# schmidtniko/visual_marker_mapping

Measured on AMD Instinct MI355X. Metric: lm_iterations_per_sec, higher is better.
Workload: dtype f64; 1 GPU; configs[1]: 500 images x 200 tags, visibility 1.00, 100000 tag observations (400000 corner residual blocks), no loss, perturbed initial guess; eliminated_family=cameras, reduced_system_order=1200, elimination_form=dense Z + MFMA rank-k, kept_family_order=natural

## Files before the change

### __graft_entry__.py

```python
import os
import subprocess
import sys

ROOT = os.path.dirname(os.path.abspath(__file__))
if ROOT not in sys.path:
    sys.path.insert(0, ROOT)


def build():
    jobs = str(min(8, os.cpu_count() or 2))
    subprocess.check_call(["make", "-C", os.path.join(ROOT, "visual_marker_mapping_amd", "csrc"), "-j", jobs, "all", "stamps"])
    subprocess.check_call(["make", "-C", os.path.join(ROOT, "tools"), "all"])
    subprocess.check_call(["make", "-C", os.path.join(ROOT, "oracle"), "all"])
    subprocess.check_call(["make", "-C", os.path.join(ROOT, "tests", "cpp"), "all"])
    import visual_marker_mapping_amd
    from visual_marker_mapping_amd import _lib
    L = _lib.lib()
    missing = [s for s in _lib.EXPORTS if not hasattr(L, s)]
    if missing:
        raise RuntimeError("libvmm_ba.so lacks symbols: %s" % missing)


def smoke():
    import numpy as np
    from oracle import oracle as O
    from visual_marker_mapping_amd import engine as eng
    from visual_marker_mapping_amd.synthetic import make_scene

    s = make_scene(1)
    ba = eng.BundleAdjuster(s.intr, s.dist, s.cam_init, s.tag_init, s.tag_wh, s.fixed_tag, s.obs_cam,
                            s.obs_tag, s.obs_px, device=0)
    out = ba.solve(eng.default_options(robustify=1), trace_capacity=64)
    cam, tag = ba.get_state()
    ba.close()
    sc = O.Scene(s.intr, s.dist, s.cam_init, s.tag_init, s.tag_wh, s.fixed_tag, s.obs_cam, s.obs_tag, s.obs_px)
    summ, _ = O.solve(sc, O.default_options(robustify=1, linear_solver=O.DENSE_NORMAL))
    assert out["termination_type"] == summ["termination_type"] == O.CONVERGENCE, (out, summ)
    assert out["iterations"] == summ["iterations"], (out["iterations"], summ["iterations"])
    assert abs(out["final_cost"] - summ["final_cost"]) <= 1e-8 * summ["final_cost"]
    scale = max(np.abs(sc.cam_qt).max(), np.abs(sc.tag_qt).max())
    assert np.abs(cam - sc.cam_qt).max() <= 1e-6 * scale
    assert np.abs(tag - sc.tag_qt).max() <= 1e-6 * scale
    print("smoke ok: %d iterations, final cost %.9g (oracle %.9g)" % (out["iterations"], out["final_cost"],
                                                                    summ["final_cost"]))


if __name__ == "__main__":
    build()
    if len(sys.argv) > 1 and sys.argv[1] == "smoke":
        smoke()
```

### include/vmm_ba.h

```cpp
#ifndef VMM_BA_H_
#define VMM_BA_H_

#include <stddef.h>
#include <stdint.h>

#ifdef __cplusplus
extern "C" {
#endif

#define VMM_BA_ABI_VERSION 6

typedef struct vmm_ba_handle_s* vmm_ba_handle;

enum {
    VMM_BA_OK = 0,
    VMM_BA_ERR_ARGUMENT = 1,
    VMM_BA_ERR_HIP = 2,
    VMM_BA_ERR_COLLECTIVE = 3,
    VMM_BA_ERR_STATE = 4,
    VMM_BA_ERR_NUMERIC = 5
};

enum {
    VMM_BA_ELIM_AUTO = 0,
// ... 259 lines not shown
    int32_t robustify;
    double  huber_a;
    double  score_cap_px;
    double  inlier_px;
    int32_t reclassify_passes;
    int32_t min_inlier_views;
    int32_t max_pair_views;
    int32_t reserved;
} vmm_ba_triangulate_options;

typedef struct vmm_ba_triangulate_result {
    int32_t status, n_obs, n_inlier_obs, trials;
    double  rms_px, cost;
} vmm_ba_triangulate_result;

void vmm_ba_default_triangulate_options(vmm_ba_triangulate_options* o);
int vmm_ba_triangulate(const double intr[4], const double dist[5],
                       int32_t n_cams, const double* cam_qt,
                       const double* cam_cov,
                       int32_t n_pts, const int64_t* pt_start,
                       const int32_t* obs_cam, const double* obs_uv,
                       const vmm_ba_triangulate_options* o,
                       double* xyz,
                       double* xyz_cov,
                       double* xyz_cov_cams,
                       uint8_t* obs_inlier,
                       vmm_ba_triangulate_result* res,
                       int device);

int vmm_ba_locate_tags(const double intr[4], const double dist[5],
                       int32_t n_cams, const double* cam_qt,
                       const double* cam_cov,
                       int32_t n_tags, const double* tag_wh,
                       const int64_t* tag_start,
                       const int32_t* obs_cam, const double* obs_px,
                       const vmm_ba_localize_options* o,
                       double* tag_qt,
                       double* tag_cov,
                       double* tag_cov_cams,
                       uint8_t* obs_inlier,
                       vmm_ba_localize_result* res,
                       int device);

enum { VMM_BA_PRED_OK = 0, VMM_BA_PRED_NO_VISIBLE_TAG = 1, VMM_BA_PRED_TOO_FEW_TAGS = 2, VMM_BA_PRED_SINGULAR = 3 };
typedef struct vmm_ba_predict_options {
    int32_t image_width, image_height;
    double  sigma_px;
    double  margin_px;
    double  min_depth;
    double  max_view_angle_deg;
    double  min_side_px;
    int32_t min_tags;
    int32_t reserved;
} vmm_ba_predict_options;

typedef struct vmm_ba_predict_result {
    int32_t status;
    int32_t n_visible;
    double  sigma_pos_m;
    double  sigma_rot_rad;
} vmm_ba_predict_result;

void vmm_ba_default_predict_options(vmm_ba_predict_options* o);
int vmm_ba_predict_localization(const double intr[4], const double dist[5],
                                int32_t n_tags, const double* tag_qt, const double* tag_wh,
                                const double* tag_cov,
                                int32_t n_poses, const double* cam_qt,
                                const vmm_ba_predict_options* o,
                                double* cov_px,
                                double* cov_map,
                                uint8_t* visible,
                                vmm_ba_predict_result* res,
                                int device);

int vmm_ba_predict_localization_joint(const double intr[4], const double dist[5],
                                      int32_t n_tags, const double* tag_qt, const double* tag_wh,
                                      const double* tag_cov_joint,
                                      int32_t n_poses, const double* cam_qt,
                                      const uint8_t* visible_in,
                                      const vmm_ba_predict_options* o,
                                      double* cov_px,
                                      double* cov_map,
                                      uint8_t* visible,
                                      vmm_ba_predict_result* res,
                                      int device);

enum { VMM_BA_CAL_OK = 0, VMM_BA_CAL_NO_IMAGES = 1, VMM_BA_CAL_SINGULAR = 2, VMM_BA_CAL_NO_CONVERGENCE = 3 };
typedef struct vmm_ba_calibrate_options {
    vmm_ba_localize_options loc;
    int32_t max_trials;
    int32_t refine_mask;
    int32_t robustify;
    int32_t reclassify_passes;
    int32_t min_inlier_tags;
    int32_t reserved;
    double  huber_a;
    double  inlier_px;
} vmm_ba_calibrate_options;
typedef struct vmm_ba_calibrate_report {
    int32_t status, trials, accepted, passes, n_images_used, n_obs_used;
    double initial_cost, final_cost, initial_rms_px, final_rms_px, time_s;
} vmm_ba_calibrate_report;
void vmm_ba_default_calibrate_options(vmm_ba_calibrate_options* o);
int vmm_ba_calibrate(const double intr0[4], const double dist0[5],
                     int32_t n_tags, const double* tag_qt, const double* tag_wh,
                     int32_t n_imgs, const int64_t* img_start, const int32_t* obs_tag, const double* obs_px,
                     const vmm_ba_calibrate_options* o,
                     double intr[4], double dist[5],
                     double* intr_cov,
                     double* cam_qt,
                     double* cam_cov,
                     uint8_t* obs_inlier,
                     vmm_ba_localize_result* res,
                     vmm_ba_calibrate_report* rep,
                     int device);

int vmm_ba_set_intrinsics(vmm_ba_handle h, const double intr[4], const double dist[5]);
int vmm_ba_get_intrinsics(vmm_ba_handle h, double intr[4], double dist[5]);

int vmm_ba_intrinsics_system(vmm_ba_handle h, int robustify, double huber_a, double* cost, double g_k[9], double C[81],
                             double r_k[9], double S_k[81]);

typedef struct vmm_ba_selfcal_options {
    int32_t max_outer_iterations;
    int32_t refine_mask;
    double parameter_tolerance;
    double function_tolerance;
} vmm_ba_selfcal_options;
typedef struct vmm_ba_selfcal_report {
    int32_t status;
    int32_t outer_iterations;
    int32_t accepted;
    int32_t inner_lm_iterations;
    double initial_cost;
    double final_cost;
    double time_s;
} vmm_ba_selfcal_report;
void vmm_ba_default_selfcal_options(vmm_ba_selfcal_options* o);
int vmm_ba_solve_selfcal(vmm_ba_handle h, const vmm_ba_options* inner, const vmm_ba_selfcal_options* o,
                         vmm_ba_summary* last_inner, vmm_ba_selfcal_report* report, double intr[4], double dist[5],
                         double* intr_cov );

int vmm_ba_eval_blocks(vmm_ba_handle h, int robustify, double huber_a, double* cost, double* V,
                       double* U, double* W, double* g_cam, double* g_tag);

int vmm_ba_dense_spd_solve(int device, int n, const double* A, const double* b, double* x, int* info);

int vmm_ba_dense_syrk(int device, int k, int n, const double* Z, double* C);

int vmm_ba_pose_plus(int64_t n, const double* qt, const double* delta, double* out, int device);

int vmm_ba_debug_overlap(vmm_ba_handle h, int reps, double* ms);

int vmm_ba_debug_chol_schedule(int n_blk, int n_df, int n_cu, int32_t* launches, int cap, int* n_launches, int* n_df_used);
int vmm_ba_debug_chol_tile(int n_blk, const int32_t* launch, int t, int* bi, int* bj);

int vmm_ba_time_kernels(vmm_ba_handle h, const vmm_ba_options* opt, int reps, vmm_ba_kernel_times* out);

#ifdef __cplusplus
}
#endif
#endif
```

### visual_marker_mapping_amd/_lib.py

```python
import ctypes as C
import os

_HERE = os.path.dirname(os.path.abspath(__file__))
LIB_PATH = os.environ.get("VMM_BA_LIB") or os.path.join(_HERE, "libvmm_ba.so")

ABI_VERSION = 6
RCCL_ID_BYTES = 128
PRECISION_F64, PRECISION_F32_ACCUM = 0, 1
LANDMARK_TAG_POSES, LANDMARK_POINTS = 0, 1
RIG_MAX_CAMS = 8
OK, ERR_ARGUMENT, ERR_HIP, ERR_COLLECTIVE, ERR_STATE, ERR_NUMERIC = 0, 1, 2, 3, 4, 5
ELIM_AUTO, ELIM_TAGS, ELIM_CAMERAS = 0, 1, 2
CONVERGENCE, NO_CONVERGENCE, FAILURE = 0, 1, 2
LOC_OK, LOC_NO_OBSERVATIONS, LOC_NO_CANDIDATE, LOC_TOO_FEW_INLIERS, LOC_SINGULAR = 0, 1, 2, 3, 4
LOC_STATUS_NAMES = ("ok", "no_observations", "no_candidate", "too_few_inliers", "singular")
TRI_OK, TRI_TOO_FEW_VIEWS, TRI_NO_CANDIDATE, TRI_TOO_FEW_INLIERS, TRI_SINGULAR = 0, 1, 2, 3, 4
TRI_STATUS_NAMES = ("ok", "too_few_views", "no_candidate", "too_few_inliers", "singular")
CAL_OK, CAL_NO_IMAGES, CAL_SINGULAR, CAL_NO_CONVERGENCE = 0, 1, 2, 3
CAL_STATUS_NAMES = ("ok", "no_images", "singular", "no_convergence")
PRED_OK, PRED_NO_VISIBLE_TAG, PRED_TOO_FEW_TAGS, PRED_SINGULAR = 0, 1, 2, 3
PRED_STATUS_NAMES = ("ok", "no_visible_tag", "too_few_tags", "singular")


class Problem(C.Structure):
# ... 35 lines not shown
                ("num_lm_iterations", C.c_int32), ("num_jacobian_evals", C.c_int32),
                ("num_cost_evals", C.c_int32), ("elimination", C.c_int32),
                ("initial_cost", C.c_double), ("final_cost", C.c_double), ("time_solve_s", C.c_double),
                ("trace", C.POINTER(Iteration)), ("trace_capacity", C.c_int32), ("reserved", C.c_int32),
                ("time_eval_s", C.c_double), ("time_eliminate_s", C.c_double), ("time_factor_solve_s", C.c_double),
                ("time_step_s", C.c_double), ("time_control_s", C.c_double),
                ("num_sync_timeouts", C.c_int32), ("sync_timeout_kernels", C.c_int32),
                ("block_sparse", C.c_int32), ("tree_ordering", C.c_int32)]


class KernelTimes(C.Structure):
    _fields_ = [("eval_elim_ms", C.c_double), ("eval_keep_ms", C.c_double), ("cost_ms", C.c_double),
                ("form_z_ms", C.c_double), ("syrk_ms", C.c_double), ("cholesky_ms", C.c_double),
                ("backsub_ms", C.c_double), ("lm_iteration_ms", C.c_double), ("n_obs", C.c_int64),
                ("reduced_dim", C.c_int32), ("elim_dim", C.c_int32), ("schur_sparse", C.c_int32),
                ("syrk_wide", C.c_int32), ("schur_flops", C.c_double), ("chol_flops", C.c_double)]


class InitOptions(C.Structure):
    _fields_ = [("sweeps", C.c_int32), ("min_tag_observations", C.c_int32), ("score_cap_px", C.c_double),
                ("refine_iterations", C.c_int32), ("reserved", C.c_int32)]


class InitReport(C.Structure):
    _fields_ = [("rounds", C.c_int32), ("cams_reached", C.c_int32), ("tags_reached", C.c_int32),
                ("reserved", C.c_int32), ("avg_reprojection_px", C.c_double), ("time_s", C.c_double)]


class LocalizeOptions(C.Structure):
    _fields_ = [("refine_iterations", C.c_int32), ("robustify", C.c_int32), ("huber_a", C.c_double),
                ("score_cap_px", C.c_double), ("inlier_px", C.c_double), ("reclassify_passes", C.c_int32),
                ("min_inlier_tags", C.c_int32)]


class LocalizeResult(C.Structure):
    _fields_ = [("status", C.c_int32), ("n_obs", C.c_int32), ("n_inlier_obs", C.c_int32), ("trials", C.c_int32),
                ("rms_px", C.c_double), ("cost", C.c_double)]


class TriangulateOptions(C.Structure):
    _fields_ = [("refine_iterations", C.c_int32), ("robustify", C.c_int32), ("huber_a", C.c_double),
                ("score_cap_px", C.c_double), ("inlier_px", C.c_double), ("reclassify_passes", C.c_int32),
                ("min_inlier_views", C.c_int32), ("max_pair_views", C.c_int32), ("reserved", C.c_int32)]


class TriangulateResult(C.Structure):
    _fields_ = [("status", C.c_int32), ("n_obs", C.c_int32), ("n_inlier_obs", C.c_int32), ("trials", C.c_int32),
                ("rms_px", C.c_double), ("cost", C.c_double)]


class PredictOptions(C.Structure):
    _fields_ = [("image_width", C.c_int32), ("image_height", C.c_int32), ("sigma_px", C.c_double), ("margin_px", C.c_double),
                ("min_depth", C.c_double), ("max_view_angle_deg", C.c_double), ("min_side_px", C.c_double),
                ("min_tags", C.c_int32), ("reserved", C.c_int32)]


class PredictResult(C.Structure):
    _fields_ = [("status", C.c_int32), ("n_visible", C.c_int32), ("sigma_pos_m", C.c_double), ("sigma_rot_rad", C.c_double)]


class CalibrateOptions(C.Structure):
    _fields_ = [("loc", LocalizeOptions), ("max_trials", C.c_int32), ("refine_mask", C.c_int32),
                ("robustify", C.c_int32), ("reclassify_passes", C.c_int32), ("min_inlier_tags", C.c_int32),
                ("reserved", C.c_int32), ("huber_a", C.c_double), ("inlier_px", C.c_double)]


class CalibrateReport(C.Structure):
    _fields_ = [("status", C.c_int32), ("trials", C.c_int32), ("accepted", C.c_int32), ("passes", C.c_int32),
                ("n_images_used", C.c_int32), ("n_obs_used", C.c_int32), ("initial_cost", C.c_double),
                ("final_cost", C.c_double), ("initial_rms_px", C.c_double), ("final_rms_px", C.c_double),
                ("time_s", C.c_double)]


class RigCalibrateOptions(C.Structure):
    _fields_ = [("loc", LocalizeOptions), ("max_trials", C.c_int32), ("refine_mask", C.c_int32),
                ("robustify", C.c_int32), ("reclassify_passes", C.c_int32), ("min_inlier_tags", C.c_int32),
                ("reserved", C.c_int32), ("huber_a", C.c_double), ("inlier_px", C.c_double)]


class RigCalibrateReport(C.Structure):
    _fields_ = [("status", C.c_int32), ("trials", C.c_int32), ("accepted", C.c_int32), ("passes", C.c_int32),
                ("n_frames_used", C.c_int32), ("n_obs_used", C.c_int32), ("cams_refined", C.c_int32),
                ("reserved", C.c_int32), ("initial_cost", C.c_double), ("final_cost", C.c_double),
                ("initial_rms_px", C.c_double), ("final_rms_px", C.c_double), ("time_s", C.c_double)]


class SelfcalOptions(C.Structure):
    _fields_ = [("max_outer_iterations", C.c_int32), ("refine_mask", C.c_int32), ("parameter_tolerance", C.c_double),
                ("function_tolerance", C.c_double)]


class SelfcalReport(C.Structure):
    _fields_ = [("status", C.c_int32), ("outer_iterations", C.c_int32), ("accepted", C.c_int32),
                ("inner_lm_iterations", C.c_int32), ("initial_cost", C.c_double), ("final_cost", C.c_double),
                ("time_s", C.c_double)]


ALLREDUCE_FN = C.CFUNCTYPE(C.c_int, C.c_void_p, C.c_void_p, C.c_size_t, C.c_void_p)

_h = _a = C.c_void_p
_i, _i32, _i64, _d, _P = C.c_int, C.c_int32, C.c_int64, C.c_double, C.POINTER
_MAP = [_i32, _a, _a]
_BATCH = [_i32, _a, _a, _a]
SIGNATURES = {
    "vmm_ba_last_error": (C.c_char_p, []),
    "vmm_ba_abi_version": (_i, []),
    "vmm_ba_default_options": (None, [_P(Options)]),
    "vmm_ba_default_create_options": (None, [_P(CreateOptions)]),
    "vmm_ba_create": (_i, [_P(Problem), _P(CreateOptions), _P(C.c_void_p)]),
    "vmm_ba_destroy": (None, [_h]),
    "vmm_ba_set_state": (_i, [_h, _a, _a]),
    "vmm_ba_get_state": (_i, [_h, _a, _a]),
    "vmm_ba_get_points": (_i, [_h, _a]),
    "vmm_ba_set_allreduce": (_i, [_h, ALLREDUCE_FN, C.c_void_p]),
    "vmm_ba_rccl_available": (_i, []),
    "vmm_ba_rccl_unique_id": (_i, [_a]),
    "vmm_ba_enable_rccl": (_i, [_h, _a]),
    "vmm_ba_set_observation_mask": (_i, [_h, _a]),
    "vmm_ba_set_constant_poses": (_i, [_h, _a, _a]),
    "vmm_ba_solve": (_i, [_h, _P(Options), _P(Summary)]),
    "vmm_ba_cost": (_i, [_h, _i, _d, _P(_d)]),
    "vmm_ba_reprojection_stats": (_i, [_h, _a, _a, _P(_d), _a]),
    "vmm_ba_tag_translation_covariance": (_i, [_h, _i, _d, _a]),
    "vmm_ba_covariance_blocks": (_i, [_h, _i, _d, _i64, _a, _a, _a]),
    "vmm_ba_project_points": (_i, [_a, _a, _i64, _a, _a, _i]),
    "vmm_ba_quad_poses": (_i, [_a, _a, _i64, _a, _a, _a, _a, _i]),
    "vmm_ba_default_init_options": (None, [_P(InitOptions)]),
    "vmm_ba_initialize": (_i, [_h, _P(InitOptions), _P(InitReport), _a, _a]),
    "vmm_ba_default_localize_options": (None, [_P(LocalizeOptions)]),
    "vmm_ba_localize": (_i, [_a, _a] + _MAP + _BATCH + [_P(LocalizeOptions), _a, _a, _a, _a, _i]),
    "vmm_ba_rig_localize": (_i, [_i32, _a, _a, _a] + _MAP + _BATCH + [_P(LocalizeOptions), _a, _a, _a, _a, _i]),
    "vmm_ba_default_rig_calibrate_options": (None, [_P(RigCalibrateOptions)]),
    "vmm_ba_rig_calibrate": (_i, [_i32, _a, _a, _a] + _MAP + _BATCH + [_P(RigCalibrateOptions), _a, _a, _a, _a, _a, _a,
                                  _P(RigCalibrateReport), _i]),
    "vmm_ba_default_triangulate_options": (None, [_P(TriangulateOptions)]),
    "vmm_ba_triangulate": (_i, [_a, _a, _i32, _a, _a] + _BATCH + [_P(TriangulateOptions), _a, _a, _a, _a, _a, _i]),
    "vmm_ba_locate_tags": (_i, [_a, _a, _i32, _a, _a, _i32, _a, _a, _a, _a, _P(LocalizeOptions), _a, _a, _a, _a, _a, _i]),
    "vmm_ba_default_predict_options": (None, [_P(PredictOptions)]),
    "vmm_ba_predict_localization": (_i, [_a, _a] + _MAP + [_a, _i32, _a, _P(PredictOptions), _a, _a, _a, _a, _i]),
    "vmm_ba_predict_localization_joint": (_i, [_a, _a] + _MAP + [_a, _i32, _a, _a, _P(PredictOptions), _a, _a, _a, _a, _i]),
    "vmm_ba_default_calibrate_options": (None, [_P(CalibrateOptions)]),
    "vmm_ba_calibrate": (_i, [_a, _a] + _MAP + _BATCH + [_P(CalibrateOptions), _a, _a, _a, _a, _a, _a, _a,
                              _P(CalibrateReport), _i]),
    "vmm_ba_set_intrinsics": (_i, [_h, _a, _a]),
    "vmm_ba_get_intrinsics": (_i, [_h, _a, _a]),
    "vmm_ba_intrinsics_system": (_i, [_h, _i, _d, _P(_d), _a, _a, _a, _a]),
    "vmm_ba_default_selfcal_options": (None, [_P(SelfcalOptions)]),
    "vmm_ba_solve_selfcal": (_i, [_h, _P(Options), _P(SelfcalOptions), _P(Summary), _P(SelfcalReport), _a, _a, _a]),
    "vmm_ba_eval_blocks": (_i, [_h, _i, _d, _P(_d), _a, _a, _a, _a, _a]),
    "vmm_ba_dense_spd_solve": (_i, [_i, _i, _a, _a, _a, _P(_i)]),
    "vmm_ba_dense_syrk": (_i, [_i, _i, _i, _a, _a]),
    "vmm_ba_pose_plus": (_i, [_i64, _a, _a, _a, _i]),
    "vmm_ba_debug_overlap": (_i, [_h, _i, _a]),
    "vmm_ba_debug_chol_schedule": (_i, [_i, _i, _i, _a, _i, _a, _a]),
    "vmm_ba_debug_chol_tile": (_i, [_i, _a, _i, _a, _a]),
    "vmm_ba_time_kernels": (_i, [_h, _P(Options), _i, _P(KernelTimes)]),
}
EXPORTS = list(SIGNATURES)
OPTIONAL = {"vmm_ba_covariance_blocks", "vmm_ba_rig_localize", "vmm_ba_default_rig_calibrate_options", "vmm_ba_rig_calibrate",
            "vmm_ba_default_calibrate_options", "vmm_ba_calibrate", "vmm_ba_default_triangulate_options",
            "vmm_ba_triangulate", "vmm_ba_locate_tags", "vmm_ba_default_predict_options", "vmm_ba_predict_localization",
            "vmm_ba_predict_localization_joint",
            "vmm_ba_set_intrinsics", "vmm_ba_get_intrinsics", "vmm_ba_intrinsics_system",
            "vmm_ba_default_selfcal_options", "vmm_ba_solve_selfcal"}

_LIB = None


class VmmBaError(RuntimeError):
    def __init__(self, status, message):
        super().__init__("libvmm_ba status %d: %s" % (status, message))
        self.status = status


def lib():
    global _LIB
    if _LIB is None:
        if not os.path.exists(LIB_PATH):
            raise ImportError("%s is missing: build it with __graft_entry__.build() or "
                              "make -C visual_marker_mapping_amd/csrc" % LIB_PATH)
        L = C.CDLL(LIB_PATH)
        L.vmm_ba_abi_version.restype = C.c_int
        if L.vmm_ba_abi_version() != ABI_VERSION:
            raise ImportError("%s has ABI version %d, this binding needs %d: rebuild it"
                              % (LIB_PATH, L.vmm_ba_abi_version(), ABI_VERSION))
        for name, (restype, argtypes) in SIGNATURES.items():
            if name in OPTIONAL and not hasattr(L, name):
                continue
            fn = getattr(L, name)
            fn.restype, fn.argtypes = restype, argtypes
        _LIB = L
    return _LIB


def check(status):
    if status != OK:
        raise VmmBaError(status, lib().vmm_ba_last_error().decode("utf-8", "replace"))
```

### visual_marker_mapping_amd/csrc/diagnostics.hip

```cpp
#include <stdio.h>
#include <string.h>

#include <string>
#include <vector>

#include "host.hpp"

namespace vmm {

template <typename T, hipError_t (*Destroy)(T), int N = 1>
struct Owned {
    T h[N] = {};
    Owned() = default;
    Owned(const Owned&) = delete;
    Owned& operator=(const Owned&) = delete;
    ~Owned() { release(); }
    void release()
    {
        for (T& x : h) {
            if (x)
                (void)Destroy(x);
            x = nullptr;
        }
    }
// ... 120 lines not shown
    for (int r = 0; r < reps; ++r) {
        if ((rc = run_iteration(e, ot))) return rc;
        passes += e.last_passes;
    }
    HIP_TRY(hipEventRecord(ev1, e.stream));
    HIP_TRY(hipEventSynchronize(ev1));
    float ms = 0.f;
    HIP_TRY(hipEventElapsedTime(&ms, ev0, ev1));
    out->lm_iteration_ms = ms / passes;
    events.release();
    return restore_raw();
}

int vmm_ba_debug_chol_schedule(int n_blk, int n_df, int n_cu, int32_t* launches, int cap, int* n_launches, int* n_df_used)
{
    if (n_blk < 1 || n_cu < 1 || cap < 0 || (cap > 0 && !launches) || !n_launches || (n_df > 0 && n_df > n_blk - 2)) {
        set_error("bad argument");
        return VMM_BA_ERR_ARGUMENT;
    }
    if (n_df < 0) {
        n_df = dataflow_blocks(n_blk, n_cu, read_switches());
        if (n_df == n_blk)
            n_df = 0;
    }
    const std::vector<CholLaunch> sched = chol_step_schedule(n_blk, n_df);
    for (size_t i = 0; i < sched.size() && (int)i < cap; ++i) {
        const CholLaunch& L = sched[i];
        const int32_t row[8] = { L.k, L.lazy[0], L.lazy[1], L.upd[0], L.upd[1], L.c0, L.t0, L.t1 };
        memcpy(launches + 8 * i, row, sizeof(row));
    }
    *n_launches = (int)sched.size();
    if (n_df_used)
        *n_df_used = n_df;
    return VMM_BA_OK;
}

int vmm_ba_debug_chol_tile(int n_blk, const int32_t* launch, int t, int* bi, int* bj)
{
    if (!launch || !bi || !bj || t < 0 || t >= launch[7]) {
        set_error("bad argument");
        return VMM_BA_ERR_ARGUMENT;
    }
    const CholLaunch L = { launch[0], { launch[1], launch[2] }, { launch[3], launch[4] }, launch[5], launch[6], launch[7] };
    chol_schedule_tile(n_blk, L, t, bi, bj);
    return VMM_BA_OK;
}

int vmm_ba_debug_overlap(vmm_ba_handle h, int reps, double* ms)
{
    if (!h || !ms || reps <= 0) {
        set_error("bad argument");
        return VMM_BA_ERR_ARGUMENT;
    }
    Engine& e = *reinterpret_cast<Engine*>(h);
    if (e.multi || e.sparse_schur || !e.Z) {
        set_error("debug_overlap needs a single-GPU handle on the dense elimination path");
        return VMM_BA_ERR_STATE;
    }
    HIP_TRY(hipSetDevice(e.device));
    int rc;
    if ((rc = flush_state(e))) return rc;
    vmm_ba_options o;
    vmm_ba_default_options(&o);
    o.max_num_iterations = 1 << 30;
    o.function_tolerance = o.parameter_tolerance = o.gradient_tolerance = 0.0;
    if (e.trace_capacity < 1) {
        if ((rc = dev_alloc(e, &e.trace, 1, false))) return rc;
        e.trace_capacity = 1;
        drop_graphs(e);
    }
    if ((rc = begin_lm_loop(e, o, 0))) return rc;
    if ((rc = enqueue_iteration(e, o))) return rc;
    HIP_TRY(hipStreamSynchronize(e.stream));
    Arena scratch;
    Owned<hipStream_t, hipStreamDestroy> second;
    OwnedEvents<5> events;
    hipStream_t& sb = second.h[0];
    hipEvent_t(&ev)[5] = events.h;
    hipError_t err = scratch.alloc(sizeof(double) * (size_t)e.ldz * e.ldz);
    double* const S2 = reinterpret_cast<double*>(scratch.base);
    if (err == hipSuccess) err = hipStreamCreateWithFlags(&sb, hipStreamNonBlocking);
    for (int i = 0; i < 5 && err == hipSuccess; ++i)
        err = hipEventCreate(&ev[i]);
    auto reset_flags = [&]() -> hipError_t {
        hipError_t r = hipMemcpy(e.ctl_host, e.ctl, sizeof(LmCtl), hipMemcpyDeviceToHost);
        if (r != hipSuccess) return r;
        e.ctl_host->done = 0;
        e.ctl_host->lin_fail = 0;
        e.ctl_host->sync_timeout = 0;
        return hipMemcpy(e.ctl, e.ctl_host, sizeof(LmCtl), hipMemcpyHostToDevice);
    };
    double acc[8] = { 0.0, 0.0, 0.0, 0.0, 0.0, 0.0, 0.0, 0.0 };
    for (int r = 0; r < reps + 1 && err == hipSuccess; ++r) {
        float t[8] = { 0.f, 0.f, 0.f, 0.f, 0.f, 0.f, 0.f, 0.f };
        if ((err = reset_flags()) != hipSuccess) break;
        (void)hipEventRecord(ev[0], e.stream);
        launch_syrk_reduced(e);
        (void)hipEventRecord(ev[1], e.stream);
        launch_cholesky_solve(e, e.S, e.n_pad, e.ldz, e.yf, e.ctl);
        (void)hipEventRecord(ev[2], e.stream);
        if ((err = hipEventSynchronize(ev[2])) != hipSuccess) break;
        (void)hipEventElapsedTime(&t[0], ev[0], ev[1]);
        (void)hipEventElapsedTime(&t[1], ev[1], ev[2]);
        (void)hipEventElapsedTime(&t[2], ev[0], ev[2]);
        if ((err = reset_flags()) != hipSuccess) break;
        launch_syrk_reduced(e);
        if ((err = hipStreamSynchronize(e.stream)) != hipSuccess) break;
        (void)hipEventRecord(ev[0], e.stream);
        (void)hipStreamWaitEvent(sb, ev[0], 0);
        launch_cholesky_solve(e, e.S, e.n_pad, e.ldz, e.yf, e.ctl);
        (void)hipEventRecord(ev[3], e.stream);
        launch_syrk_plan(sb, e.ctl, e.Z, e.ldz, e.syrk);
        launch_reduce_plan(sb, e.ctl, e.syrk, e.ldz, e.n_pad + 1, S2);
        (void)hipEventRecord(ev[1], sb);
        (void)hipStreamWaitEvent(e.stream, ev[1], 0);
        (void)hipEventRecord(ev[2], e.stream);
        if ((err = hipEventSynchronize(ev[2])) != hipSuccess) break;
        (void)hipEventElapsedTime(&t[3], ev[0], ev[2]);
        (void)hipEventElapsedTime(&t[4], ev[0], ev[3]);
        (void)hipEventElapsedTime(&t[5], ev[0], ev[1]);
        if ((err = reset_flags()) != hipSuccess) break;
        launch_syrk_reduced(e);
        if ((err = hipStreamSynchronize(e.stream)) != hipSuccess) break;
        (void)hipEventRecord(ev[0], e.stream);
        (void)hipStreamWaitEvent(sb, ev[0], 0);
        launch_syrk_plan(sb, e.ctl, e.Z, e.ldz, e.syrk);
        launch_reduce_plan(sb, e.ctl, e.syrk, e.ldz, e.n_pad + 1, S2);
        (void)hipEventRecord(ev[1], sb);
        (void)hipEventRecord(ev[4], e.stream);
        launch_cholesky_solve(e, e.S, e.n_pad, e.ldz, e.yf, e.ctl);
        (void)hipEventRecord(ev[3], e.stream);
        (void)hipStreamWaitEvent(e.stream, ev[1], 0);
        (void)hipEventRecord(ev[2], e.stream);
        if ((err = hipEventSynchronize(ev[2])) != hipSuccess) break;
        (void)hipEventElapsedTime(&t[6], ev[0], ev[2]);
        (void)hipEventElapsedTime(&t[7], ev[4], ev[3]);
        if (r > 0)
            for (int i = 0; i < 8; ++i)
                acc[i] += t[i];
    }
    if (err == hipSuccess)
        err = hipGetLastError();
    events.release();
    second.release();
    if (err != hipSuccess) {
        set_error(std::string("debug_overlap: ") + hipGetErrorString(err));
        return VMM_BA_ERR_HIP;
    }
    for (int i = 0; i < 8; ++i)
        ms[i] = acc[i] / reps;
    return VMM_BA_OK;
}

}
```

### visual_marker_mapping_amd/csrc/engine.hpp

```cpp
#pragma once
#include <hip/hip_runtime.h>
#include <stdint.h>

#include <string>
#include <vector>

#include "../../include/vmm_ba.h"
#include "geom.hpp"
#include "plan.hpp"

namespace vmm {

constexpr int kLdsRow = 80;

struct ObsOrder {
    int64_t n = 0;
    int64_t n_pad = 0;
    int32_t* own = nullptr;
    int32_t* other = nullptr;
    int32_t* caller = nullptr;
    double* px = nullptr;
    Task* tasks = nullptr;
    int32_t n_tasks = 0;
    int32_t* pose_task = nullptr;
    double* part = nullptr;
    int32_t* start = nullptr;
};

struct LmCtl {
    int32_t max_num_iterations, robustify, jacobi_scaling, max_invalid;
    double huber_a, function_tolerance, gradient_tolerance, parameter_tolerance;
    double max_radius, min_radius, min_relative_decrease, min_lm_diagonal, max_lm_diagonal;
    double radius, decrease_factor;
    int32_t reuse_diagonal, num_invalid;
    double x_cost, cand_cost, model_cost_change, x_norm, initial_cost;
    int32_t iteration;
    int32_t first_eval;
    int32_t done, termination;
    int32_t lin_fail;
    int32_t sync_timeout;
    int32_t num_sync_timeouts;
    int32_t sync_kernels;
    uint32_t spin_limit_df, spin_limit_chain;
    int32_t spin_wg;
    int32_t records;
    int32_t num_successful, num_unsuccessful, num_lm_iterations, num_jac_evals, num_cost_evals;
    int32_t trace_capacity;
    int32_t w_which;
    vmm_ba_iteration cur;
    unsigned long long stamp[6];
    unsigned long long phase_ticks[5];
};

__device__ __forceinline__ int64_t small_sel(const LmCtl* ctl, const int64_t alt_off) { return ctl->w_which ? alt_off : 0; }

__device__ __forceinline__ void phase_stamp(const LmCtl* ctl, int slot)
{
    if (blockIdx.x == 0 && blockIdx.y == 0 && threadIdx.x == 0)
        const_cast<LmCtl*>(ctl)->stamp[slot] = __builtin_amdgcn_s_memrealtime();
}

struct SyrkPlan {
    int n_tiles = 0, n_kt = 0, n_wg = 0, n_segments = 0;
    int32_t *tile_bi = nullptr, *tile_bj = nullptr, *wg_seg0 = nullptr, *tile_seg0 = nullptr;
    int64_t *wg_u0 = nullptr, *wg_u1 = nullptr;
    double* partials = nullptr;
    bool wide = false;
};

struct Engine {
    int device = 0;
    int n_cu = 256;
    hipStream_t stream = nullptr;
    int rank = 0, world = 1;
    Switches sw;
    bool multi = false;
    vmm_ba_allreduce_fn allreduce = nullptr;
    void* allreduce_user = nullptr;
    void* rccl_comm = nullptr;
    bool rccl_graph = true;

    Intrinsics K;
    int n_cams = 0, n_tags = 0, fixed_tag = -1;
    bool points = false;
    int n_tags_user = 0;
    int64_t n_obs_user = 0;
    std::vector<double> user_tag_wh;
    int64_t n_obs = 0;
    bool elim_cams = true;
    int n_e = 0, n_f = 0;

    double* cam_qt = nullptr;
    double* tag_qt = nullptr;
    double* cam_cand = nullptr;
    double* tag_cand = nullptr;
    double* tag_wh = nullptr;

    ObsOrder ordE, ordF;

    double* small = nullptr;
    size_t small_count = 0;
    double *H_cam = nullptr, *H_tag = nullptr, *g_cam = nullptr, *g_tag = nullptr, *cost_slot = nullptr;
    double* small_stage = nullptr;
    int64_t small_alt_off = 0;
    double *ev_H_cam = nullptr, *ev_H_tag = nullptr, *ev_g_cam = nullptr, *ev_g_tag = nullptr, *ev_cost = nullptr;
    double* ev_pose_cost = nullptr;
    double* W = nullptr;
    double* W2 = nullptr;
    float* Wf2 = nullptr;
    uint8_t* obs_mask = nullptr;
    uint8_t* pose_const = nullptr;
    bool any_const = false;
    float* Wf = nullptr;
    bool f32_accum = false;

    bool fused_eval = false;
    int32_t* pair_obs = nullptr;
    int32_t* fused_e_list = nullptr;
    int32_t* fused_e_part0 = nullptr;
    int32_t* fused_pose_task = nullptr;
    double* fused_partE = nullptr;
    double* fused_partF = nullptr;
    int fused_n_e_act = 0, fused_f_pad = 0, fused_chunks = 0, fused_group = 1, fused_groups = 0;

    double *scale = nullptr, *diag = nullptr, *D2 = nullptr, *delta = nullptr;
    int32_t* active = nullptr;

    double* Le = nullptr;
    double* ze = nullptr;
    double* Z = nullptr;
    int k_dim = 0, k_pad = 0;
    int n_red = 0, n_pad = 0, ldz = 0, n_blk = 0;
    bool sparse_schur = false;
    double* Zc = nullptr;
    int32_t* f2e = nullptr;
    int32_t* pair_start = nullptr;
    int32_t* pair_tstart = nullptr;
    int32_t* pair_terms = nullptr;
    int32_t* row_items = nullptr;
    double co_terms = 0.0;
    bool explicit_pairs = false;
    int32_t* pair_col = nullptr;
    int32_t* row_of = nullptr;
    int32_t* pose_of_row = nullptr;
    std::vector<int32_t> h_row_of;
    unsigned long long* chol_nz = nullptr;
    unsigned char* chol_order = nullptr;
    int32_t* df_wg = nullptr;
    int32_t* df_slot = nullptr;
    int n_df_wg = 0;
    size_t df_tree_slots = 0;
    bool chol_nz_on = false;
    std::vector<int32_t> nd_node_first_blk;
    int n_row_items = 0;
    double schur_flops = 0.0;
    double chol_flops = 0.0;
    SyrkPlan syrk;
    double* S = nullptr;
    double* S_packed = nullptr;
    double* P = nullptr;
    double* P4[4] = { nullptr, nullptr, nullptr, nullptr };
    double* dinv = nullptr;
    double* Ldiag = nullptr;
    double* Linv = nullptr;
    unsigned* flags = nullptr;
    unsigned long long* gran = nullptr;
    unsigned long long* df_gran = nullptr;
    double* df_compact = nullptr;
    unsigned* df_done = nullptr;
    double* yf = nullptr;
    double* step_comm = nullptr;
    double* cost_comm = nullptr;
    double* part_cost = nullptr;
    double* part_cross = nullptr;
    double* part_k1 = nullptr;
    double* pose_part = nullptr;
    double* pose_gm = nullptr;

    double* stats_part = nullptr;
    int32_t* stats_cnt = nullptr;
    double* stats_pose = nullptr;
    double* stats_corner = nullptr;

    double* init_quad_qt = nullptr;
    double* init_quad_rms = nullptr;
    int32_t* init_placed = nullptr;
    int32_t* init_todo = nullptr;
    int32_t* init_counter = nullptr;
    double* init_stats = nullptr;
    double* init_host = nullptr;

    LmCtl* ctl = nullptr;
    LmCtl* ctl_host = nullptr;
    double* pose_stage = nullptr;
    hipEvent_t pose_ev = nullptr;
    bool pose_ev_pending = false;
    double* pose_stage_dev = nullptr;
    bool dirty_cam = false, dirty_tag = false;
    vmm_ba_iteration* trace = nullptr;
    int trace_capacity = 0;

    hipGraphExec_t iter_graph = nullptr;
    hipGraphExec_t iter_graph_seg[5] = { nullptr, nullptr, nullptr, nullptr, nullptr };
    int graph_robustify = -1;
    double graph_huber_a = 0.0;
    int last_passes = 1;
    bool launched_eagerly = false;

    std::vector<void*> allocs;
};

void set_error(const std::string& s);

__host__ __device__ inline Intrinsics make_intrinsics(const double intr[4], const double dist[5])
{
    Intrinsics K;
    K.fx = intr[0]; K.fy = intr[1]; K.cx = intr[2]; K.cy = intr[3];
    K.k1 = dist[0]; K.k2 = dist[1]; K.p1 = dist[2]; K.p2 = dist[3]; K.k3 = dist[4];
    return K;
}
__host__ __device__ inline Intrinsics make_intrinsics(const double k[9]) { return make_intrinsics(k, k + 4); }

struct Arena {
    char* base = nullptr;
    size_t used = 0;
    hipError_t err = hipSuccess;
    Arena() = default;
    Arena(const Arena&) = delete;
    Arena& operator=(const Arena&) = delete;
    ~Arena()
    {
        if (base)
            (void)hipFree(base);
    }
    hipError_t alloc(size_t bytes)
    {
        err = hipMalloc((void**)&base, bytes);
        if (err != hipSuccess)
            base = nullptr;
        return err;
    }
    static size_t round(size_t bytes) { return (bytes + 255) & ~(size_t)255; }
    template <typename T>
    T* take(size_t count)
    {
        T* p = base ? reinterpret_cast<T*>(base + used) : nullptr;
        used += round(count * sizeof(T));
        return p;
    }
    template <typename Carve>
    hipError_t layout(Carve&& carve)
    {
        carve(*this);
        const size_t total = used;
        used = 0;
        if (alloc(total) == hipSuccess)
            carve(*this);
        return err;
    }
    void copy(void* dst, const void* src, size_t bytes, hipMemcpyKind kind)
    {
        if (err == hipSuccess)
            err = hipMemcpy(dst, src, bytes, kind);
    }
};

int preload_eval_kernels();
int preload_schur_kernels();
int preload_chol_kernels();
int preload_lm_kernels();
int preload_cov_kernels();
int preload_init_kernels();

void launch_eval_passes(Engine& e, int robustify, double huber_a, bool use_ctl);
void launch_cost_kernel(Engine& e, const double* cam, const double* tag, bool guard, int robustify, double huber_a);
void launch_cost(Engine& e, const double* cam, const double* tag, bool guard, int robustify, double huber_a,
// ... 254 lines not shown
```

### visual_marker_mapping_amd/csrc/kernels_eval.hip

```cpp
#include "engine.hpp"

namespace vmm {

struct EvalArgs {
    Intrinsics K;
    const Task* tasks;
    int n_tasks;
    const int32_t* other;
    const double* px;
    int64_t n_pad;
    const double* own_pose;
    const double* other_pose;
    const double* tag_wh;
    const uint8_t* cam_const;
    const uint8_t* tag_const;
    int robustify;
    double huber_a;
    double* part;
    void* W;
    void* W_alt;
    const int32_t* caller;
    const uint8_t* mask;
    const LmCtl* ctl;
};

__device__ __forceinline__ int tri(int a, int b) { return a * (a + 1) / 2 + b; }

template <bool OWN_IS_CAM, bool WRITE_W, typename AT, bool POINTS = false>
__device__ __forceinline__ void eval_body(const EvalArgs& a, const int wave)
{
    const int lane = threadIdx.x & 63;
    if (wave >= a.n_tasks)
        return;
    const Task t = a.tasks[wave];
    const int64_t i = (int64_t)t.begin + lane;
    const bool valid = i < t.end;
    const int64_t is = valid ? i : t.begin;
    const int o = a.other[is];
    AT* __restrict__ const Wout = static_cast<AT*>((WRITE_W && a.W_alt && a.ctl && a.ctl->w_which == 0) ? a.W_alt : a.W);

    const int tag_idx = OWN_IS_CAM ? o : t.pose;
    const int cam_idx = OWN_IS_CAM ? t.pose : o;
    const double* camq = (OWN_IS_CAM ? a.own_pose : a.other_pose) + 7 * (int64_t)cam_idx;
    const double* tagq = (OWN_IS_CAM ? a.other_pose : a.own_pose) + 7 * (int64_t)tag_idx;
    Rigid cam, tag;
    double pt[6];
    if (POINTS) {
        load_rigid<false>(camq, cam);
#pragma unroll
        for (int k = 0; k < 6; ++k)
            pt[k] = tagq[k];
    } else {
        load_rigid<true>(camq, cam);
        load_rigid<true>(tagq, tag);
    }
    const double hw = POINTS ? 0.0 : 0.5 * a.tag_wh[2 * tag_idx], hh = POINTS ? 0.0 : 0.5 * a.tag_wh[2 * tag_idx + 1];
    const bool cam_c = a.cam_const[cam_idx] != 0, tag_c = a.tag_const[tag_idx] != 0;
    const bool on = valid && a.mask[a.caller[is]];

    AT H[21];
    double g[6], cost = 0.0;
    AT Wacc[WRITE_W ? 36 : 1];
#pragma unroll
    for (int k = 0; k < 21; ++k)
        H[k] = (AT)0;
#pragma unroll
    for (int k = 0; k < 6; ++k)
        g[k] = 0.0;
    if (WRITE_W) {
#pragma unroll
        for (int k = 0; k < 36; ++k)
            Wacc[k] = (AT)0;
    }

    constexpr bool NEED_JC = OWN_IS_CAM || WRITE_W;
    constexpr bool NEED_JT = !OWN_IS_CAM || WRITE_W;
#pragma unroll 1
    for (int c = 0; c < (POINTS ? 2 : 4); ++c) {
        const double sx = (c == 1 || c == 2) ? hw : -hw;
        const double sy = (c >= 2) ? hh : -hh;
        const double u = a.px[(2 * c) * a.n_pad + is];
        const double v = a.px[(2 * c + 1) * a.n_pad + is];
        CornerEval e;
        if (POINTS) {
            eval_point<NEED_JC, NEED_JT>(a.K, cam, camq, pt[3 * c], pt[3 * c + 1], pt[3 * c + 2], u, v, e, on);
            if (NEED_JT) {
#pragma unroll
                for (int r = 0; r < 2; ++r) {
                    const double j0 = e.jt[r][0], j1 = e.jt[r][1], j2 = e.jt[r][2];
                    e.jt[r][0] = c == 0 ? j0 : 0.0;
                    e.jt[r][1] = c == 0 ? j1 : 0.0;
                    e.jt[r][2] = c == 0 ? j2 : 0.0;
                    e.jt[r][3] = c == 0 ? 0.0 : j0;
                    e.jt[r][4] = c == 0 ? 0.0 : j1;
                    e.jt[r][5] = c == 0 ? 0.0 : j2;
                }
            }
        } else {
            eval_corner<NEED_JC, NEED_JT>(a.K, cam, tag, sx, sy, u, v, e, on);
        }
        const double s = e.ru * e.ru + e.rv * e.rv;
        double rho0, wgt;
        huber(a.robustify != 0, a.huber_a, s, rho0, wgt);
        wgt = on ? wgt : 0.0;
        cost += on ? 0.5 * rho0 : 0.0;
        const double w_cam = cam_c ? 0.0 : wgt, w_tag = tag_c ? 0.0 : wgt;
        const double w_own = OWN_IS_CAM ? w_cam : w_tag;
        const double w_oth = OWN_IS_CAM ? w_tag : w_cam;
#pragma unroll
        for (int r = 0; r < 2; ++r) {
            const double res = (r == 0 ? e.ru : e.rv) * wgt;
            double jo[6];
#pragma unroll
            for (int k = 0; k < 6; ++k)
                jo[k] = (OWN_IS_CAM ? e.jc[r][k] : e.jt[r][k]) * w_own;
            AT ja[6];
#pragma unroll
            for (int k = 0; k < 6; ++k)
                ja[k] = (AT)jo[k];
#pragma unroll
            for (int p = 0; p < 6; ++p) {
                g[p] += jo[p] * res;
#pragma unroll
                for (int q = 0; q <= p; ++q)
                    H[tri(p, q)] += ja[p] * ja[q];
            }
            if (WRITE_W) {
                AT jx[6];
#pragma unroll
                for (int k = 0; k < 6; ++k)
                    jx[k] = (AT)((OWN_IS_CAM ? e.jt[r][k] : e.jc[r][k]) * w_oth);
#pragma unroll
                for (int p = 0; p < 6; ++p)
#pragma unroll
                    for (int q = 0; q < 6; ++q)
                        Wacc[6 * p + q] += ja[p] * jx[q];
            }
        }
    }
    if (WRITE_W && valid) {
#pragma unroll
        for (int k = 0; k < 36; ++k)
            Wout[(int64_t)k * a.n_pad + i] = Wacc[k];
    }
    double red[32];
#pragma unroll
    for (int k = 0; k < 21; ++k)
        red[k] = (double)H[k];
#pragma unroll
    for (int k = 0; k < 6; ++k)
        red[21 + k] = g[k];
    red[27] = cost;
#pragma unroll
    for (int k = 28; k < 32; ++k)
        red[k] = 0.0;
    const double mine = wave_sum32(red, lane);
    const int slot = wave_sum32_index(lane);
    if (!(lane & 1) && slot < 28)
        a.part[(int64_t)wave * kPart + slot] = mine;
}

template <bool E_IS_CAM, typename AT = double, bool POINTS = false>
__global__ __launch_bounds__(256) __attribute__((amdgpu_waves_per_eu(2, 2))) void k_eval_both(const EvalArgs aE, const EvalArgs aF, const int nb_e)
{
    if (aE.ctl) {
        if (aE.ctl->done)
            return;
        phase_stamp(aE.ctl, 0);
    }
    if ((int)blockIdx.x < nb_e)
        eval_body<E_IS_CAM, true, AT, POINTS>(aE, (int)((blockIdx.x * blockDim.x + threadIdx.x) >> 6));
    else
        eval_body<!E_IS_CAM, false, AT, POINTS>(aF, (int)(((blockIdx.x - nb_e) * blockDim.x + threadIdx.x) >> 6));
}


struct FusedArgs {
    const int32_t* pair_obs;
    const int32_t* e_list;
    const int32_t* e_part0;
    int n_e_act, n_f, n_f_pad, n_chunks, group, n_groups;
    double* partF;
};

template <bool E_IS_CAM, typename AT, bool POINTS>
__global__ __launch_bounds__(256) __attribute__((amdgpu_waves_per_eu(1, 1)))
void k_eval_fused(const EvalArgs a, const FusedArgs fa)
{
    if (a.ctl) {
        if (a.ctl->done)
            return;
        phase_stamp(a.ctl, 0);
    }
    const int lane = threadIdx.x & 63;
    const int wave = (int)((blockIdx.x * blockDim.x + threadIdx.x) >> 6);
    if (wave >= fa.n_groups * fa.n_chunks)
        return;
    const int grp = wave / fa.n_chunks, c = wave - grp * fa.n_chunks;
    const int f = 64 * c + lane;
    const bool fvalid = f < fa.n_f;
    const int fs = fvalid ? f : fa.n_f - 1;
    AT* __restrict__ const Wout = static_cast<AT*>((a.W_alt && a.ctl && a.ctl->w_which == 0) ? a.W_alt : a.W);
    const double* keptq = a.other_pose + 7 * (int64_t)fs;
    Rigid kept;
    double pt[6];
    if (POINTS && E_IS_CAM) {
#pragma unroll
        for (int k = 0; k < 6; ++k)
            pt[k] = keptq[k];
    } else if (POINTS) {
        load_rigid<false>(keptq, kept);
    } else {
        load_rigid<true>(keptq, kept);
    }
    AT HF[21];
    double gF[6];
#pragma unroll
    for (int k = 0; k < 21; ++k)
        HF[k] = (AT)0;
#pragma unroll
    for (int k = 0; k < 6; ++k)
        gF[k] = 0.0;
    const int e0 = grp * fa.group, e1 = min(e0 + fa.group, fa.n_e_act);
    constexpr int NPX = POINTS ? 4 : 8;
    int e_n = __builtin_amdgcn_readfirstlane(fa.e_list[e0]);
    int idx_n = fvalid ? fa.pair_obs[(int64_t)e_n * fa.n_f_pad + f] : -1;
    int e_nn = e_n, idx_nn = -1;
    if (e0 + 1 < e1) {
        e_nn = __builtin_amdgcn_readfirstlane(fa.e_list[e0 + 1]);
        idx_nn = fvalid ? fa.pair_obs[(int64_t)e_nn * fa.n_f_pad + f] : -1;
    }
    double px_n[NPX];
    int on_n;
    {
        const int64_t isn = idx_n >= 0 ? idx_n : 0;
#pragma unroll
        for (int k = 0; k < NPX; ++k)
            px_n[k] = a.px[(int64_t)k * a.n_pad + isn];
        on_n = idx_n >= 0 && a.mask[a.caller[isn]];
    }
    for (int ei = e0; ei < e1; ++ei) {
        const int e = e_n;
        const int idx = idx_n;
        const bool valid = idx >= 0;
        const bool on = on_n != 0;
        double pxc[NPX];
#pragma unroll
        for (int k = 0; k < NPX; ++k)
            pxc[k] = px_n[k];
        e_n = e_nn;
        idx_n = idx_nn;
        if (ei + 1 < e1) {
            const int64_t isn = idx_n >= 0 ? idx_n : 0;
#pragma unroll
            for (int k = 0; k < NPX; ++k)
                px_n[k] = a.px[(int64_t)k * a.n_pad + isn];
            on_n = idx_n >= 0 && a.mask[a.caller[isn]];
        }
        if (ei + 2 < e1) {
            e_nn = __builtin_amdgcn_readfirstlane(fa.e_list[ei + 2]);
            idx_nn = fvalid ? fa.pair_obs[(int64_t)e_nn * fa.n_f_pad + f] : -1;
        }
        const int tag_idx = E_IS_CAM ? fs : e;
        const double* elimq = a.own_pose + 7 * (int64_t)e;
        Rigid elim;
        if (POINTS && !E_IS_CAM) {
#pragma unroll
            for (int k = 0; k < 6; ++k)
                pt[k] = elimq[k];
        } else if (POINTS) {
            load_rigid<false>(elimq, elim);
        } else {
            load_rigid<true>(elimq, elim);
        }
        const Rigid& cam = E_IS_CAM ? elim : kept;
        const Rigid& tag = E_IS_CAM ? kept : elim;
        const double* camq = E_IS_CAM ? elimq : keptq;
        const double hw = POINTS ? 0.0 : 0.5 * a.tag_wh[2 * tag_idx], hh = POINTS ? 0.0 : 0.5 * a.tag_wh[2 * tag_idx + 1];
        const int cam_idx = E_IS_CAM ? e : fs;
        const bool cam_c = a.cam_const[cam_idx] != 0, tag_c = a.tag_const[tag_idx] != 0;
        AT H[21];
        double g[6], cost = 0.0;
        AT Wacc[36];
#pragma unroll
        for (int k = 0; k < 21; ++k)
            H[k] = (AT)0;
#pragma unroll
        for (int k = 0; k < 6; ++k)
            g[k] = 0.0;
#pragma unroll
        for (int k = 0; k < 36; ++k)
            Wacc[k] = (AT)0;
#pragma unroll 1
        for (int cn = 0; cn < (POINTS ? 2 : 4); ++cn) {
            const double sx = (cn == 1 || cn == 2) ? hw : -hw;
            const double sy = (cn >= 2) ? hh : -hh;
            double u = pxc[0], v = pxc[1];
#pragma unroll
            for (int k = 1; k < NPX / 2; ++k) {
                u = (cn == k) ? pxc[2 * k] : u;
                v = (cn == k) ? pxc[2 * k + 1] : v;
            }
            CornerEval ce;
            if (POINTS) {
                eval_point<true, true>(a.K, cam, camq, pt[3 * cn], pt[3 * cn + 1], pt[3 * cn + 2], u, v, ce, on);
#pragma unroll
                for (int r = 0; r < 2; ++r) {
                    const double j0 = ce.jt[r][0], j1 = ce.jt[r][1], j2 = ce.jt[r][2];
                    ce.jt[r][0] = cn == 0 ? j0 : 0.0;
                    ce.jt[r][1] = cn == 0 ? j1 : 0.0;
                    ce.jt[r][2] = cn == 0 ? j2 : 0.0;
                    ce.jt[r][3] = cn == 0 ? 0.0 : j0;
                    ce.jt[r][4] = cn == 0 ? 0.0 : j1;
                    ce.jt[r][5] = cn == 0 ? 0.0 : j2;
                }
            } else {
                eval_corner<true, true>(a.K, cam, tag, sx, sy, u, v, ce, on);
            }
            const double s = ce.ru * ce.ru + ce.rv * ce.rv;
            double rho0, wgt;
            huber(a.robustify != 0, a.huber_a, s, rho0, wgt);
            wgt = on ? wgt : 0.0;
            cost += on ? 0.5 * rho0 : 0.0;
            const double w_cam = cam_c ? 0.0 : wgt, w_tag = tag_c ? 0.0 : wgt;
            const double w_e = E_IS_CAM ? w_cam : w_tag;
            const double w_f = E_IS_CAM ? w_tag : w_cam;
#pragma unroll
            for (int r = 0; r < 2; ++r) {
                const double res = (r == 0 ? ce.ru : ce.rv) * wgt;
                double je[6], jf[6];
                AT ae[6], af[6];
#pragma unroll
                for (int k = 0; k < 6; ++k) {
                    je[k] = (E_IS_CAM ? ce.jc[r][k] : ce.jt[r][k]) * w_e;
                    jf[k] = (E_IS_CAM ? ce.jt[r][k] : ce.jc[r][k]) * w_f;
                    ae[k] = (AT)je[k];
                    af[k] = (AT)jf[k];
                }
#pragma unroll
                for (int p = 0; p < 6; ++p) {
                    g[p] += je[p] * res;
                    gF[p] += jf[p] * res;
#pragma unroll
                    for (int q = 0; q <= p; ++q) {
                        H[tri(p, q)] += ae[p] * ae[q];
                        HF[tri(p, q)] += af[p] * af[q];
                    }
#pragma unroll
                    for (int q = 0; q < 6; ++q)
                        Wacc[6 * p + q] += ae[p] * af[q];
                }
            }
        }
        if (valid) {
#pragma unroll
            for (int k = 0; k < 36; ++k)
                Wout[(int64_t)k * a.n_pad + idx] = Wacc[k];
        }
        double red[32];
#pragma unroll
        for (int k = 0; k < 21; ++k)
            red[k] = (double)H[k];
#pragma unroll
        for (int k = 0; k < 6; ++k)
            red[21 + k] = g[k];
        red[27] = cost;
#pragma unroll
        for (int k = 28; k < 32; ++k)
            red[k] = 0.0;
        const double mine = wave_sum32(red, lane);
        const int slot = wave_sum32_index(lane);
        if (!(lane & 1) && slot < 28)
            a.part[(int64_t)(fa.e_part0[e] + c) * kPart + slot] = mine;
    }
    if (fvalid) {
        double* pf = fa.partF + (int64_t)grp * 28 * fa.n_f_pad + f;
#pragma unroll
        for (int k = 0; k < 21; ++k)
            pf[(int64_t)k * fa.n_f_pad] = (double)HF[k];
#pragma unroll
        for (int k = 0; k < 6; ++k)
            pf[(int64_t)(21 + k) * fa.n_f_pad] = gF[k];
    }
}

struct ReduceArgs {
    int n_pose;
    const int32_t* pose_task;
    int n_fixed;
    int64_t st, sk, sp;
    const double* part;
    double* Hout;
    double* gout;
    double* pose_cost;
    const double* pose7;
    int euclid;
    double* gm_out;
};

__global__ void k_reduce_pose(const LmCtl* ctl, const ReduceArgs rE, const ReduceArgs rF, const int64_t alt_off)
{
    int64_t off = 0;
    if (ctl) {
        if (ctl->done)
            return;
        off = ctl->w_which ? 0 : alt_off;
    }
    int tid = blockIdx.x * blockDim.x + threadIdx.x;
    const bool first = tid < 32 * rE.n_pose;
    if (!first)
        tid -= 32 * rE.n_pose;
    const ReduceArgs& r = first ? rE : rF;
    const int n_pose = r.n_pose;
    const int32_t* __restrict__ pose_task = r.pose_task;
    const double* __restrict__ part = r.part;
    double* __restrict__ Hout = r.Hout + off;
    double* __restrict__ gout = r.gout + off;
    double* __restrict__ pose_cost = r.pose_cost;
    const int p = tid >> 5, k = tid & 31;
    if (p >= n_pose || k >= 28)
        return;
    const int t0 = pose_task ? pose_task[p] : 0, t1 = pose_task ? pose_task[p + 1] : r.n_fixed;
    const double* __restrict__ pp = part + (int64_t)k * r.sk + (int64_t)p * r.sp;
    double s0 = 0.0, s1 = 0.0, s2 = 0.0, s3 = 0.0;
    int t = t0;
    for (; t + 3 < t1; t += 4) {
        s0 += pp[(int64_t)t * r.st];
        s1 += pp[(int64_t)(t + 1) * r.st];
        s2 += pp[(int64_t)(t + 2) * r.st];
        s3 += pp[(int64_t)(t + 3) * r.st];
    }
    if (t < t1) s0 += pp[(int64_t)t * r.st];
    if (t + 1 < t1) s1 += pp[(int64_t)(t + 1) * r.st];
    if (t + 2 < t1) s2 += pp[(int64_t)(t + 2) * r.st];
    const double s = (s0 + s1) + (s2 + s3);
    if (k < 21) {
        int a = 0;
        while ((a + 1) * (a + 2) / 2 <= k)
            ++a;
        const int b = k - a * (a + 1) / 2;
        Hout[36 * (int64_t)p + 6 * a + b] = s;
        Hout[36 * (int64_t)p + 6 * b + a] = s;
    } else if (k < 27) {
        gout[6 * (int64_t)p + (k - 21)] = s;
    } else if (pose_cost) {
        pose_cost[p] = s;
    }
    if (r.gm_out) {
        double ng[6];
#pragma unroll
        for (int j = 0; j < 6; ++j)
            ng[j] = -__shfl(s, 21 + j, 32);
        if (k == 21) {
            const double* x = r.pose7 + 7 * (int64_t)p;
            double xp[7], gm = 0.0;
            if (r.euclid) {
#pragma unroll
                for (int j = 0; j < 6; ++j)
                    xp[j] = x[j] + ng[j];
                xp[6] = x[6];
            } else {
                pose_plus(x, ng, xp);
            }
#pragma unroll
            for (int j = 0; j < 7; ++j)
                gm = fmax(gm, fabs(x[j] - xp[j]));
            r.gm_out[p] = gm;
        }
    }
}

__global__ __launch_bounds__(256) void k_sum(const LmCtl* ctl, const double* __restrict__ in, int n, int stride,
                                             double* __restrict__ out)
{
    if (ctl && ctl->done)
        return;
    __shared__ double sh[256];
    double s = 0.0;
    for (int i = threadIdx.x; i < n; i += 256)
        s += in[(int64_t)i * stride];
    sh[threadIdx.x] = s;
    __syncthreads();
    for (int m = 128; m >= 1; m >>= 1) {
        if ((int)threadIdx.x < m)
            sh[threadIdx.x] += sh[threadIdx.x + m];
        __syncthreads();
    }
    if (threadIdx.x == 0)
        out[0] = sh[0];
}

struct CostArgs {
    Intrinsics K;
    const Task* tasks;
    int n_tasks;
    const int32_t* other;
    const double* px;
    int64_t n_pad;
    const double* own_pose;
    const double* other_pose;
    const double* tag_wh;
    int robustify;
    double huber_a;
    double* part;
    const int32_t* caller;
    const uint8_t* mask;
    const LmCtl* ctl;
};

template <bool OWN_IS_CAM, bool POINTS = false>
__global__ __launch_bounds__(256) void k_cost(const CostArgs a)
{
    if (a.ctl && a.ctl->done)
        return;
    const int wave = (int)((blockIdx.x * blockDim.x + threadIdx.x) >> 6);
    const int lane = threadIdx.x & 63;
    if (wave >= a.n_tasks)
        return;
    const Task t = a.tasks[wave];
    const int64_t i = (int64_t)t.begin + lane;
    const bool valid = i < t.end;
    const int64_t is = valid ? i : t.begin;
    const int o = a.other[is];
    const int tag_idx = OWN_IS_CAM ? o : t.pose;
    const int cam_idx = OWN_IS_CAM ? t.pose : o;
    const double* camq = (OWN_IS_CAM ? a.own_pose : a.other_pose) + 7 * (int64_t)cam_idx;
    const double* tagq = (OWN_IS_CAM ? a.other_pose : a.own_pose) + 7 * (int64_t)tag_idx;
    Rigid cam, tag;
    double pt[6];
    if (POINTS) {
        load_rigid<false>(camq, cam);
#pragma unroll
        for (int k = 0; k < 6; ++k)
            pt[k] = tagq[k];
    } else {
        load_rigid<true>(camq, cam);
        load_rigid<true>(tagq, tag);
    }
    const double hw = POINTS ? 0.0 : 0.5 * a.tag_wh[2 * tag_idx], hh = POINTS ? 0.0 : 0.5 * a.tag_wh[2 * tag_idx + 1];
    double cost = 0.0;
#pragma unroll
    for (int c = 0; c < (POINTS ? 2 : 4); ++c) {
        const double sx = (c == 1 || c == 2) ? hw : -hw;
        const double sy = (c >= 2) ? hh : -hh;
        CornerEval e;
        if (POINTS)
            eval_point<false, false>(a.K, cam, camq, pt[3 * c], pt[3 * c + 1], pt[3 * c + 2],
                                     a.px[(2 * c) * a.n_pad + is], a.px[(2 * c + 1) * a.n_pad + is], e);
        else
            eval_corner<false, false>(a.K, cam, tag, sx, sy, a.px[(2 * c) * a.n_pad + is],
                                      a.px[(2 * c + 1) * a.n_pad + is], e);
        double rho0, wgt;
        huber(a.robustify != 0, a.huber_a, e.ru * e.ru + e.rv * e.rv, rho0, wgt);
        cost += 0.5 * rho0;
    }
    cost = wave_sum((valid && a.mask[a.caller[is]]) ? cost : 0.0);
    if (lane == 0)
        a.part[wave] = cost;
}

struct StatsArgs {
    Intrinsics K;
    const Task* tasks;
    int n_tasks;
    const int32_t* other;
    const int32_t* caller;
    const double* px;
    int64_t n_pad;
    const double* own_pose;
    const double* other_pose;
    const double* tag_wh;
    double* part;
    int32_t* part_n;
    double* per_corner;
    const uint8_t* mask;
};

template <bool OWN_IS_CAM>
__global__ __launch_bounds__(256) void k_stats(const StatsArgs a)
{
    const int wave = (int)((blockIdx.x * blockDim.x + threadIdx.x) >> 6);
    const int lane = threadIdx.x & 63;
    if (wave >= a.n_tasks)
        return;
    const Task t = a.tasks[wave];
    const int64_t i = (int64_t)t.begin + lane;
    const bool valid = i < t.end;
    const int64_t is = valid ? i : t.begin;
    const int o = a.other[is];
    Rigid own, oth;
    load_rigid<false>(a.own_pose + 7 * (int64_t)t.pose, own);
    load_rigid<false>(a.other_pose + 7 * (int64_t)o, oth);
    const Rigid& cam = OWN_IS_CAM ? own : oth;
    const Rigid& tag = OWN_IS_CAM ? oth : own;
    const int tag_idx = OWN_IS_CAM ? o : t.pose;
    const double hw = 0.5 * a.tag_wh[2 * tag_idx], hh = 0.5 * a.tag_wh[2 * tag_idx + 1];
    const int64_t ci = a.caller[is];
    const bool on = valid && a.mask[ci];
    double sum = 0.0;
#pragma unroll
    for (int c = 0; c < 4; ++c) {
        const double sx = (c == 1 || c == 2) ? hw : -hw;
        const double sy = (c >= 2) ? hh : -hh;
        CornerEval e;
        eval_corner<false, false, true>(a.K, cam, tag, sx, sy, a.px[(2 * c) * a.n_pad + is],
                                        a.px[(2 * c + 1) * a.n_pad + is], e);
        sum += sqrt(e.ru * e.ru + e.rv * e.rv);
        if (a.per_corner && valid) {
            a.per_corner[8 * ci + 2 * c] = on ? e.ru : 0.0;
            a.per_corner[8 * ci + 2 * c + 1] = on ? e.rv : 0.0;
        }
    }
    sum = wave_sum(on ? sum : 0.0);
    const int n_on = __popcll(__ballot(on));
    if (lane == 0) {
        a.part[wave] = sum;
        a.part_n[wave] = n_on;
    }
}

__global__ void k_stats_pose(int n_cam, const int32_t* __restrict__ task_c, const double* __restrict__ part_c,
                             const int32_t* __restrict__ cnt_c, int n_tag, const int32_t* __restrict__ task_t,
                             const double* __restrict__ part_t, const int32_t* __restrict__ cnt_t,
                             double* __restrict__ out)
{
    const int p = blockIdx.x * blockDim.x + threadIdx.x;
    if (p >= n_cam + n_tag)
        return;
    const bool is_cam = p < n_cam;
    const int q = is_cam ? p : p - n_cam;
    const int32_t* pt = is_cam ? task_c : task_t;
    const double* part = is_cam ? part_c : part_t;
    const int32_t* cnt = is_cam ? cnt_c : cnt_t;
    double s = 0.0;
    int64_t n = 0;
    for (int t = pt[q]; t < pt[q + 1]; ++t) {
        s += part[t];
        n += 4 * (int64_t)cnt[t];
    }
    out[p] = s;
    out[n_cam + n_tag + p] = (double)n;
}

__global__ void k_project(Intrinsics K, int64_t n, const double* __restrict__ pc, double* __restrict__ uv)
{
    const int64_t i = (int64_t)blockIdx.x * blockDim.x + threadIdx.x;
    if (i >= n)
        return;
    const double X = pc[3 * i], Y = pc[3 * i + 1], Z = pc[3 * i + 2];
    const double x = X / Z, y = Y / Z;
    const double r2 = x * x + y * y;
    const double rad = 1.0 + r2 * (K.k1 + r2 * (K.k2 + r2 * K.k3));
    double xd, yd;
    distort(K, true, x, y, r2, rad, xd, yd);
    uv[2 * i] = K.fx * xd + K.cx;
    uv[2 * i + 1] = K.fy * yd + K.cy;
}


static inline int blocks_for_tasks(int n_tasks) { return (n_tasks + 3) / 4; }

static EvalArgs make_eval_args(Engine& e, const ObsOrder& ord, bool own_is_cam, void* W, bool lm = false)
{
    EvalArgs a;
    a.K = e.K;
    a.tasks = ord.tasks;
    a.n_tasks = ord.n_tasks;
    a.other = ord.other;
    a.px = ord.px;
    a.n_pad = ord.n_pad;
    const double* cam = lm ? e.cam_cand : e.cam_qt;
    const double* tag = lm ? e.tag_cand : e.tag_qt;
    a.own_pose = own_is_cam ? cam : tag;
    a.other_pose = own_is_cam ? tag : cam;
    a.tag_wh = e.tag_wh;
    a.cam_const = e.pose_const;
    a.tag_const = e.pose_const + e.n_cams;
    a.robustify = 0;
    a.huber_a = 1.0;
    a.part = ord.part;
    a.W = W;
    a.W_alt = (lm && W) ? (e.f32_accum ? (void*)e.Wf2 : (void*)e.W2) : nullptr;
    a.caller = ord.caller;
    a.mask = e.obs_mask;
    a.ctl = e.ctl;
    return a;
}

void launch_eval_passes(Engine& e, int robustify, double huber_a, bool use_ctl)
{
    const bool e_is_cam = e.elim_cams;
    const bool lm = use_ctl;
    EvalArgs aE = make_eval_args(e, e.ordE, e_is_cam, e.f32_accum ? (void*)e.Wf : (void*)e.W, lm);
    EvalArgs aF = make_eval_args(e, e.ordF, !e_is_cam, nullptr, lm);
    aE.robustify = aF.robustify = robustify;
    aE.huber_a = aF.huber_a = huber_a;
    if (!use_ctl)
        aE.ctl = aF.ctl = nullptr;
    const int nb_e = blocks_for_tasks(aE.n_tasks), nb_f = blocks_for_tasks(aF.n_tasks);
    if (e.fused_eval) {
        FusedArgs fa;
        fa.pair_obs = e.pair_obs;
        fa.e_list = e.fused_e_list;
        fa.e_part0 = e.fused_e_part0;
        fa.n_e_act = e.fused_n_e_act;
        fa.n_f = e.n_f;
        fa.n_f_pad = e.fused_f_pad;
        fa.n_chunks = e.fused_chunks;
        fa.group = e.fused_group;
        fa.n_groups = e.fused_groups;
        fa.partF = e.fused_partF;
        aE.part = e.fused_partE;
        const int n_waves = fa.n_groups * fa.n_chunks;
        const dim3 grid((n_waves + 3) / 4);
        if (n_waves > 0) {
            if (e.points) {
                if (e_is_cam)
                    hipLaunchKernelGGL((k_eval_fused<true, double, true>), grid, dim3(256), 0, e.stream, aE, fa);
                else
                    hipLaunchKernelGGL((k_eval_fused<false, double, true>), grid, dim3(256), 0, e.stream, aE, fa);
            } else if (e.f32_accum) {
                if (e_is_cam)
                    hipLaunchKernelGGL((k_eval_fused<true, float, false>), grid, dim3(256), 0, e.stream, aE, fa);
                else
                    hipLaunchKernelGGL((k_eval_fused<false, float, false>), grid, dim3(256), 0, e.stream, aE, fa);
            } else if (e_is_cam)
                hipLaunchKernelGGL((k_eval_fused<true, double, false>), grid, dim3(256), 0, e.stream, aE, fa);
            else
                hipLaunchKernelGGL((k_eval_fused<false, double, false>), grid, dim3(256), 0, e.stream, aE, fa);
        }
    } else if (nb_e + nb_f > 0) {
        if (e.points) {
            if (e_is_cam)
                hipLaunchKernelGGL((k_eval_both<true, double, true>), dim3(nb_e + nb_f), dim3(256), 0, e.stream, aE, aF, nb_e);
            else
                hipLaunchKernelGGL((k_eval_both<false, double, true>), dim3(nb_e + nb_f), dim3(256), 0, e.stream, aE, aF, nb_e);
        } else if (e.f32_accum) {
            if (e_is_cam)
                hipLaunchKernelGGL((k_eval_both<true, float>), dim3(nb_e + nb_f), dim3(256), 0, e.stream, aE, aF, nb_e);
            else
                hipLaunchKernelGGL((k_eval_both<false, float>), dim3(nb_e + nb_f), dim3(256), 0, e.stream, aE, aF, nb_e);
        } else if (e_is_cam)
            hipLaunchKernelGGL((k_eval_both<true>), dim3(nb_e + nb_f), dim3(256), 0, e.stream, aE, aF, nb_e);
        else
            hipLaunchKernelGGL((k_eval_both<false>), dim3(nb_e + nb_f), dim3(256), 0, e.stream, aE, aF, nb_e);
    }
    const LmCtl* ctl = use_ctl ? e.ctl : nullptr;
    const bool stage = lm && e.multi;
    double* const oH_cam = stage ? e.ev_H_cam : e.H_cam;
    double* const oH_tag = stage ? e.ev_H_tag : e.H_tag;
    double* const og_cam = stage ? e.ev_g_cam : e.g_cam;
    double* const og_tag = stage ? e.ev_g_tag : e.g_tag;
    ReduceArgs rE, rF;
    rE.n_pose = e.n_e;
    rE.pose_task = e.ordE.pose_task;
    rE.part = e.ordE.part;
    rE.Hout = e_is_cam ? oH_cam : oH_tag;
    rE.gout = e_is_cam ? og_cam : og_tag;
    rE.pose_cost = (lm && e.multi) ? e.ev_pose_cost : e.part_cost;
    const bool want_gm = lm && !e.multi;
    rE.pose7 = want_gm ? (e_is_cam ? e.cam_cand : e.tag_cand) : nullptr;
    rE.euclid = (e.points && !e_is_cam) ? 1 : 0;
    rE.gm_out = want_gm ? e.pose_gm + (e_is_cam ? 0 : e.n_cams) : nullptr;
    rF.pose7 = want_gm ? (e_is_cam ? e.tag_cand : e.cam_cand) : nullptr;
    rF.euclid = (e.points && e_is_cam) ? 1 : 0;
    rF.gm_out = want_gm ? e.pose_gm + (e_is_cam ? e.n_cams : 0) : nullptr;
    rF.n_pose = e.n_f;
    rF.pose_task = e.ordF.pose_task;
    rF.part = e.ordF.part;
    rE.n_fixed = rF.n_fixed = 0;
    rE.st = rF.st = kPart;
    rE.sk = rF.sk = 1;
    rE.sp = rF.sp = 0;
    if (e.fused_eval) {
        rE.pose_task = e.fused_pose_task;
        rE.part = e.fused_partE;
        rF.pose_task = nullptr;
        rF.n_fixed = e.fused_groups;
        rF.part = e.fused_partF;
        rF.st = 28 * (int64_t)e.fused_f_pad;
        rF.sk = e.fused_f_pad;
        rF.sp = 1;
    }
    rF.Hout = e_is_cam ? oH_tag : oH_cam;
    rF.gout = e_is_cam ? og_tag : og_cam;
    rF.pose_cost = nullptr;
    hipLaunchKernelGGL(k_reduce_pose, dim3(((e.n_e + e.n_f) * 32 + 255) / 256), dim3(256), 0, e.stream, ctl, rE, rF,
                       (lm && !e.multi) ? e.small_alt_off : (int64_t)0);
    if (!lm)
        hipLaunchKernelGGL(k_sum, dim3(1), dim3(256), 0, e.stream, ctl, e.part_cost, e.n_e, 1,
                           e.cost_slot);
}

void launch_sum(Engine& e, bool guard, const double* in, int n, double* out)
{
    hipLaunchKernelGGL(k_sum, dim3(1), dim3(256), 0, e.stream, guard ? e.ctl : (const LmCtl*)nullptr, in, n, 1, out);
}

void launch_cost_kernel(Engine& e, const double* cam, const double* tag, bool guard, int robustify, double huber_a)
{
    CostArgs a;
    a.K = e.K;
    a.tasks = e.ordE.tasks;
    a.n_tasks = e.ordE.n_tasks;
    a.other = e.ordE.other;
    a.px = e.ordE.px;
    a.n_pad = e.ordE.n_pad;
    a.own_pose = e.elim_cams ? cam : tag;
    a.other_pose = e.elim_cams ? tag : cam;
    a.tag_wh = e.tag_wh;
    a.robustify = robustify;
    a.huber_a = huber_a;
    a.part = e.part_k1;
    a.caller = e.ordE.caller;
    a.mask = e.obs_mask;
    a.ctl = guard ? e.ctl : nullptr;
    if (a.n_tasks <= 0)
        return;
    const dim3 grid(blocks_for_tasks(a.n_tasks));
    if (e.points) {
        if (e.elim_cams)
            hipLaunchKernelGGL((k_cost<true, true>), grid, dim3(256), 0, e.stream, a);
        else
            hipLaunchKernelGGL((k_cost<false, true>), grid, dim3(256), 0, e.stream, a);
    } else if (e.elim_cams)
        hipLaunchKernelGGL((k_cost<true>), grid, dim3(256), 0, e.stream, a);
    else
        hipLaunchKernelGGL((k_cost<false>), grid, dim3(256), 0, e.stream, a);
}

void launch_cost(Engine& e, const double* cam, const double* tag, bool guard, int robustify, double huber_a,
                 double* out_scalar)
{
    launch_cost_kernel(e, cam, tag, guard, robustify, huber_a);
    launch_sum(e, guard, e.part_k1, e.ordE.n_tasks, out_scalar);
}

void launch_stats(Engine& e, double* per_corner_dev)
{
    const ObsOrder& oc = e.elim_cams ? e.ordE : e.ordF;
    const ObsOrder& ot = e.elim_cams ? e.ordF : e.ordE;
    double* part_cam = e.stats_part;
    double* part_tag = e.stats_part + oc.n_tasks;
    int32_t* n_cam = e.stats_cnt;
    int32_t* n_tag = e.stats_cnt + oc.n_tasks;
    StatsArgs a;
    a.K = e.K;
    a.tag_wh = e.tag_wh;
    a.mask = e.obs_mask;
    a.tasks = oc.tasks; a.n_tasks = oc.n_tasks; a.other = oc.other; a.caller = oc.caller; a.px = oc.px;
    a.n_pad = oc.n_pad; a.own_pose = e.cam_qt; a.other_pose = e.tag_qt; a.part = part_cam; a.part_n = n_cam;
    a.per_corner = per_corner_dev;
    if (a.n_tasks > 0)
        hipLaunchKernelGGL((k_stats<true>), dim3(blocks_for_tasks(a.n_tasks)), dim3(256), 0, e.stream, a);
    a.tasks = ot.tasks; a.n_tasks = ot.n_tasks; a.other = ot.other; a.caller = ot.caller; a.px = ot.px;
    a.n_pad = ot.n_pad; a.own_pose = e.tag_qt; a.other_pose = e.cam_qt; a.part = part_tag; a.part_n = n_tag;
    a.per_corner = nullptr;
    if (a.n_tasks > 0)
        hipLaunchKernelGGL((k_stats<false>), dim3(blocks_for_tasks(a.n_tasks)), dim3(256), 0, e.stream, a);
    hipLaunchKernelGGL(k_stats_pose, dim3((e.n_cams + e.n_tags + 255) / 256), dim3(256), 0, e.stream, e.n_cams,
                       (const int32_t*)oc.pose_task, (const double*)part_cam, (const int32_t*)n_cam, e.n_tags,
                       (const int32_t*)ot.pose_task, (const double*)part_tag, (const int32_t*)n_tag, e.stats_pose);
}

void launch_project(hipStream_t st, const Intrinsics& K, int64_t n, const double* pc, double* uv)
{
    if (n > 0)
        hipLaunchKernelGGL(k_project, dim3((unsigned)((n + 255) / 256)), dim3(256), 0, st, K, n, pc, uv);
}

int preload_eval_kernels()
{
    hipFuncAttributes at;
    int bad = 0;
    bad += hipFuncGetAttributes(&at, reinterpret_cast<const void*>(&k_eval_both<true, double>)) != hipSuccess;
    bad += hipFuncGetAttributes(&at, reinterpret_cast<const void*>(&k_eval_both<false, double>)) != hipSuccess;
    bad += hipFuncGetAttributes(&at, reinterpret_cast<const void*>(&k_eval_both<true, float>)) != hipSuccess;
    bad += hipFuncGetAttributes(&at, reinterpret_cast<const void*>(&k_eval_both<false, float>)) != hipSuccess;
    bad += hipFuncGetAttributes(&at, reinterpret_cast<const void*>(&k_eval_both<true, double, true>)) != hipSuccess;
    bad += hipFuncGetAttributes(&at, reinterpret_cast<const void*>(&k_eval_both<false, double, true>)) != hipSuccess;
    bad += hipFuncGetAttributes(&at, reinterpret_cast<const void*>(&k_eval_fused<true, double, false>)) != hipSuccess;
    bad += hipFuncGetAttributes(&at, reinterpret_cast<const void*>(&k_eval_fused<false, double, false>)) != hipSuccess;
    bad += hipFuncGetAttributes(&at, reinterpret_cast<const void*>(&k_eval_fused<true, float, false>)) != hipSuccess;
    bad += hipFuncGetAttributes(&at, reinterpret_cast<const void*>(&k_eval_fused<false, float, false>)) != hipSuccess;
    bad += hipFuncGetAttributes(&at, reinterpret_cast<const void*>(&k_eval_fused<true, double, true>)) != hipSuccess;
    bad += hipFuncGetAttributes(&at, reinterpret_cast<const void*>(&k_eval_fused<false, double, true>)) != hipSuccess;
    bad += hipFuncGetAttributes(&at, reinterpret_cast<const void*>(&k_cost<true, true>)) != hipSuccess;
    bad += hipFuncGetAttributes(&at, reinterpret_cast<const void*>(&k_cost<false, true>)) != hipSuccess;
    bad += hipFuncGetAttributes(&at, reinterpret_cast<const void*>(&k_reduce_pose)) != hipSuccess;
    bad += hipFuncGetAttributes(&at, reinterpret_cast<const void*>(&k_sum)) != hipSuccess;
    bad += hipFuncGetAttributes(&at, reinterpret_cast<const void*>(&k_cost<true>)) != hipSuccess;
    bad += hipFuncGetAttributes(&at, reinterpret_cast<const void*>(&k_cost<false>)) != hipSuccess;
    bad += hipFuncGetAttributes(&at, reinterpret_cast<const void*>(&k_stats<true>)) != hipSuccess;
    bad += hipFuncGetAttributes(&at, reinterpret_cast<const void*>(&k_stats<false>)) != hipSuccess;
    bad += hipFuncGetAttributes(&at, reinterpret_cast<const void*>(&k_stats_pose)) != hipSuccess;
    bad += hipFuncGetAttributes(&at, reinterpret_cast<const void*>(&k_project)) != hipSuccess;
    return bad;
}

}
```

### visual_marker_mapping_amd/csrc/kernels_schur.hip

```cpp
#include "engine.hpp"
#include "small_solve.hpp"

namespace vmm {


__device__ __forceinline__ bool chol6(double (&A)[36])
{
    return cholesky<6>(A, A, RowMajor<6>{}, PivotOrOne{});
}

template <typename WT, bool SPARSE>
__global__ __launch_bounds__(256) void k_form_z(LmCtl* ctl, int64_t n_obs, int64_t n_pad,
                                                 const int32_t* __restrict__ own,
                                                 const int32_t* __restrict__ other,
                                                 const WT* __restrict__ W0, const WT* __restrict__ W1,
                                                 const double* __restrict__ H_E0, const double* __restrict__ g_E0,
                                                 const int64_t alt_off,
                                                 const double* __restrict__ D2,
                                                 double* __restrict__ Le, double* __restrict__ ze,
                                                 const double* __restrict__ scale, int e_off_pose,
                                                 int f_off_pose, double* __restrict__ Z, int ldz, int zcol,
                                                 const int32_t* __restrict__ e_start)
{
    if (ctl->done)
        return;
    phase_stamp(ctl, 2);
    const int64_t i = (int64_t)blockIdx.x * blockDim.x + threadIdx.x;
    if (i >= n_obs)
        return;
    const WT* __restrict__ W = ctl->w_which ? W1 : W0;
    const double* __restrict__ H_E = H_E0 + small_sel(ctl, alt_off);
    const double* __restrict__ g_E = g_E0 + small_sel(ctl, alt_off);
    const int e = own[i], f = other[i];
    const double* se = scale + 6 * (int64_t)(e_off_pose + e);
    const double* sf = scale + 6 * (int64_t)(f_off_pose + f);
    double L[36];
    {
        const double* d2 = D2 + 6 * (int64_t)(e_off_pose + e);
#pragma unroll
        for (int a = 0; a < 6; ++a) {
#pragma unroll
            for (int b = 0; b < 6; ++b)
                L[6 * a + b] = se[a] * H_E[36 * (int64_t)e + 6 * a + b] * se[b];
            L[6 * a + a] += d2[a];
        }
    }
    const bool ok = chol6(L);
    const bool first = i == 0 || own[i - 1] != e;
    if (first) {
        if (!ok)
            ctl->lin_fail = 1;
        double v[6];
#pragma unroll
        for (int a = 0; a < 6; ++a)
            v[a] = se[a] * g_E[6 * (int64_t)e + a];
        forward_substitute<6>(L, RowMajor<6>{}, [&](const int r) { return v[r]; }, [&](const int r, const double t) { v[r] = t; });
#pragma unroll
        for (int k = 0; k < 36; ++k)
            Le[36 * (int64_t)e + k] = L[k];
#pragma unroll
        for (int k = 0; k < 6; ++k) {
            ze[6 * (int64_t)e + k] = v[k];
            if (!SPARSE)
                Z[(int64_t)(6 * e + k) * ldz + zcol] = v[k];
        }
    }
    double X[36];
#pragma unroll
    for (int a = 0; a < 6; ++a)
#pragma unroll
        for (int b = 0; b < 6; ++b)
            X[6 * a + b] = se[a] * (double)W[(int64_t)(6 * a + b) * n_pad + i] * sf[b];
    forward_block<6, 6>(L, RowMajor<6>{}, X);
    int64_t rs = ldz;
    double* zrow = Z + (int64_t)(6 * e) * ldz + 6 * f;
    if (SPARSE) {
        double* zb = Z + 36 * i;
#pragma unroll
        for (int c = 0; c < 6; ++c)
#pragma unroll
            for (int r = 0; r < 6; ++r)
                zb[6 * c + r] = X[6 * r + c];
        return;
    }
#pragma unroll
    for (int r = 0; r < 6; ++r)
#pragma unroll
        for (int c = 0; c < 6; ++c)
            zrow[(int64_t)r * rs + c] = X[6 * r + c];
}


typedef double double4_t __attribute__((ext_vector_type(4)));

constexpr int kSyrkKT = kKT;
constexpr int kSyrkT = kST;
constexpr int kSyrkRow = 144;
constexpr int kSyrkTile = kSyrkT * kSyrkT;

struct SyrkPlanDev {
    int n_tiles, n_kt, n_wg;
    const int32_t* tile_bi;
    const int32_t* tile_bj;
    const int64_t* wg_u0;
    const int64_t* wg_u1;
    const int32_t* wg_seg0;
    const int32_t* tile_seg0;
    double* partials;
};

__global__ __launch_bounds__(256, 2) void k_syrk_streamk(const LmCtl* ctl, const double* __restrict__ Z, int ldz,
                                                         SyrkPlanDev pl)
{
    if (ctl && ctl->done)
        return;
    __shared__ __attribute__((aligned(16))) double As[2][kSyrkKT * kSyrkRow];
    __shared__ __attribute__((aligned(16))) double Bs[2][kSyrkKT * kSyrkRow];
    const int g = blockIdx.x;
    int64_t u = pl.wg_u0[g];
    const int64_t u_end = pl.wg_u1[g];
    int seg = pl.wg_seg0[g];
    const int tid = threadIdx.x;
    const int lane = tid & 63, wave = tid >> 6;
    const int wi = wave >> 1, wj = wave & 1;
    const int lr = tid >> 5;
    const int lc = (tid & 31) * 4;
    const int fk = lane >> 4, fi = lane & 15;
    while (u < u_end) {
        const int t = (int)(u / pl.n_kt);
        const int kt0 = (int)(u % pl.n_kt);
        const int64_t left = u_end - u;
        const int kt1 = (kt0 + left < pl.n_kt) ? (int)(kt0 + left) : pl.n_kt;
        const int I0 = pl.tile_bi[t] * kSyrkT, J0 = pl.tile_bj[t] * kSyrkT;
        const bool diag = I0 == J0;
        double4_t acc[4][4];
#pragma unroll
        for (int a = 0; a < 4; ++a)
#pragma unroll
            for (int b = 0; b < 4; ++b)
                acc[a][b] = (double4_t){ 0.0, 0.0, 0.0, 0.0 };
        double4_t va[2], vb[2];
        auto gload = [&](int kt) {
#pragma unroll
            for (int h = 0; h < 2; ++h) {
                const double* zr = Z + (int64_t)(kt * kSyrkKT + lr + 8 * h) * ldz;
                va[h] = *reinterpret_cast<const double4_t*>(zr + I0 + lc);
                vb[h] = *reinterpret_cast<const double4_t*>(zr + J0 + lc);
            }
        };
        auto lstore = [&](int buf) {
#pragma unroll
            for (int h = 0; h < 2; ++h) {
                *reinterpret_cast<double4_t*>(&As[buf][(lr + 8 * h) * kSyrkRow + lc]) = va[h];
                *reinterpret_cast<double4_t*>(&Bs[buf][(lr + 8 * h) * kSyrkRow + lc]) = vb[h];
            }
        };
        gload(kt0);
        __syncthreads();
        lstore(0);
        __syncthreads();
        const bool live = !(diag && wi == 0 && wj == 1);
        for (int kt = kt0; kt < kt1; ++kt) {
            const int buf = (kt - kt0) & 1;
            if (kt + 1 < kt1)
                gload(kt + 1);
            const double* Ap = As[buf];
            const double* Bp = Bs[buf];
            if (live) {
#pragma unroll
                for (int ks = 0; ks < kSyrkKT / 4; ++ks) {
                    const int row = (ks * 4 + fk) * kSyrkRow;
                    double a[4], b[4];
#pragma unroll
                    for (int i = 0; i < 4; ++i) {
                        a[i] = Ap[row + wi * 64 + 16 * i + fi];
                        b[i] = Bp[row + wj * 64 + 16 * i + fi];
                    }
#pragma unroll
                    for (int i = 0; i < 4; ++i)
#pragma unroll
                        for (int j = 0; j < 4; ++j)
                            acc[i][j] = __builtin_amdgcn_mfma_f64_16x16x4f64(a[i], b[j], acc[i][j], 0, 0, 0);
                }
            }
            if (kt + 1 < kt1)
                lstore(buf ^ 1);
            __syncthreads();
        }
        double* Cb = pl.partials + (size_t)seg * kSyrkTile;
        if (live) {
#pragma unroll
            for (int a = 0; a < 4; ++a)
#pragma unroll
                for (int b = 0; b < 4; ++b)
#pragma unroll
                    for (int r = 0; r < 4; ++r)
                        Cb[(wi * 64 + a * 16 + fk + 4 * r) * kSyrkT + wj * 64 + b * 16 + fi] = acc[a][b][r];
        }
        u += kt1 - kt0;
        ++seg;
    }
}

constexpr int kWideRows = 2 * kSyrkKT;
constexpr int kWideStage = kWideRows * kSyrkRow;

template <bool DIAG, int W>
struct WideTiles {
    static constexpr int NT = DIAG ? 9 : 16, NA = DIAG ? 2 : 4, NB = DIAG ? 8 - W : 4;
    static __device__ __host__ constexpr int arow(int i) { return DIAG ? (i == 0 ? W : 7 - W) : 4 * (W >> 1) + i; }
    static __device__ __host__ constexpr int bcol(int j) { return DIAG ? j : 4 * (W & 1) + j; }
    static __device__ __host__ constexpr int ai(int n) { return DIAG ? (n <= W ? 0 : 1) : (n >> 2); }
    static __device__ __host__ constexpr int bi(int n) { return DIAG ? (n <= W ? n : n - (W + 1)) : (n & 3); }
};

template <bool DIAG, int W>
__device__ __forceinline__ void syrk_wide_item(const double* __restrict__ Z, const int ldz, const int I0, const int J0,
                                               const int kt0, const int kt1, double* smem, double* __restrict__ Cb)
{
    using T = WideTiles<DIAG, W>;
    const int tid = threadIdx.x;
    const int lane = tid & 63;
    const int g = tid >> 8;
    const int t = tid & 255;
    const int lr = t >> 5;
    const int lc = (t & 31) * 4;
// ... 286 lines not shown
            double2 v[NI];
#pragma unroll
            for (int u = 0; u < NI; ++u) {
                const int i = tid + kPairThreads * u;
                const int k = min(i / 18, hi - lo - 1);
                ie[u] = a.f2e[fs + lo + k];
            }
#pragma unroll
            for (int u = 0; u < NI; ++u) {
                const int i = tid + kPairThreads * u;
                v[u] = *reinterpret_cast<const double2*>(Zc + 36 * (int64_t)ie[u] + 2 * (i % 18));
            }
#pragma unroll
            for (int u = 0; u < NI; ++u) {
                const int i = tid + kPairThreads * u;
                if (i < (hi - lo) * 18)
                    *reinterpret_cast<double2*>(&As[kPairBlk * (i / 18) + 2 * (i % 18)]) = v[u];
            }
        }
        __syncthreads();
#ifndef VMM_PAIR_TB
#define VMM_PAIR_TB 4
#endif
        constexpr int TB = VMM_PAIR_TB;
        int2 tt[TB];
        if (active && t < t1) {
#pragma unroll
            for (int u = 0; u < TB; ++u)
                tt[u] = terms[min(t + u * kPairSplit, t1 - 1)];
        }
        while (active && t < t1) {
            double b[TB][6];
            bool ok[TB];
#pragma unroll
            for (int u = 0; u < TB; ++u) {
                ok[u] = t + u * kPairSplit < t1 && tt[u].x < hi;
                if (rhs) {
#pragma unroll
                    for (int r = 0; r < 6; ++r)
                        b[u][r] = a.ze[6 * (int64_t)tt[u].y + r];
                } else {
                    const double2* __restrict__ bp = reinterpret_cast<const double2*>(Zc + 36 * (int64_t)tt[u].y + 6 * c);
#pragma unroll
                    for (int r = 0; r < 3; ++r) {
                        const double2 v2 = bp[r];
                        b[u][2 * r] = v2.x;
                        b[u][2 * r + 1] = v2.y;
                    }
                }
            }
            int2 tn[TB];
#pragma unroll
            for (int u = 0; u < TB; ++u)
                tn[u] = terms[min(t + (TB + u) * kPairSplit, t1 - 1)];
            int n_ok = 0;
#pragma unroll
            for (int u = 0; u < TB; ++u) {
                if (ok[u]) {
                    const double* __restrict__ Ap = As + kPairBlk * (tt[u].x - lo);
#pragma unroll
                    for (int r = 0; r < 6; ++r)
#pragma unroll
                        for (int q = 0; q < 6; ++q)
                            acc[q] = fma(Ap[6 * q + r], b[u][r], acc[q]);
                    ++n_ok;
                }
            }
            t += n_ok * kPairSplit;
            if (n_ok < TB)
                break;
#pragma unroll
            for (int u = 0; u < TB; ++u)
                tt[u] = tn[u];
        }
    }
#pragma unroll
    for (int m = 1; m < kPairSplit; m <<= 1)
#pragma unroll
        for (int q = 0; q < 6; ++q)
            acc[q] += __shfl_xor(acc[q], m, 64);
    if (!active || sl != 0)
        return;
    if (a.add_diag && a.ctl) {
        a.da.H_F += small_sel(a.ctl, a.da.alt_off);
        a.da.g_F += small_sel(a.ctl, a.da.alt_off);
    }
    if (rhs) {
#pragma unroll
        for (int q = 0; q < 6; ++q) {
            const int par = 6 * f + q;
            a.S[(int64_t)n_pad * ld + rbase + q] = (a.add_diag ? a.da.scale_F[par] * a.da.g_F[par] : 0.0) - acc[q];
        }
        return;
    }
    const bool diag_pair = cbase == rbase;
#pragma unroll
    for (int q = 0; q < 6; ++q) {
        const int par = 6 * f + q;
        double v = -acc[q];
        if (a.add_diag && diag_pair) {
            v += a.da.scale_F[par] * a.da.H_F[36 * (int64_t)f + 6 * q + c] * a.da.scale_F[6 * f + c];
            if (q == c)
                v += a.da.D2_F[par];
        }
        a.S[(int64_t)(rbase + q) * ld + cbase + c] = v;
    }
}

__global__ __launch_bounds__(256) void k_fill_lower(const LmCtl* ctl, double* __restrict__ S, int ld, int n_pad, int unit_diag)
{
    if (ctl && ctl->done)
        return;
    const int row = blockIdx.x;
    const int c1 = row == n_pad ? n_pad : (row / 64) * 64 + 64;
    double2* __restrict__ dst = reinterpret_cast<double2*>(S + (int64_t)row * ld);
    for (int j = threadIdx.x; 2 * j < c1; j += 256) {
        double2 v = make_double2(0.0, 0.0);
        if (unit_diag && row < n_pad) {
            if (2 * j == row)
                v.x = 1.0;
            if (2 * j + 1 == row)
                v.y = 1.0;
        }
        dst[j] = v;
    }
}


static SyrkPlanDev plan_dev(const SyrkPlan& p)
{
    SyrkPlanDev d;
    d.n_tiles = p.n_tiles;
    d.n_kt = p.n_kt;
    d.n_wg = p.n_wg;
    d.tile_bi = p.tile_bi;
    d.tile_bj = p.tile_bj;
    d.wg_u0 = p.wg_u0;
    d.wg_u1 = p.wg_u1;
    d.wg_seg0 = p.wg_seg0;
    d.tile_seg0 = p.tile_seg0;
    d.partials = p.partials;
    return d;
}

void launch_elim(Engine& e)
{
    const int e_off = e.elim_cams ? 0 : e.n_cams;
    const int f_off = e.elim_cams ? e.n_cams : 0;
    const double* H_E = e.elim_cams ? e.H_cam : e.H_tag;
    const double* g_E = e.elim_cams ? e.g_cam : e.g_tag;
    if (e.ordE.n > 0) {
        const dim3 grid((unsigned)((e.ordE.n + 255) / 256));
        double* const Zout = e.sparse_schur ? e.Zc : e.Z;
#define VMM_FORM_Z(WT, SP, W0, W1)                                                                                      \
    hipLaunchKernelGGL((k_form_z<WT, SP>), grid, dim3(256), 0, e.stream, e.ctl, e.ordE.n, e.ordE.n_pad, e.ordE.own,      \
                       e.ordE.other, (const WT*)(W0), (const WT*)(W1), H_E, g_E, e.small_alt_off, (const double*)e.D2,   \
                       e.Le, e.ze, e.scale, e_off, f_off, Zout, e.ldz, e.n_pad, (const int32_t*)e.ordE.start)
        if (e.f32_accum) {
            if (e.sparse_schur)
                VMM_FORM_Z(float, true, e.Wf, e.Wf2);
            else
                VMM_FORM_Z(float, false, e.Wf, e.Wf2);
        } else {
            if (e.sparse_schur)
                VMM_FORM_Z(double, true, e.W, e.W2);
            else
                VMM_FORM_Z(double, false, e.W, e.W2);
        }
#undef VMM_FORM_Z
    }
}

void launch_syrk_plan(hipStream_t st, const LmCtl* ctl, const double* Z, int ldz, const SyrkPlan& p)
{
    if (p.n_wg > 0 && p.wide)
        hipLaunchKernelGGL(k_syrk_wide, dim3(p.n_wg), dim3(512), 0, st, ctl, Z, ldz, plan_dev(p));
    else if (p.n_wg > 0)
        hipLaunchKernelGGL(k_syrk_streamk, dim3(p.n_wg), dim3(256), 0, st, ctl, Z, ldz, plan_dev(p));
}

void launch_reduce_plan(hipStream_t st, const LmCtl* ctl, const SyrkPlan& p, int ld, int n_rows, double* S)
{
    DiagArgs da = {};
    if (p.n_tiles > 0)
        hipLaunchKernelGGL((k_reduce_partials<false>), dim3(16 * p.n_tiles), dim3(256), 0, st, ctl, plan_dev(p), ld, n_rows,
                           S, da);
}

void launch_schur_rows(Engine& e, bool add_diag)
{
    if (e.n_row_items <= 0)
        return;
    const int f_off = e.elim_cams ? e.n_cams : 0;
    PairArgs a;
    a.ctl = e.ctl;
    a.item_row = e.row_items;
    a.item_p0 = e.row_items + e.n_row_items;
    a.pair_start = e.pair_start;
    a.tstart = e.pair_tstart;
    a.terms = reinterpret_cast<const int2*>(e.pair_terms);
    a.f_start = e.ordF.start;
    a.f2e = e.f2e;
    a.Zc = e.Zc;
    a.ze = e.ze;
    a.S = e.S;
    a.ld = e.ldz;
    a.n_items = e.n_row_items;
    a.n_f = e.n_f;
    a.da.H_F = e.elim_cams ? e.H_tag : e.H_cam;
    a.da.g_F = e.elim_cams ? e.g_tag : e.g_cam;
    a.da.scale_F = e.scale + 6 * (size_t)f_off;
    a.da.D2_F = e.D2 + 6 * (size_t)f_off;
    a.da.n_red = e.n_red;
    a.da.n_pad = e.n_pad;
    a.da.alt_off = e.small_alt_off;
    a.add_diag = add_diag ? 1 : 0;
    a.pair_col = e.explicit_pairs ? e.pair_col : nullptr;
    a.row_of = e.explicit_pairs ? e.row_of : nullptr;
    if (e.explicit_pairs)
        hipLaunchKernelGGL(k_fill_lower, dim3(e.n_pad + 1), dim3(256), 0, e.stream, (const LmCtl*)e.ctl, e.S, e.ldz, e.n_pad,
                           add_diag ? 1 : 0);
    const int n_fill = e.explicit_pairs ? 0 : std::min(64, e.n_pad + 1);
    hipLaunchKernelGGL(k_schur_pairs, dim3(e.n_row_items + n_fill), dim3(kPairThreads), 0, e.stream, a);
}

void launch_syrk_only(Engine& e)
{
    if (e.sparse_schur)
        launch_schur_rows(e, !e.multi);
    else
        launch_syrk_plan(e.stream, e.ctl, e.Z, e.ldz, e.syrk);
}

void launch_syrk_reduced(Engine& e)
{
    launch_syrk_only(e);
    if (e.sparse_schur)
        return;
    if (e.multi) {
        DiagArgs none = {};
        if (e.syrk.n_tiles > 0)
            hipLaunchKernelGGL((k_reduce_partials<false>), dim3(16 * e.syrk.n_tiles), dim3(256), 0, e.stream, e.ctl,
                               plan_dev(e.syrk), e.ldz, e.n_pad + 1, e.S, none, e.S_packed);
        return;
    }
    const int f_off = e.elim_cams ? e.n_cams : 0;
    DiagArgs da;
    da.H_F = e.elim_cams ? e.H_tag : e.H_cam;
    da.g_F = e.elim_cams ? e.g_tag : e.g_cam;
    da.scale_F = e.scale + 6 * (size_t)f_off;
    da.D2_F = e.D2 + 6 * (size_t)f_off;
    da.n_red = e.n_red;
    da.n_pad = e.n_pad;
    da.alt_off = e.small_alt_off;
    hipLaunchKernelGGL((k_reduce_partials<true>), dim3(16 * e.syrk.n_tiles), dim3(256), 0, e.stream, e.ctl,
                       plan_dev(e.syrk), e.ldz, e.n_pad + 1, e.S, da);
}

__global__ __launch_bounds__(256) void k_pack_lower(const LmCtl* ctl, const double* __restrict__ S, int ld, int n_rows,
                                                    double* __restrict__ packed, bool unpack, double* __restrict__ Sout)
{
    if (ctl && ctl->done)
        return;
    const int r = blockIdx.x;
    if (r >= n_rows)
        return;
    const int64_t base = (int64_t)r * (r + 1) / 2;
    for (int c = threadIdx.x; c <= r; c += 256) {
        if (unpack)
            Sout[(int64_t)r * ld + c] = packed[base + c];
        else
            packed[base + c] = S[(int64_t)r * ld + c];
    }
}

__global__ __launch_bounds__(256) void k_unpack_diag(const LmCtl* ctl, const double* __restrict__ packed, int ld,
                                                     int f_off_pose, const double* __restrict__ H_F,
                                                     const double* __restrict__ g_F, const double* __restrict__ scale,
                                                     const double* __restrict__ D2, double* __restrict__ S, int n_red,
                                                     int n_pad, const int32_t* __restrict__ pose_of_row,
                                                     const int32_t* __restrict__ row_of)
{
    if (ctl && ctl->done)
        return;
    const int r = blockIdx.x;
    const int64_t base = (int64_t)r * (r + 1) / 2;
    const double* sF = scale + 6 * (int64_t)f_off_pose;
    const double* dF = D2 + 6 * (int64_t)f_off_pose;
    if (pose_of_row) {
        const int fr = r < n_pad ? pose_of_row[r] : -1;
        for (int c = threadIdx.x; c <= r; c += 256) {
            double v = packed[base + c];
            const int fc = c < n_pad ? pose_of_row[c] : -1;
            if (r == n_pad) {
                if (fc >= 0) {
                    const int k = 6 * fc + (c - row_of[fc]);
                    v += sF[k] * g_F[k];
                }
            } else if (fr >= 0) {
                if (fc == fr) {
                    const int a = r - row_of[fr], b = c - row_of[fr];
                    double add = sF[6 * fr + a] * H_F[36 * (int64_t)fr + 6 * a + b] * sF[6 * fr + b];
                    if (c == r)
                        add += dF[6 * fr + a];
                    v += add;
                }
            } else if (c == r) {
                v = 1.0;
            }
            S[(int64_t)r * ld + c] = v;
        }
        return;
    }
    for (int c = threadIdx.x; c <= r; c += 256) {
        double v = packed[base + c];
        if (r == n_pad) {
            if (c < n_red)
                v += sF[c] * g_F[c];
        } else if (r < n_red) {
            if (c / 6 == r / 6) {
                double add = sF[r] * H_F[36 * (int64_t)(r / 6) + 6 * (r % 6) + c % 6] * sF[c];
                if (c == r)
                    add += dF[r];
                v += add;
            }
        } else if (c == r) {
            v = 1.0;
        }
        S[(int64_t)r * ld + c] = v;
    }
}

void launch_pack_lower(Engine& e, bool unpack)
{
    if (!e.multi)
        return;
    if (!unpack) {
        if (e.sparse_schur)
            hipLaunchKernelGGL(k_pack_lower, dim3(e.n_pad + 1), dim3(256), 0, e.stream, (const LmCtl*)e.ctl,
                               (const double*)e.S, e.ldz, e.n_pad + 1, e.S_packed, false, e.S);
        return;
    }
    const int f_off = e.elim_cams ? e.n_cams : 0;
    const double* H_F = e.elim_cams ? e.H_tag : e.H_cam;
    const double* g_F = e.elim_cams ? e.g_tag : e.g_cam;
    hipLaunchKernelGGL(k_unpack_diag, dim3(e.n_pad + 1), dim3(256), 0, e.stream, (const LmCtl*)e.ctl,
                       (const double*)e.S_packed, e.ldz, f_off, H_F, g_F, (const double*)e.scale, (const double*)e.D2,
                       e.S, e.n_red, e.n_pad, (const int32_t*)e.pose_of_row, (const int32_t*)e.row_of);
}


int preload_schur_kernels()
{
    hipFuncAttributes at;
    int bad = 0;
    bad += hipFuncGetAttributes(&at, reinterpret_cast<const void*>(&k_form_z<double, false>)) != hipSuccess;
    bad += hipFuncGetAttributes(&at, reinterpret_cast<const void*>(&k_form_z<float, false>)) != hipSuccess;
    bad += hipFuncGetAttributes(&at, reinterpret_cast<const void*>(&k_form_z<double, true>)) != hipSuccess;
    bad += hipFuncGetAttributes(&at, reinterpret_cast<const void*>(&k_form_z<float, true>)) != hipSuccess;
    bad += hipFuncGetAttributes(&at, reinterpret_cast<const void*>(&k_schur_pairs)) != hipSuccess;
    bad += hipFuncGetAttributes(&at, reinterpret_cast<const void*>(&k_fill_lower)) != hipSuccess;
    bad += hipFuncGetAttributes(&at, reinterpret_cast<const void*>(&k_syrk_streamk)) != hipSuccess;
    bad += hipFuncGetAttributes(&at, reinterpret_cast<const void*>(&k_syrk_wide)) != hipSuccess;
    bad += hipFuncGetAttributes(&at, reinterpret_cast<const void*>(&k_reduce_partials<true>)) != hipSuccess;
    bad += hipFuncGetAttributes(&at, reinterpret_cast<const void*>(&k_reduce_partials<false>)) != hipSuccess;
    bad += hipFuncGetAttributes(&at, reinterpret_cast<const void*>(&k_unpack_diag)) != hipSuccess;
    bad += hipFuncGetAttributes(&at, reinterpret_cast<const void*>(&k_pack_lower)) != hipSuccess;
    return bad;
}

}
```

### visual_marker_mapping_amd/csrc/plan.cpp

```cpp
#include "plan.hpp"

#include <math.h>
#include <stdio.h>
#include <stdlib.h>
#include <string.h>

#include <algorithm>
#include <utility>

namespace vmm {


Switches read_switches()
{
    auto env_is = [](const char* name, char c) {
        const char* v = getenv(name);
        return v && v[0] == c;
    };
    Switches s;
    s.debug = getenv("VMM_BA_DEBUG") != nullptr;
    s.force_collectives = env_is("VMM_BA_FORCE_COLLECTIVES", '1');
    s.no_preload = env_is("VMM_BA_NO_PRELOAD", '1');
    s.eager_first = env_is("VMM_BA_EAGER_FIRST", '1');
    s.rccl_graph = !env_is("VMM_BA_RCCL_GRAPH", '0');
    s.use_graph = !env_is("VMM_BA_NO_GRAPH", '1');
    if (const char* v = getenv("VMM_BA_GRAPH_PASSES"))
        s.graph_passes = std::min(std::max(atoi(v), 1), 8);
    s.no_chain = env_is("VMM_BA_NO_CHAIN", '1');
    s.no_dataflow = env_is("VMM_BA_NO_DATAFLOW", '1');
    if (const char* v = getenv("VMM_BA_DEBUG_CAPTURE_FAIL"))
        if (v[0])
            s.capture_fail_rank = atoi(v);
    if (const char* sl = getenv("VMM_BA_DEBUG_SPIN_LIMIT")) {
        const unsigned lim = (unsigned)std::max(1L, atol(sl));
        const char* sk = getenv("VMM_BA_DEBUG_SPIN_KERNEL");
        const std::string which = sk ? sk : "both";
        if (which == "df" || which == "both")
            s.spin_df = lim;
        if (which == "chain" || which == "both")
            s.spin_chain = lim;
        s.spin_once = env_is("VMM_BA_DEBUG_SPIN_ONCE", '1');
        const char* sw = getenv("VMM_BA_DEBUG_SPIN_WG");
        s.spin_wg = sw ? atoi(sw) : -1;
    }
    if (const char* v = getenv("VMM_BA_EVAL"))
        s.eval_fused = !strcmp(v, "fused");
    if (const char* v = getenv("VMM_BA_FUSED_GROUP"))
        s.fused_group = std::min(64, std::max(1, atoi(v)));
    if (const char* v = getenv("VMM_BA_SCHUR"))
        s.schur = !strcmp(v, "dense") ? 1 : !strcmp(v, "sparse") ? 2 : 0;
    if (const char* v = getenv("VMM_BA_ORDER")) {
        s.order_nd = !strcmp(v, "nd");
        s.order_natural = !strcmp(v, "natural");
    }
    if (const char* v = getenv("VMM_BA_ND_LEAF"))
        s.nd_leaf = std::max(1, atoi(v));
    if (const char* v = getenv("VMM_BA_TREE_MAX_WG"))
        s.tree_max_wg = atoi(v);
    if (const char* v = getenv("VMM_BA_TREE_MODEL"))
        s.tree_model_r3 = !strcmp(v, "r3");
    if (const char* v = getenv("VMM_BA_PAIRS"))
        s.pairs = !strcmp(v, "explicit") ? 1 : 0;
    if (const char* v = getenv("VMM_BA_SYRK_WG_PER_CU"))
        s.syrk_wg_per_cu = std::max(1, atoi(v));
    if (const char* v = getenv("VMM_BA_SYRK_SLICES"))
        s.syrk_slices = std::max(1, atoi(v));
    s.syrk_no_xcd = env_is("VMM_BA_SYRK_NO_XCD", '1');
    s.syrk_wide = !env_is("VMM_BA_SYRK_WIDE", '0');
    if (const char* v = getenv("VMM_BA_DF_MAX_WG"))
        s.df_max_wg = atoi(v);
    if (const char* v = getenv("VMM_BA_CHOL_TAIL"))
        s.chol_tail = atoi(v);
    if (const char* v = getenv("VMM_BA_DF_BULK"))
        s.df_bulk = atoi(v) > 0;
    if (const char* v = getenv("VMM_BA_DF_HELP"))
        s.df_help = v[0] == '1';
    return s;
}

static void tag_to_points(const double* qt, const double* wh, double* pts)
{
    const double w = qt[0], x = qt[1], y = qt[2], z = qt[3];
    const double R[9] = { 1.0 - 2.0 * (y * y + z * z), 2.0 * (x * y - w * z), 2.0 * (x * z + w * y),
                          2.0 * (x * y + w * z), 1.0 - 2.0 * (x * x + z * z), 2.0 * (y * z - w * x),
                          2.0 * (x * z - w * y), 2.0 * (y * z + w * x), 1.0 - 2.0 * (x * x + y * y) };
    static const double sx[4] = { -1.0, 1.0, 1.0, -1.0 }, sy[4] = { -1.0, -1.0, 1.0, 1.0 };
    for (int k = 0; k < 4; ++k) {
        const double lx = sx[k] * wh[0] / 2.0, ly = sy[k] * wh[1] / 2.0;
        for (int a = 0; a < 3; ++a)
            pts[3 * k + a] = (R[3 * a] * lx + R[3 * a + 1] * ly) + qt[4 + a];
    }
}

std::vector<double> pairs_from_tags(const double* tag_qt, const double* tag_wh, int n_tags)
{
    std::vector<double> pairs((size_t)14 * n_tags, 0.0);
    for (int t = 0; t < n_tags; ++t) {
        double pts[12];
        tag_to_points(tag_qt + 7 * (size_t)t, tag_wh + 2 * (size_t)t, pts);
        for (int k = 0; k < 6; ++k) {
            pairs[(size_t)14 * t + k] = pts[k];
            pairs[(size_t)14 * t + 7 + k] = pts[6 + k];
        }
    }
    return pairs;
}

void expand_points(const vmm_ba_problem& user, PointProblem& x)
{
    const vmm_ba_problem* p = &user;
    x.tag_qt = pairs_from_tags(p->tag_qt, p->tag_wh, p->n_tags);
    x.tag_wh.assign((size_t)4 * p->n_tags, 0.0);
    x.cam.resize((size_t)2 * p->n_obs);
    x.tag.resize((size_t)2 * p->n_obs);
    x.px.assign((size_t)16 * p->n_obs, 0.0);
    for (int64_t i = 0; i < p->n_obs; ++i)
        for (int h2 = 0; h2 < 2; ++h2) {
            x.cam[(size_t)2 * i + h2] = p->obs_cam[i];
            x.tag[(size_t)2 * i + h2] = 2 * p->obs_tag[i] + h2;
            for (int k = 0; k < 4; ++k)
                x.px[(size_t)8 * (2 * i + h2) + k] = p->obs_px[8 * i + 4 * h2 + k];
        }
    x.problem = user;
    x.problem.n_tags = 2 * p->n_tags;
    x.problem.tag_qt = x.tag_qt.data();
    x.problem.tag_wh = x.tag_wh.data();
    x.problem.n_obs = 2 * p->n_obs;
    x.problem.obs_cam = x.cam.data();
    x.problem.obs_tag = x.tag.data();
    x.problem.obs_px = x.px.data();
}


OrderPlan plan_order(int n_own, const int32_t* own_idx, const int32_t* other_idx, const double* px, int64_t n)
{
    OrderPlan o;
    std::vector<int64_t> start((size_t)n_own + 1, 0);
    for (int64_t i = 0; i < n; ++i)
        start[own_idx[i] + 1]++;
    for (int p = 0; p < n_own; ++p)
        start[p + 1] += start[p];
    std::vector<int64_t> pos(start.begin(), start.end() - 1);
    o.n = n;
    o.n_pad = std::max<int64_t>(64, round_up(n, 64));
    o.own.resize((size_t)n);
    o.other.resize((size_t)n);
    o.caller.resize((size_t)n);
    o.px.assign((size_t)8 * o.n_pad, 0.0);
    for (int64_t i = 0; i < n; ++i) {
        const int64_t d = pos[own_idx[i]]++;
        o.own[d] = own_idx[i];
        o.other[d] = other_idx[i];
        o.caller[d] = (int32_t)i;
        for (int k = 0; k < 8; ++k)
            o.px[(size_t)k * o.n_pad + d] = px[8 * i + k];
    }
    o.pose_task.assign((size_t)n_own + 1, 0);
    for (int p = 0; p < n_own; ++p) {
        o.pose_task[p] = (int32_t)o.tasks.size();
        for (int64_t b = start[p]; b < start[p + 1]; b += kWave) {
            Task t;
            t.pose = p;
            t.begin = (int32_t)b;
            t.end = (int32_t)std::min<int64_t>(b + kWave, start[p + 1]);
            o.tasks.push_back(t);
        }
    }
    o.pose_task[n_own] = (int32_t)o.tasks.size();
    o.start.assign(start.begin(), start.end());
    return o;
}

SyrkSchedule plan_syrk(int n_row_blk, int n_col_blk, int k_pad, int n_cu, const Switches& sw)
{
    SyrkSchedule p;
    std::vector<int32_t>& bi = p.tile_bi;
    std::vector<int32_t>& bj = p.tile_bj;
    for (int r = 0; r < n_row_blk; ++r)
        for (int c = 0; c <= std::min(r, n_col_blk - 1); ++c) {
            bi.push_back(r);
            bj.push_back(c);
        }
    p.n_tiles = (int)bi.size();
    p.n_kt = k_pad / kKT;
    const int hw = n_cu > 0 ? n_cu : 256;
    const int per_cu = sw.syrk_wg_per_cu > 0 ? sw.syrk_wg_per_cu : 2;
    const int64_t slots = per_cu * (int64_t)hw;
    const bool xcd_rounds = !sw.syrk_no_xcd;
    const int n_xcd = 8;
    std::vector<int64_t>& wg_u0 = p.wg_u0;
    std::vector<int64_t>& wg_u1 = p.wg_u1;
    std::vector<int32_t>& wg_seg0 = p.wg_seg0;
    std::vector<int32_t>& tile_seg0 = p.tile_seg0;
    tile_seg0.assign((size_t)p.n_tiles + 1, 0);
    int seg = 0;
    if (xcd_rounds && (int64_t)p.n_tiles * n_xcd <= slots && p.n_kt >= n_xcd) {
        std::vector<int> order;
        for (int t = 0; t < p.n_tiles; ++t)
            if (bi[t] != bj[t])
                order.push_back(t);
        for (int t = 0; t < p.n_tiles; ++t)
            if (bi[t] == bj[t])
                order.push_back(t);
        std::vector<int32_t> bi2(bi.size()), bj2(bj.size());
        for (int t = 0; t < p.n_tiles; ++t) {
            bi2[t] = bi[order[t]];
            bj2[t] = bj[order[t]];
        }
        bi.swap(bi2);
        bj.swap(bj2);
        if (sw.syrk_wide && !sw.syrk_slices && !sw.syrk_wg_per_cu) {
            int n_diag = 0;
            for (int t = 0; t < p.n_tiles; ++t)
                n_diag += bi[t] == bj[t];
            const int n_off = p.n_tiles - n_diag;
            const double kDiagCost = 9.0 / 16.0;
            const int max_w = std::max(1, p.n_kt / 2);
            int w_off = (int)std::floor(hw / (n_off + kDiagCost * n_diag));
            w_off = std::max(1, std::min(w_off, max_w));
            int w_diag = std::max(1, std::min((int)std::lround(kDiagCost * w_off), max_w));
            while (w_off > 1 && (int64_t)w_off * n_off + (int64_t)w_diag * n_diag > hw) {
                --w_off;
                w_diag = std::max(1, std::min((int)std::lround(kDiagCost * w_off), max_w));
            }
            std::vector<int> w_of((size_t)p.n_tiles);
            int n_items = 0;
            for (int t = 0; t < p.n_tiles; ++t) {
                w_of[t] = bi[t] == bj[t] ? w_diag : w_off;
                tile_seg0[t] = n_items;
                n_items += w_of[t];
            }
            tile_seg0[p.n_tiles] = n_items;
            std::vector<std::pair<int, int>> items;
            for (int sl = 0; sl < std::max(w_off, w_diag); ++sl)
                for (int t = 0; t < p.n_tiles; ++t)
                    if (sl < w_of[t])
                        items.emplace_back(t, sl);
            const int per_x = (n_items + n_xcd - 1) / n_xcd;
            p.n_wg = per_x * n_xcd;
            p.wide = true;
            wg_u0.assign((size_t)p.n_wg, 0);
            wg_u1.assign((size_t)p.n_wg, 0);
            wg_seg0.assign((size_t)p.n_wg, 0);
            for (int b = 0; b < p.n_wg; ++b) {
                const int x = b % n_xcd, j = b / n_xcd;
                const int it = x * per_x + j;
                if (j >= per_x || it >= n_items)
                    continue;
                const int t = items[(size_t)it].first, sl = items[(size_t)it].second;
                wg_u0[b] = (int64_t)t * p.n_kt + (int64_t)p.n_kt * sl / w_of[t];
                wg_u1[b] = (int64_t)t * p.n_kt + (int64_t)p.n_kt * (sl + 1) / w_of[t];
                wg_seg0[b] = tile_seg0[t] + sl;
            }
            seg = n_items;
        } else {
        int n_sl = (int)std::min<int64_t>(slots / p.n_tiles, p.n_kt);
        if (sw.syrk_slices)
            n_sl = std::max(1, std::min(sw.syrk_slices, p.n_kt));
        const int n_items = p.n_tiles * n_sl;
        const int per_x = (n_items + n_xcd - 1) / n_xcd;
        p.n_wg = per_x * n_xcd;
        wg_u0.assign((size_t)p.n_wg, 0);
        wg_u1.assign((size_t)p.n_wg, 0);
        wg_seg0.assign((size_t)p.n_wg, 0);
        for (int b = 0; b < p.n_wg; ++b) {
            const int x = b % n_xcd, j = b / n_xcd;
            const int it = x * per_x + j;
            if (j >= per_x || it >= n_items)
                continue;
            const int sl = it / p.n_tiles, t = it % p.n_tiles;
            wg_u0[b] = (int64_t)t * p.n_kt + (int64_t)p.n_kt * sl / n_sl;
            wg_u1[b] = (int64_t)t * p.n_kt + (int64_t)p.n_kt * (sl + 1) / n_sl;
            wg_seg0[b] = n_sl * t + sl;
        }
        for (int t = 0; t <= p.n_tiles; ++t)
            tile_seg0[t] = n_sl * t;
        seg = n_sl * p.n_tiles;
        }
    } else {
    const int64_t full_rounds = (xcd_rounds && slots % n_xcd == 0) ? p.n_tiles / slots : 0;
    const int64_t tiles_a = full_rounds * slots;
    const int64_t units_b = (int64_t)(p.n_tiles - tiles_a) * p.n_kt;
    int64_t n_wg_b = std::min<int64_t>(units_b, slots);
    if (full_rounds == 0 && units_b > 64 * slots)
        n_wg_b = 4 * slots;
    const int64_t upw_b = n_wg_b > 0 ? (units_b + n_wg_b - 1) / n_wg_b : 0;
    n_wg_b = upw_b > 0 ? (units_b + upw_b - 1) / upw_b : 0;
    p.n_wg = (int)(tiles_a + n_wg_b);
    std::vector<int64_t> lu0((size_t)p.n_wg + 1, 0);
    for (int64_t l = 0; l < tiles_a; ++l)
        lu0[(size_t)l] = l * p.n_kt;
    for (int64_t l = 0; l <= n_wg_b; ++l)
        lu0[(size_t)(tiles_a + l)] = std::min<int64_t>(tiles_a * p.n_kt + l * upw_b, (int64_t)p.n_tiles * p.n_kt);
    std::vector<int32_t> lseg0((size_t)p.n_wg + 1, 0);
    for (int l = 0; l < p.n_wg; ++l) {
        lseg0[l] = seg;
        int64_t u = lu0[l];
        const int64_t u_end = lu0[l + 1];
        while (u < u_end) {
            const int t = (int)(u / p.n_kt);
            const int kt0 = (int)(u % p.n_kt);
            const int64_t take = std::min<int64_t>(p.n_kt - kt0, u_end - u);
            if (kt0 == 0)
                tile_seg0[t] = seg;
            u += take;
            ++seg;
        }
    }
    tile_seg0[p.n_tiles] = seg;
    wg_u0.resize((size_t)p.n_wg);
    wg_u1.resize((size_t)p.n_wg);
    wg_seg0.resize((size_t)p.n_wg);
    for (int b = 0; b < p.n_wg; ++b) {
        int64_t l = b;
        if (b < tiles_a) {
            const int64_t r = b / slots, o = b % slots;
            l = r * slots + (o % n_xcd) * (slots / n_xcd) + o / n_xcd;
        }
        wg_u0[b] = lu0[(size_t)l];
        wg_u1[b] = lu0[(size_t)l + 1];
        wg_seg0[b] = lseg0[(size_t)l];
    }
    }
// ... 194 lines not shown
    P.pair_obs.swap(pair);
    P.fused_e_list.swap(e_list);
    P.fused_e_part0.swap(part0);
    P.fused_pose_task.swap(ptask);
}

Plan make_plan(const vmm_ba_problem& p, const vmm_ba_create_options& co, bool elim_cams, bool multi, int world,
               bool points, const Switches& sw)
{
    Plan P;
    P.n_e = elim_cams ? p.n_cams : p.n_tags;
    P.n_f = elim_cams ? p.n_tags : p.n_cams;
    const int n_e = P.n_e, n_f = P.n_f;
    const int64_t n_obs = p.n_obs;

    const int32_t* own_e = elim_cams ? p.obs_cam : p.obs_tag;
    const int32_t* own_f = elim_cams ? p.obs_tag : p.obs_cam;
    P.ordE = plan_order(n_e, own_e, own_f, p.obs_px, n_obs);
    P.ordF = plan_order(n_f, own_f, own_e, p.obs_px, n_obs);
    const std::vector<int32_t>& startE = P.ordE.start;
    const std::vector<int32_t>& otherE = P.ordE.other;
    const std::vector<int32_t>& callerE = P.ordE.caller;
    const std::vector<int32_t>& startF = P.ordF.start;
    const std::vector<int32_t>& callerF = P.ordF.caller;

    plan_fused_eval(P, n_obs, sw);

    P.n_red = 6 * n_f;
    P.n_pad = round_up(P.n_red, kNB);
    P.n_blk = P.n_pad / kNB;
    P.ldz = round_up(P.n_pad + 1, kST) + 32;
    P.k_dim = 6 * n_e;
    P.k_pad = round_up(P.k_dim, kKT);
    std::vector<int32_t> gStartV, gOtherV;
    const bool have_structure = co.n_structure_obs > 0 && co.structure_obs_cam && co.structure_obs_tag;
    if (multi && have_structure) {
        gStartV.assign((size_t)n_e + 1, 0);
        for (int64_t d = 0; d < co.n_structure_obs; ++d) {
            const int32_t c = co.structure_obs_cam[d], t = co.structure_obs_tag[d];
            if (c < 0 || c >= p.n_cams || t < 0 || t >= p.n_tags) {
                P.error = "structure_obs index out of range";
                return P;
            }
            if (points) {
                P.error = "structure_obs is not supported with point landmarks";
                return P;
            }
            gStartV[(size_t)(elim_cams ? c : t) + 1]++;
        }
        for (int q = 0; q < n_e; ++q)
            gStartV[(size_t)q + 1] += gStartV[(size_t)q];
        gOtherV.resize((size_t)co.n_structure_obs);
        std::vector<int32_t> fillg(gStartV.begin(), gStartV.end() - 1);
        for (int64_t d = 0; d < co.n_structure_obs; ++d) {
            const int32_t c = co.structure_obs_cam[d], t = co.structure_obs_tag[d];
            gOtherV[(size_t)fillg[(size_t)(elim_cams ? c : t)]++] = elim_cams ? t : c;
        }
    }
    const bool global_lists = !gStartV.empty();
    const std::vector<int32_t>& gStart = global_lists ? gStartV : startE;
    const std::vector<int32_t>& gOther = global_lists ? gOtherV : otherE;
    const bool layout_free = !multi || world == 1 || global_lists;
    {
        double pairs = 0.0;
        P.co_terms = 0.0;
        for (int q = 0; q < n_e; ++q) {
            const double deg = (double)(gStart[q + 1] - gStart[q]);
            pairs += 0.5 * deg * (deg + 1.0);
            P.co_terms += deg * deg;
        }
        const double dense_flops = (double)(P.n_pad + 1) * (P.n_pad + 2) * P.k_dim;
        const double n_obs_model = global_lists ? (double)co.n_structure_obs : (double)n_obs;
        const double sparse_flops = 432.0 * pairs + 72.0 * n_obs_model;
        const double dense_us = dense_flops / 44e6 + 12.0, sparse_us = sparse_flops / 9e6 + 18.0;
        const double plan_terms = pairs + n_obs_model;
        P.sparse_schur = n_obs_model > 0 && sparse_us < dense_us && plan_terms <= 4e7;
        if (sw.schur == 1)
            P.sparse_schur = false;
        else if (sw.schur == 2)
            P.sparse_schur = n_obs_model > 0;
        if (P.sparse_schur && plan_terms >= 2147483647.0) {
            P.error = "block-sparse elimination: more than 2^31 block products (set VMM_BA_SCHUR=dense)";
            return P;
        }
        P.schur_flops = P.sparse_schur ? sparse_flops : dense_flops;
    }
    std::vector<std::vector<int32_t>> tree_nbr;
    if (P.sparse_schur && layout_free && !sw.order_natural && n_f > 1 && P.n_blk >= 4 && P.co_terms <= 5e7) {
        std::vector<std::vector<int32_t>>& nbr = tree_nbr;
        nbr.assign((size_t)n_f, {});
        for (int q = 0; q < n_e; ++q)
            for (int32_t d1 = gStart[q]; d1 < gStart[q + 1]; ++d1)
                for (int32_t d2 = gStart[q]; d2 < gStart[q + 1]; ++d2)
                    if (d1 != d2)
                        nbr[(size_t)gOther[(size_t)d1]].push_back(gOther[(size_t)d2]);
        for (auto& v : nbr) {
            std::sort(v.begin(), v.end());
            v.erase(std::unique(v.begin(), v.end()), v.end());
        }
        std::vector<int32_t> all((size_t)n_f), stamp((size_t)n_f, 0);
        for (int fq = 0; fq < n_f; ++fq)
            all[(size_t)fq] = fq;
        int32_t stamp_next = 1;
        std::vector<std::vector<int32_t>> nodes;
        nd_dissect(nbr, all, sw.nd_leaf, 12, stamp, stamp_next, nodes);
        std::vector<int32_t> rows((size_t)n_f, -1);
        int row = 0;
        for (const auto& nd : nodes) {
            row = round_up(row, kNB);
            for (const int32_t v : nd) {
                rows[(size_t)v] = row;
                row += 6;
            }
        }
        const int n_pad_nd = round_up(row, kNB);
        const int nb = n_pad_nd / kNB;
        bool take = nodes.size() > 2 && nb <= kDfMaxBlk - 1;
        if (take) {
            const std::vector<BlkMask> nzr = symbolic_factor(nb, rows, nbr);
            int n_wg = nb;
            for (int i = 0; i < nb; ++i)
                for (int k = 0; k < i; ++k)
                    n_wg += nzr[(size_t)i].test(k) ? 1 : 0;
            n_wg += nb;
            int path_max = 1;
            const double t_tree = model_tree_factorisation(nb, nzr, nullptr, &path_max, sw.tree_model_r3);
            const double t_nat = P.n_blk <= 48 ? 9.8 * P.n_blk : 32.0 * P.n_blk;
            take = n_wg <= sw.tree_max_wg && (sw.order_nd || (path_max * 10 <= P.n_blk * 7 && t_tree <= 0.9 * t_nat));
            if (sw.debug)
                fprintf(stderr, "[vmm_ba debug] tree ordering candidate: longest chain %d of %d block columns against %d in "
                                "natural order, %d workgroups, modelled %.0f against %.0f us -> %s\n", path_max, nb, P.n_blk,
                        n_wg, t_tree, t_nat, take ? "taken" : "not taken");
        }
        if (take) {
            P.h_row_of = rows;
            int r2 = 0;
            for (const auto& nd : nodes) {
                r2 = round_up(r2, kNB);
                P.nd_node_first_blk.push_back(r2 / kNB);
                r2 += 6 * (int)nd.size();
            }
            P.n_pad = n_pad_nd;
            P.n_blk = P.n_pad / kNB;
            P.ldz = round_up(P.n_pad + 1, kST) + 32;
            if (sw.debug) {
                fprintf(stderr, "[vmm_ba debug] tree ordering: %zu nodes, %d rows (%d blocks) for %d kept poses; node sizes:",
                        nodes.size(), P.n_pad, P.n_blk, n_f);
                for (const auto& nd : nodes)
                    fprintf(stderr, " %zu", nd.size());
                fprintf(stderr, "\n");
            }
        }
    }
    if (!P.sparse_schur)
        return P;

    std::vector<int32_t> posE((size_t)n_obs), row_pos((size_t)n_obs);
    P.f2e.assign((size_t)n_obs, 0);
    for (int64_t d = 0; d < n_obs; ++d)
        posE[(size_t)callerE[(size_t)d]] = (int32_t)d;
    for (int fq = 0; fq < n_f; ++fq)
        for (int32_t d = startF[fq]; d < startF[fq + 1]; ++d) {
            P.f2e[(size_t)d] = posE[(size_t)callerF[(size_t)d]];
            row_pos[(size_t)P.f2e[(size_t)d]] = d - startF[fq];
        }
    const bool tree = !P.h_row_of.empty();
    std::vector<int32_t> rank_of((size_t)n_f);
    for (int fq = 0; fq < n_f; ++fq)
        rank_of[(size_t)fq] = tree ? P.h_row_of[(size_t)fq] : fq;
    std::vector<std::vector<int32_t>> partners;
    {
        double co_pairs = 0.0;
        std::vector<std::vector<int32_t>> adj((size_t)n_f);
        const bool list_pairs = tree || P.co_terms <= 5e7;
        for (int q = 0; q < n_e && list_pairs; ++q)
            for (int32_t d1 = startE[q]; d1 < startE[q + 1]; ++d1)
                for (int32_t d2 = startE[q]; d2 < startE[q + 1]; ++d2) {
                    const int f1 = otherE[(size_t)d1], f2 = otherE[(size_t)d2];
                    if (rank_of[(size_t)f2] < rank_of[(size_t)f1])
                        adj[(size_t)f1].push_back(f2);
                }
        for (int fq = 0; fq < n_f; ++fq) {
            std::vector<int32_t>& a = adj[(size_t)fq];
            std::sort(a.begin(), a.end(), [&](int32_t x, int32_t y) { return rank_of[(size_t)x] < rank_of[(size_t)y]; });
            a.erase(std::unique(a.begin(), a.end()), a.end());
            a.push_back(fq);
            co_pairs += (double)a.size();
        }
        const double all = 0.5 * (double)n_f * (n_f + 1.0);
        P.explicit_pairs = tree || (list_pairs && co_pairs < 0.5 * all);
        if (sw.pairs >= 0)
            P.explicit_pairs = tree || (list_pairs && sw.pairs == 1);
        if (P.explicit_pairs)
            partners.swap(adj);
    }
    std::vector<int32_t>& pstart = P.pair_start;
    pstart.assign((size_t)n_f + 1, 0);
    for (int fq = 0; fq < n_f; ++fq)
        pstart[(size_t)fq + 1] = pstart[(size_t)fq] + (P.explicit_pairs ? (int32_t)partners[(size_t)fq].size() + 1 : fq + 2);
    const size_t n_pairs = (size_t)pstart[(size_t)n_f];
    if (P.explicit_pairs) {
        P.pair_col.assign(n_pairs, -1);
        for (int fq = 0; fq < n_f; ++fq)
            for (size_t k = 0; k < partners[(size_t)fq].size(); ++k)
                P.pair_col[(size_t)pstart[(size_t)fq] + k] = tree ? P.h_row_of[(size_t)partners[(size_t)fq][k]]
                                                                   : 6 * partners[(size_t)fq][k];
    }
    auto pair_id = [&](int f1, int f2) -> int64_t {
        if (!P.explicit_pairs)
            return f2 <= f1 ? (int64_t)pstart[(size_t)f1] + f2 : -1;
        if (rank_of[(size_t)f2] > rank_of[(size_t)f1])
            return -1;
        const std::vector<int32_t>& a = partners[(size_t)f1];
        const auto it = std::lower_bound(a.begin(), a.end(), f2,
                                         [&](int32_t x, int32_t y) { return rank_of[(size_t)x] < rank_of[(size_t)y]; });
        return (int64_t)pstart[(size_t)f1] + (it - a.begin());
    };
    auto rhs_id = [&](int f1) -> int64_t { return (int64_t)pstart[(size_t)f1 + 1] - 1; };
    std::vector<int32_t>& tstart = P.pair_tstart;
    tstart.assign(n_pairs + 1, 0);
    for (int q = 0; q < n_e; ++q)
        for (int32_t d1 = startE[q]; d1 < startE[q + 1]; ++d1) {
            const int f1 = otherE[(size_t)d1];
            tstart[(size_t)rhs_id(f1) + 1]++;
            for (int32_t d2 = startE[q]; d2 < startE[q + 1]; ++d2) {
                const int64_t id = pair_id(f1, otherE[(size_t)d2]);
                if (id >= 0)
                    tstart[(size_t)id + 1]++;
            }
        }
    for (size_t k = 0; k < n_pairs; ++k)
        tstart[k + 1] += tstart[k];
    const size_t n_terms = (size_t)tstart[n_pairs];
    if (n_terms >= ((size_t)1 << 31)) {
        P.error = "block-sparse elimination: more than 2^31 block products (set VMM_BA_SCHUR=dense)";
        return P;
    }
    std::vector<int32_t> ta(n_terms), tb(n_terms), fill(tstart.begin(), tstart.end() - 1);
    for (int q = 0; q < n_e; ++q)
        for (int32_t d1 = startE[q]; d1 < startE[q + 1]; ++d1) {
            const int f1 = otherE[(size_t)d1];
            {
                const int32_t k = fill[(size_t)rhs_id(f1)]++;
                ta[(size_t)k] = row_pos[(size_t)d1];
                tb[(size_t)k] = q;
            }
            for (int32_t d2 = startE[q]; d2 < startE[q + 1]; ++d2) {
                const int64_t id = pair_id(f1, otherE[(size_t)d2]);
                if (id < 0)
                    continue;
                const int32_t k = fill[(size_t)id]++;
                ta[(size_t)k] = row_pos[(size_t)d1];
                tb[(size_t)k] = d2;
            }
        }
    for (size_t k = 0; k < n_pairs; ++k) {
        const int32_t t0 = tstart[k], t1 = tstart[k + 1];
        bool sorted = true;
        for (int32_t t = t0 + 1; t < t1 && sorted; ++t)
            sorted = ta[(size_t)t - 1] <= ta[(size_t)t];
        if (!sorted) {
            std::vector<std::pair<int32_t, int32_t>> tmp;
            for (int32_t t = t0; t < t1; ++t)
                tmp.emplace_back(ta[(size_t)t], tb[(size_t)t]);
            std::stable_sort(tmp.begin(), tmp.end(),
                             [](const std::pair<int32_t, int32_t>& x, const std::pair<int32_t, int32_t>& y) { return x.first < y.first; });
            for (int32_t t = t0; t < t1; ++t) {
                ta[(size_t)t] = tmp[(size_t)(t - t0)].first;
                tb[(size_t)t] = tmp[(size_t)(t - t0)].second;
            }
        }
    }
    P.pair_terms.assign(2 * std::max<size_t>(n_terms, 1), 0);
    for (size_t k = 0; k < n_terms; ++k) {
        P.pair_terms[2 * k] = ta[k];
        P.pair_terms[2 * k + 1] = tb[k];
    }
    std::vector<int32_t> item_row, item_p0;
    std::vector<int32_t> rows_by_len((size_t)n_f);
    for (int fq = 0; fq < n_f; ++fq)
        rows_by_len[(size_t)fq] = n_f - 1 - fq;
    if (P.explicit_pairs)
        std::stable_sort(rows_by_len.begin(), rows_by_len.end(), [&](int32_t x, int32_t y) {
            return pstart[(size_t)x + 1] - pstart[(size_t)x] > pstart[(size_t)y + 1] - pstart[(size_t)y];
        });
    for (const int32_t fq : rows_by_len)
        for (int j0 = 0; j0 < pstart[(size_t)fq + 1] - pstart[(size_t)fq]; j0 += kPairsPerItem) {
            item_row.push_back(fq);
            item_p0.push_back(pstart[(size_t)fq] + j0);
        }
    P.n_row_items = (int)item_row.size();
    P.row_items = item_row;
    P.row_items.insert(P.row_items.end(), item_p0.begin(), item_p0.end());
    if (tree) {
        const int nb = P.n_blk;
        const std::vector<BlkMask> nzr = symbolic_factor(nb, P.h_row_of, tree_nbr);
        P.chol_nz.assign((size_t)(nb + 1) * kDfMaskWords, 0);
        for (int i = 0; i <= nb; ++i)
            for (int w = 0; w < kDfMaskWords; ++w)
                P.chol_nz[(size_t)i * kDfMaskWords + w] = nzr[(size_t)i].w[w];
        {
            const double d = (double)kNB;
            double fl = 0.0;
            for (int j2 = 0; j2 < nb; ++j2) {
                int nbl = 0;
                for (int r = j2 + 1; r < nb; ++r)
// ... 51 lines not shown
```

### visual_marker_mapping_amd/csrc/plan.hpp

```cpp
#pragma once
#include <stdint.h>

#include <string>
#include <vector>

#include "../../include/vmm_ba.h"

namespace vmm {

constexpr int kWave = 64;
constexpr int kPart = 32;
constexpr int kNB = 64;
constexpr int kDfMaskWords = 4;
constexpr int kDfMaxBlk = 256;
constexpr int kKT = 16;
constexpr int kST = 128;

#ifndef VMM_PAIR_NS
#define VMM_PAIR_NS 2
#endif
#ifndef VMM_PAIR_THREADS
#define VMM_PAIR_THREADS 256
#endif
constexpr int kPairSplit = VMM_PAIR_NS;
constexpr int kPairThreads = VMM_PAIR_THREADS;
constexpr int kPairsPerItem = kPairThreads / (6 * kPairSplit);

inline int round_up(int64_t v, int m) { return (int)(((v + m - 1) / m) * m); }

struct Task {
    int32_t pose;
    int32_t begin;
    int32_t end;
};

struct Switches {
    bool debug = false;
    bool force_collectives = false;
    bool no_preload = false;
    bool eager_first = false;
    bool rccl_graph = true;
    bool use_graph = true;
    int graph_passes = 2;
    bool no_chain = false;
    bool no_dataflow = false;
    int capture_fail_rank = -1;
    uint32_t spin_df = 0, spin_chain = 0;
    bool spin_once = false;
    int spin_wg = -1;
    bool eval_fused = false;
    int fused_group = 0;
    int schur = 0;
    bool order_nd = false;
    bool order_natural = false;
    int nd_leaf = 42;
    int tree_max_wg = 16384;
    bool tree_model_r3 = false;
    int pairs = -1;
    int syrk_wg_per_cu = 0;
    int syrk_slices = 0;
    bool syrk_no_xcd = false;
    bool syrk_wide = true;
    int df_max_wg = 0;
    int chol_tail = -1;
    bool df_bulk = false;
    int df_help = -1;
};
Switches read_switches();

struct PointProblem {
    std::vector<double> tag_qt, tag_wh, px;
    std::vector<int32_t> cam, tag;
    vmm_ba_problem problem;
};
void expand_points(const vmm_ba_problem& user, PointProblem& x);
std::vector<double> pairs_from_tags(const double* tag_qt, const double* tag_wh, int n_tags);

struct OrderPlan {
    int64_t n = 0;
    int64_t n_pad = 0;
    std::vector<int32_t> own, other, caller;
    std::vector<double> px;
    std::vector<Task> tasks;
    std::vector<int32_t> pose_task;
    std::vector<int32_t> start;
};
OrderPlan plan_order(int n_own, const int32_t* own_idx, const int32_t* other_idx, const double* px, int64_t n);

struct SyrkSchedule {
    int n_tiles = 0, n_kt = 0, n_wg = 0, n_segments = 0;
    bool wide = false;
    std::vector<int32_t> tile_bi, tile_bj, wg_seg0, tile_seg0;
    std::vector<int64_t> wg_u0, wg_u1;
};
SyrkSchedule plan_syrk(int n_row_blk, int n_col_blk, int k_pad, int n_cu, const Switches& sw);

struct Plan {
    std::string error;
    int n_e = 0, n_f = 0;
    OrderPlan ordE, ordF;
    bool fused_eval = false;
    int fused_n_e_act = 0, fused_f_pad = 0, fused_chunks = 0, fused_group = 1, fused_groups = 0, fused_slots = 0;
    std::vector<int32_t> pair_obs, fused_e_list, fused_e_part0, fused_pose_task;
    int n_red = 0, n_pad = 0, n_blk = 0, ldz = 0, k_dim = 0, k_pad = 0;
    bool sparse_schur = false;
    double co_terms = 0.0, schur_flops = 0.0;
    std::vector<int32_t> h_row_of;
    std::vector<int32_t> nd_node_first_blk;
    std::vector<int32_t> f2e, pair_start, pair_tstart;
    std::vector<int32_t> pair_terms;
    std::vector<int32_t> row_items;
    int n_row_items = 0;
    bool explicit_pairs = false;
    std::vector<int32_t> pair_col, row_of, pose_of_row;
    std::vector<unsigned long long> chol_nz;
    std::vector<unsigned char> chol_order;
    std::vector<int32_t> df_wg, df_slot;
    int n_df_wg = 0;
    size_t df_tree_slots = 0;
    double chol_flops = 0.0;
};
Plan make_plan(const vmm_ba_problem& p, const vmm_ba_create_options& co, bool elim_cams, bool multi, int world,
               bool points, const Switches& sw);

}
```

### visual_marker_mapping_amd/csrc/vmm_ba.hip

```cpp
#include <dlfcn.h>
#include <math.h>
#include <rccl/rccl.h>
#include <stdio.h>
#include <stdlib.h>
#include <string.h>

#include <algorithm>
#include <chrono>
#include <cmath>
#include <string>
#include <functional>
#include <vector>

#include "host.hpp"

namespace vmm {

static thread_local std::string g_err;
void set_error(const std::string& s) { g_err = s; }

template <typename T>
static int upload(Engine& e, T* dst, const std::vector<T>& src)
{
    if (!src.empty())
// ... 441 lines not shown
}

static int recover_sync_timeout(Engine& e, const vmm_ba_options& o)
{
    LmCtl& c = *e.ctl_host;
    c.num_sync_timeouts++;
    c.sync_kernels |= c.sync_timeout;
    c.sync_timeout = 0;
    c.lin_fail = 0;
    c.done = 0;
    if (e.sw.spin_once)
        c.spin_limit_df = c.spin_limit_chain = 0;
    HIP_TRY(hipMemcpyAsync(e.ctl, e.ctl_host, sizeof(LmCtl), hipMemcpyHostToDevice, e.stream));
    Range r("vmm_ba sync time-out recovery");
    int rc;
    for (int seg = 1; seg < kNumSeg; ++seg) {
        if (seg == kNumSeg - 1 && !e.multi)
            break;
        enqueue_segment(e, o, seg, true);
        if (e.multi && (rc = allreduce_after(e, seg)))
            return rc;
    }
    HIP_TRY(hipGetLastError());
    return VMM_BA_OK;
}

int begin_lm_loop(Engine& e, const vmm_ba_options& o, int trace_capacity)
{
    init_ctl(e, *e.ctl_host, o, trace_capacity);
    launch_begin_loop(e, *e.ctl_host);
    HIP_TRY(hipGetLastError());
    if (e.dirty_cam || e.dirty_tag) {
        HIP_TRY(hipEventRecord(e.pose_ev, e.stream));
        e.pose_ev_pending = true;
        e.dirty_cam = e.dirty_tag = false;
    }
    return VMM_BA_OK;
}

int flush_state(Engine& e)
{
    if (!e.dirty_cam && !e.dirty_tag)
        return VMM_BA_OK;
    if (e.dirty_cam)
        HIP_TRY(hipMemcpyAsync(e.cam_qt, e.pose_stage, sizeof(double) * 7 * e.n_cams, hipMemcpyHostToDevice, e.stream));
    if (e.dirty_tag)
        HIP_TRY(hipMemcpyAsync(e.tag_qt, e.pose_stage + (size_t)7 * e.n_cams, sizeof(double) * 7 * e.n_tags,
                               hipMemcpyHostToDevice, e.stream));
    HIP_TRY(hipEventRecord(e.pose_ev, e.stream));
    e.pose_ev_pending = true;
    e.dirty_cam = e.dirty_tag = false;
    return VMM_BA_OK;
}

void init_ctl(Engine& e, LmCtl& c, const vmm_ba_options& o, int trace_capacity)
{
    memset(&c, 0, sizeof(c));
    c.spin_limit_df = e.sw.spin_df;
    c.spin_limit_chain = e.sw.spin_chain;
    c.spin_wg = e.sw.spin_wg;
    c.max_num_iterations = o.max_num_iterations;
    c.robustify = o.robustify;
    c.jacobi_scaling = o.jacobi_scaling;
    c.max_invalid = o.max_num_consecutive_invalid_steps;
    c.huber_a = o.huber_a;
    c.function_tolerance = o.function_tolerance;
    c.gradient_tolerance = o.gradient_tolerance;
    c.parameter_tolerance = o.parameter_tolerance;
    c.max_radius = o.max_trust_region_radius;
    c.min_radius = o.min_trust_region_radius;
    c.min_relative_decrease = o.min_relative_decrease;
    c.min_lm_diagonal = o.min_lm_diagonal;
    c.max_lm_diagonal = o.max_lm_diagonal;
    c.radius = o.initial_trust_region_radius;
    c.decrease_factor = 2.0;
    c.first_eval = 1;
    c.termination = VMM_BA_NO_CONVERGENCE;
    c.trace_capacity = trace_capacity;
}


static int validate_problem(const vmm_ba_problem* p, const vmm_ba_create_options& co)
{
    if (p->n_cams <= 0 || p->n_tags <= 0 || p->n_obs < 0 || !p->cam_qt || !p->tag_qt || !p->tag_wh
        || (p->n_obs > 0 && (!p->obs_cam || !p->obs_tag || !p->obs_px))) {
        set_error("problem needs >= 1 camera, >= 1 tag and non-null arrays");
        return VMM_BA_ERR_ARGUMENT;
    }
    if (p->n_obs >= (int64_t)1 << 31) {
        set_error("n_obs must fit in 31 bits");
        return VMM_BA_ERR_ARGUMENT;
    }
    for (int64_t i = 0; i < p->n_obs; ++i)
        if (p->obs_cam[i] < 0 || p->obs_cam[i] >= p->n_cams || p->obs_tag[i] < 0 || p->obs_tag[i] >= p->n_tags) {
            set_error("observation " + std::to_string(i) + " references a camera or tag index out of range");
            return VMM_BA_ERR_ARGUMENT;
        }
    if (p->fixed_tag >= p->n_tags) {
        set_error("fixed_tag out of range");
        return VMM_BA_ERR_ARGUMENT;
    }
    if (co.landmarks != VMM_BA_LANDMARK_TAG_POSES && co.landmarks != VMM_BA_LANDMARK_POINTS) {
        set_error("create_options.landmarks must be VMM_BA_LANDMARK_TAG_POSES or VMM_BA_LANDMARK_POINTS");
        return VMM_BA_ERR_ARGUMENT;
    }
    if (co.landmarks == VMM_BA_LANDMARK_POINTS && co.precision != VMM_BA_PRECISION_F64) {
        set_error("point landmarks run in f64 only");
        return VMM_BA_ERR_ARGUMENT;
    }
    if (co.landmarks == VMM_BA_LANDMARK_POINTS && (p->n_obs >= (int64_t)1 << 30 || p->n_tags >= 1 << 30)) {
        set_error("problem too large for point landmarks");
        return VMM_BA_ERR_ARGUMENT;
    }
    if (co.precision != VMM_BA_PRECISION_F64 && co.precision != VMM_BA_PRECISION_F32_ACCUM) {
        set_error("create_options.precision must be VMM_BA_PRECISION_F64 or VMM_BA_PRECISION_F32_ACCUM");
        return VMM_BA_ERR_ARGUMENT;
    }
    if (co.world_size < 1 || co.rank < 0 || co.rank >= co.world_size) {
        set_error("bad rank / world_size");
        return VMM_BA_ERR_ARGUMENT;
    }
    return VMM_BA_OK;
}

static int open_device(Engine& e, int device)
{
    e.device = device;
    if (hipSetDevice(e.device) != hipSuccess || hipStreamCreateWithFlags(&e.stream, hipStreamNonBlocking) != hipSuccess) {
        set_error("hipSetDevice / hipStreamCreate failed");
        e.stream = nullptr;
        return VMM_BA_ERR_HIP;
    }
    hipDeviceProp_t prop;
    if (hipGetDeviceProperties(&prop, e.device) == hipSuccess && prop.multiProcessorCount > 0)
        e.n_cu = prop.multiProcessorCount;
    static bool preloaded[64] = {};
    if (e.device < 64 && !preloaded[e.device] && !e.sw.no_preload) {
        const int bad = preload_eval_kernels() + preload_schur_kernels() + preload_chol_kernels() + preload_lm_kernels()
            + preload_cov_kernels() + preload_init_kernels() + preload_border_kernels();
        if (bad) {
            set_error("hipFuncGetAttributes failed for " + std::to_string(bad) + " kernels (code object not loadable on this device)");
            return VMM_BA_ERR_HIP;
        }
        preloaded[e.device] = true;
    }
    return VMM_BA_OK;
}

static void take_plan(Engine& e, const Plan& P)
{
    e.n_e = P.n_e;
    e.n_f = P.n_f;
    e.fused_eval = P.fused_eval;
    e.fused_n_e_act = P.fused_n_e_act;
    e.fused_f_pad = P.fused_f_pad;
    e.fused_chunks = P.fused_chunks;
    e.fused_group = P.fused_group;
    e.fused_groups = P.fused_groups;
    e.n_red = P.n_red;
    e.n_pad = P.n_pad;
    e.n_blk = P.n_blk;
    e.ldz = P.ldz;
    e.k_dim = P.k_dim;
    e.k_pad = P.k_pad;
    e.sparse_schur = P.sparse_schur;
    e.co_terms = P.co_terms;
    e.schur_flops = P.schur_flops;
    e.h_row_of = P.h_row_of;
    e.nd_node_first_blk = P.nd_node_first_blk;
    e.explicit_pairs = P.explicit_pairs;
    e.n_row_items = P.n_row_items;
    e.chol_flops = P.chol_flops;
    e.n_df_wg = P.n_df_wg;
    e.df_tree_slots = P.df_tree_slots;
    e.chol_nz_on = !P.chol_nz.empty();
}

static int upload_pose_const(Engine& e, const uint8_t* cam_const, const uint8_t* tag_const)
{
    std::vector<uint8_t> c((size_t)e.n_cams + (size_t)e.n_tags, 0);
    const int rep = e.points ? 2 : 1;
    if (cam_const)
        for (int i = 0; i < e.n_cams; ++i)
            c[(size_t)i] = cam_const[i] ? 1 : 0;
    for (int t = 0; t < e.n_tags; ++t)
        c[(size_t)e.n_cams + t] = ((tag_const && tag_const[t / rep]) || t / rep == e.fixed_tag) ? 1 : 0;
    if (c.empty())
        return VMM_BA_OK;
    HIP_TRY(hipMemcpyAsync(e.pose_const, c.data(), c.size(), hipMemcpyHostToDevice, e.stream));
    HIP_TRY(hipStreamSynchronize(e.stream));
    e.any_const = std::find(c.begin(), c.end(), (uint8_t)1) != c.end();
    return VMM_BA_OK;
}

static int allocate_and_upload(Engine& e, const Plan& P, const vmm_ba_problem& p)
{
    const int n_pose = e.n_cams + e.n_tags;
    int rc;
    if ((rc = dev_alloc(e, &e.cam_qt, (size_t)7 * e.n_cams))) return rc;
    if ((rc = dev_alloc(e, &e.tag_qt, (size_t)7 * e.n_tags))) return rc;
    if ((rc = dev_alloc(e, &e.cam_cand, (size_t)7 * e.n_cams))) return rc;
    if ((rc = dev_alloc(e, &e.tag_cand, (size_t)7 * e.n_tags))) return rc;
    if ((rc = dev_alloc(e, &e.tag_wh, (size_t)2 * e.n_tags))) return rc;
    if (hipMemcpyAsync(e.cam_qt, p.cam_qt, sizeof(double) * 7 * e.n_cams, hipMemcpyHostToDevice, e.stream) != hipSuccess
        || hipMemcpyAsync(e.tag_qt, p.tag_qt, sizeof(double) * 7 * e.n_tags, hipMemcpyHostToDevice, e.stream) != hipSuccess
        || hipMemcpyAsync(e.tag_wh, p.tag_wh, sizeof(double) * 2 * e.n_tags, hipMemcpyHostToDevice, e.stream) != hipSuccess
        || hipStreamSynchronize(e.stream) != hipSuccess) {
        set_error("pose upload failed");
        return VMM_BA_ERR_HIP;
    }
    if ((rc = upload_order(e, e.ordE, P.ordE))) return rc;
    if ((rc = upload_order(e, e.ordF, P.ordF))) return rc;
    if (e.fused_eval) {
        if ((rc = dev_alloc(e, &e.pair_obs, P.pair_obs.size()))) return rc;
        if ((rc = dev_alloc(e, &e.fused_e_list, P.fused_e_list.size()))) return rc;
        if ((rc = dev_alloc(e, &e.fused_e_part0, P.fused_e_part0.size()))) return rc;
        if ((rc = dev_alloc(e, &e.fused_pose_task, P.fused_pose_task.size()))) return rc;
        if ((rc = dev_alloc(e, &e.fused_partE, (size_t)std::max(P.fused_slots, 1) * kPart))) return rc;
        if ((rc = dev_alloc(e, &e.fused_partF, (size_t)e.fused_groups * 28 * e.fused_f_pad))) return rc;
        if ((rc = upload(e, e.pair_obs, P.pair_obs))) return rc;
        if ((rc = upload(e, e.fused_e_list, P.fused_e_list))) return rc;
        if ((rc = upload(e, e.fused_e_part0, P.fused_e_part0))) return rc;
        if ((rc = upload(e, e.fused_pose_task, P.fused_pose_task))) return rc;
    }

    e.small_count = (size_t)42 * n_pose + 2;
    if ((rc = dev_alloc(e, &e.small, e.small_count))) return rc;
    e.H_cam = e.small;
    e.H_tag = e.H_cam + (size_t)36 * e.n_cams;
    e.g_cam = e.H_tag + (size_t)36 * e.n_tags;
    e.g_tag = e.g_cam + (size_t)6 * e.n_cams;
    e.cost_slot = e.g_tag + (size_t)6 * e.n_tags;
    if ((rc = dev_alloc(e, &e.small_stage, e.small_count + (size_t)e.n_e))) return rc;
    e.ev_pose_cost = e.small_stage + e.small_count;
    e.small_alt_off = e.multi ? 0 : (int64_t)(e.small_stage - e.small);
    e.ev_H_cam = e.small_stage;
    e.ev_H_tag = e.ev_H_cam + (size_t)36 * e.n_cams;
    e.ev_g_cam = e.ev_H_tag + (size_t)36 * e.n_tags;
    e.ev_g_tag = e.ev_g_cam + (size_t)6 * e.n_cams;
    e.ev_cost = e.ev_g_tag + (size_t)6 * e.n_tags;
    if ((rc = dev_alloc(e, &e.obs_mask, (size_t)std::max<int64_t>(e.n_obs, 1), false))) return rc;
    if (hipMemsetAsync(e.obs_mask, 1, (size_t)std::max<int64_t>(e.n_obs, 1), e.stream) != hipSuccess) {
        set_error("hipMemsetAsync(obs_mask) failed");
        return VMM_BA_ERR_HIP;
    }
    if ((rc = dev_alloc(e, &e.pose_const, (size_t)n_pose))) return rc;
    if ((rc = upload_pose_const(e, nullptr, nullptr))) return rc;
    const size_t n_stat = (size_t)e.ordE.n_tasks + (size_t)e.ordF.n_tasks + 1;
    if ((rc = dev_alloc(e, &e.stats_part, n_stat))) return rc;
    if ((rc = dev_alloc(e, &e.stats_cnt, n_stat))) return rc;
    if ((rc = dev_alloc(e, &e.stats_pose, (size_t)2 * n_pose))) return rc;
    if (e.f32_accum) {
        if ((rc = dev_alloc(e, &e.Wf, (size_t)36 * e.ordE.n_pad))) return rc;
        if ((rc = dev_alloc(e, &e.Wf2, (size_t)36 * e.ordE.n_pad))) return rc;
    } else {
        if ((rc = dev_alloc(e, &e.W, (size_t)36 * e.ordE.n_pad))) return rc;
        if ((rc = dev_alloc(e, &e.W2, (size_t)36 * e.ordE.n_pad))) return rc;
    }
    if ((rc = dev_alloc(e, &e.scale, (size_t)6 * n_pose))) return rc;
    if ((rc = dev_alloc(e, &e.diag, (size_t)6 * n_pose))) return rc;
    if ((rc = dev_alloc(e, &e.D2, (size_t)6 * n_pose))) return rc;
    if ((rc = dev_alloc(e, &e.delta, (size_t)6 * n_pose))) return rc;
    if ((rc = dev_alloc(e, &e.active, (size_t)n_pose))) return rc;

    if ((rc = dev_alloc(e, &e.Le, (size_t)36 * e.n_e))) return rc;
    if ((rc = dev_alloc(e, &e.ze, (size_t)6 * e.n_e))) return rc;
    if (e.sparse_schur) {
        if ((rc = dev_alloc(e, &e.Zc, (size_t)36 * std::max<int64_t>(e.n_obs, 1)))) return rc;
        if ((rc = dev_alloc(e, &e.f2e, P.f2e.size()))) return rc;
        if ((rc = dev_alloc(e, &e.pair_start, P.pair_start.size()))) return rc;
        if ((rc = dev_alloc(e, &e.pair_tstart, P.pair_tstart.size()))) return rc;
        if ((rc = dev_alloc(e, &e.pair_terms, P.pair_terms.size()))) return rc;
        if ((rc = dev_alloc(e, &e.row_items, P.row_items.size()))) return rc;
        if ((rc = upload(e, e.f2e, P.f2e))) return rc;
        if ((rc = upload(e, e.pair_start, P.pair_start))) return rc;
        if ((rc = upload(e, e.pair_tstart, P.pair_tstart))) return rc;
        if ((rc = upload(e, e.pair_terms, P.pair_terms))) return rc;
        if ((rc = upload(e, e.row_items, P.row_items))) return rc;
        if (e.chol_nz_on) {
            if ((rc = dev_alloc(e, &e.chol_nz, P.chol_nz.size()))) return rc;
            if ((rc = upload(e, e.chol_nz, P.chol_nz))) return rc;
            if ((rc = dev_alloc(e, &e.chol_order, P.chol_order.size()))) return rc;
            if ((rc = upload(e, e.chol_order, P.chol_order))) return rc;
            if ((rc = dev_alloc(e, &e.df_wg, P.df_wg.size()))) return rc;
            if ((rc = upload(e, e.df_wg, P.df_wg))) return rc;
            if ((rc = dev_alloc(e, &e.df_slot, P.df_slot.size()))) return rc;
            if ((rc = upload(e, e.df_slot, P.df_slot))) return rc;
        }
        if (e.explicit_pairs) {
            if ((rc = dev_alloc(e, &e.pair_col, P.pair_col.size()))) return rc;
            if ((rc = dev_alloc(e, &e.row_of, P.row_of.size()))) return rc;
            if ((rc = upload(e, e.pair_col, P.pair_col))) return rc;
            if ((rc = upload(e, e.row_of, P.row_of))) return rc;
            if (!P.pose_of_row.empty()) {
                if ((rc = dev_alloc(e, &e.pose_of_row, P.pose_of_row.size()))) return rc;
                if ((rc = upload(e, e.pose_of_row, P.pose_of_row))) return rc;
            }
        }
    } else {
        if ((rc = ensure_dense_schur(e))) return rc;
    }
    if ((rc = dev_alloc(e, &e.S, (size_t)e.ldz * e.ldz))) return rc;
    if (e.multi && (rc = dev_alloc(e, &e.S_packed, (size_t)(e.n_pad + 1) * (e.n_pad + 2) / 2))) return rc;
    if ((rc = dev_alloc(e, &e.P, (size_t)4 * kNB * e.ldz))) return rc;
    if ((rc = setup_lookahead(e, e.n_blk, e.ldz))) return rc;
    if ((rc = dev_alloc(e, &e.dinv, (size_t)e.ldz))) return rc;
    if ((rc = dev_alloc(e, &e.Ldiag, (size_t)(e.n_blk + 1) * 4096))) return rc;
    if ((rc = dev_alloc(e, &e.Linv, (size_t)(e.n_blk + 1) * 4096))) return rc;
    if ((rc = dev_alloc(e, &e.flags, 264))) return rc;
    if ((rc = dev_alloc(e, &e.gran, (size_t)2 * e.ldz))) return rc;
    {
        const size_t nd = e.sw.no_dataflow ? 0 : (size_t)dataflow_blocks(e.n_blk, e.n_cu, e.sw);
        const size_t slots = std::max(nd * (nd + 1) / 2, e.sw.no_dataflow ? (size_t)0 : e.df_tree_slots);
        if (slots > 0 && (rc = dev_alloc(e, &e.df_gran, slots * 8 * 1024)))
            return rc;
        if (slots > 0 && (rc = dev_alloc(e, &e.df_compact, slots * 4096, false)))
            return rc;
        if (slots > 0 && (rc = dev_alloc(e, &e.df_done, slots)))
            return rc;
    }
    if ((rc = dev_alloc(e, &e.yf, (size_t)e.ldz))) return rc;
    if ((rc = dev_alloc(e, &e.step_comm, (size_t)7 * e.n_e + 1))) return rc;
    if ((rc = dev_alloc(e, &e.cost_comm, 2))) return rc;
    const size_t n_part = (size_t)std::max<int>(e.ordE.n_tasks, e.n_e) + 1;
    if ((rc = dev_alloc(e, &e.part_cost, n_part))) return rc;
    if ((rc = dev_alloc(e, &e.part_cross, n_part))) return rc;
    if ((rc = dev_alloc(e, &e.part_k1, n_part))) return rc;
    if ((rc = dev_alloc(e, &e.pose_part, (size_t)5 * n_pose))) return rc;
    if ((rc = dev_alloc(e, &e.pose_gm, (size_t)n_pose))) return rc;
    if ((rc = dev_alloc(e, &e.ctl, 1))) return rc;
    if (hipHostMalloc((void**)&e.ctl_host, sizeof(LmCtl)) != hipSuccess) {
        set_error("hipHostMalloc failed");
        e.ctl_host = nullptr;
        return VMM_BA_ERR_HIP;
    }
    memset(e.ctl_host, 0, sizeof(LmCtl));
    if (hipHostMalloc((void**)&e.pose_stage, sizeof(double) * 7 * (size_t)n_pose, hipHostMallocMapped) != hipSuccess
        || hipHostGetDevicePointer((void**)&e.pose_stage_dev, e.pose_stage, 0) != hipSuccess
        || hipEventCreateWithFlags(&e.pose_ev, hipEventDisableTiming) != hipSuccess) {
        set_error("hipHostMalloc / hipEventCreate (pose staging) failed");
        return VMM_BA_ERR_HIP;
    }
    e.trace_capacity = 0;
    if (hipStreamSynchronize(e.stream) != hipSuccess) {
        set_error("create: device synchronisation failed");
        return VMM_BA_ERR_HIP;
    }
    return VMM_BA_OK;
}
}

using namespace vmm;

extern "C" {

const char* vmm_ba_last_error(void) { return g_err.c_str(); }
int vmm_ba_abi_version(void) { return VMM_BA_ABI_VERSION; }

void vmm_ba_default_options(vmm_ba_options* o)
{
    memset(o, 0, sizeof(*o));
    o->max_num_iterations = 400;
    o->robustify = 1;
    o->huber_a = 1.0;
    o->function_tolerance = 1e-6;
    o->gradient_tolerance = 1e-10;
    o->parameter_tolerance = 1e-8;
    o->initial_trust_region_radius = 1e4;
    o->max_trust_region_radius = 1e16;
    o->min_trust_region_radius = 1e-32;
    o->min_relative_decrease = 1e-3;
    o->min_lm_diagonal = 1e-6;
    o->max_lm_diagonal = 1e32;
    o->max_num_consecutive_invalid_steps = 5;
    o->jacobi_scaling = 1;
    o->num_threads = 1;
// ... 480 lines not shown
```

### visual_marker_mapping_amd/engine.py

```python
import ctypes as C
import functools

import numpy as np

from . import _lib
from ._lib import (CONVERGENCE, ELIM_AUTO, ELIM_CAMERAS, ELIM_TAGS, FAILURE, LANDMARK_POINTS,
                   LANDMARK_TAG_POSES, NO_CONVERGENCE, PRECISION_F32_ACCUM, PRECISION_F64)


def _ptr(a):
    return None if a is None else a.ctypes.data_as(C.c_void_p)


@functools.lru_cache(maxsize=None)
def _fields(cls, skip=()):
    return tuple(k for k, _ in cls._fields_ if k != "reserved" and k not in skip)


def _set_fields(struct, kw, what, nested=None):
    names = _fields(type(struct), nested[1:] if nested else ())
    for k, v in kw.items():
        if k in names:
            setattr(struct, k, v)
        elif nested and k.startswith(nested[0]) and k[len(nested[0]):] in _fields(type(getattr(struct, nested[1]))):
# ... 103 lines not shown
            _lib.check(_lib.lib().vmm_ba_set_observation_mask(self._h, None))
            return
        m = np.ascontiguousarray(np.asarray(mask) != 0, np.uint8).reshape(-1)
        if len(m) != self.n_obs:
            raise ValueError("mask length differs from the number of observations")
        _lib.check(_lib.lib().vmm_ba_set_observation_mask(self._h, m.ctypes.data_as(C.c_void_p)))

    def set_constant_poses(self, cam_const=None, tag_const=None):
        flags = []
        for name, a, n in (("cam_const", cam_const, self.n_cams), ("tag_const", tag_const, self.n_tags)):
            if a is None:
                flags.append(None)
                continue
            a = np.asarray(a)
            if a.dtype != np.bool_ and not np.issubdtype(a.dtype, np.integer):
                raise TypeError("%s must be a boolean or integer array, not %s" % (name, a.dtype))
            if a.shape != (n,):
                raise ValueError("%s must have shape (%d,), not %s" % (name, n, a.shape))
            flags.append(np.ascontiguousarray(a != 0, np.uint8))
        _lib.check(_lib.lib().vmm_ba_set_constant_poses(self._h, _ptr(flags[0]), _ptr(flags[1])))
        self.constant_poses = tuple(None if f is None or not f.any() else f.tobytes() for f in flags)

    def get_state(self):
        cam, tag = np.zeros((self.n_cams, 7)), np.zeros((self.n_tags, 7))
        _lib.check(_lib.lib().vmm_ba_get_state(self._h, _ptr(cam), _ptr(tag)))
        return cam, tag

    def get_points(self):
        pts = np.zeros((self.n_tags, 4, 3))
        _lib.check(_lib.lib().vmm_ba_get_points(self._h, _ptr(pts)))
        return pts

    def set_allreduce(self, fn):
        def tramp(_user, buf, count, stream):
            try:
                fn(int(buf), int(count), int(stream or 0))
                return 0
            except Exception:
                import traceback
                traceback.print_exc()
                return 1
        self._allreduce_cb = _lib.ALLREDUCE_FN(tramp)
        _lib.check(_lib.lib().vmm_ba_set_allreduce(self._h, self._allreduce_cb, None))

    def enable_rccl(self, unique_id):
        buf = bytes(unique_id)
        if len(buf) != _lib.RCCL_ID_BYTES:
            raise ValueError("unique_id must be %d bytes" % _lib.RCCL_ID_BYTES)
        _lib.check(_lib.lib().vmm_ba_enable_rccl(self._h, C.c_char_p(buf)))

    def solve(self, options=None, trace_capacity=0, **kw):
        o = options or default_options(**kw)
        s, buf = _summary(trace_capacity)
        _lib.check(_lib.lib().vmm_ba_solve(self._h, C.byref(o), C.byref(s)))
        return _summary_dict(s, buf, trace_capacity)

    def initialize(self, **options):
        o = _options(_lib.InitOptions, "vmm_ba_default_init_options", options, "initialisation")
        r = _lib.InitReport()
        cam, tag = np.zeros(self.n_cams, np.uint8), np.zeros(self.n_tags, np.uint8)
        _lib.check(_lib.lib().vmm_ba_initialize(self._h, C.byref(o), C.byref(r), _ptr(cam), _ptr(tag)))
        return _struct_dict(r), cam.astype(bool), tag.astype(bool)

    def cost(self, robustify=True, huber_a=1.0):
        c = C.c_double(0)
        _lib.check(_lib.lib().vmm_ba_cost(self._h, int(bool(robustify)), float(huber_a), C.byref(c)))
        return c.value

    def reprojection_stats(self, per_corner=True):
        pc, pt = np.zeros(self.n_cams), np.zeros(self.n_tags)
        avg = C.c_double(0)
        corner = np.zeros((self.n_obs, 8)) if per_corner else None
        _lib.check(_lib.lib().vmm_ba_reprojection_stats(self._h, _ptr(pc), _ptr(pt), C.byref(avg), _ptr(corner)))
        return pc, pt, avg.value, corner

    def tag_translation_covariance(self, robustify=False, huber_a=1.0):
        cov = np.zeros((self.n_tags, 3, 3))
        _lib.check(_lib.lib().vmm_ba_tag_translation_covariance(self._h, int(bool(robustify)), float(huber_a),
                                                               _ptr(cov)))
        return cov

    def covariance_blocks(self, pairs, robustify=False, huber_a=1.0):
        pr = np.asarray(pairs, np.int64).reshape(-1, 2)
        if len(pr) and (pr.min() < -2 ** 31 or pr.max() >= 2 ** 31):
            raise ValueError("pose index out of the int32 range")
        a, b = np.ascontiguousarray(pr[:, 0], np.int32), np.ascontiguousarray(pr[:, 1], np.int32)
        cov = np.zeros((len(pr), 6, 6))
        _lib.check(_lib.lib().vmm_ba_covariance_blocks(self._h, int(bool(robustify)), float(huber_a), len(pr), _ptr(a),
                                                       _ptr(b), _ptr(cov)))
        return cov

    def pose_covariances(self, robustify=False, huber_a=1.0):
        idx = np.arange(self.n_cams + self.n_tags)
        cov = self.covariance_blocks(np.stack([idx, idx], axis=1), robustify, huber_a)
        return cov[:self.n_cams], cov[self.n_cams:]

    def tag_joint_covariance(self, robustify=False, huber_a=1.0):
        T = self.n_tags
        s, t = np.tril_indices(T)
        cov = self.covariance_blocks(np.stack([self.n_cams + s, self.n_cams + t], axis=1), robustify, huber_a)
        out = np.zeros((T, T, 6, 6))
        out[t, s] = np.swapaxes(cov, 1, 2)
        out[s, t] = cov
        return out

    def set_intrinsics(self, intr, dist):
        intr, dist = _model_arrays(intr, dist)
        _lib.check(_lib.lib().vmm_ba_set_intrinsics(self._h, _ptr(intr), _ptr(dist)))
        self.intr, self.dist = intr.copy(), dist.copy()

    def get_intrinsics(self):
        intr, dist = np.zeros(4), np.zeros(5)
        _lib.check(_lib.lib().vmm_ba_get_intrinsics(self._h, _ptr(intr), _ptr(dist)))
        return intr, dist

    def intrinsics_system(self, robustify=True, huber_a=1.0):
        c = C.c_double(0)
        gk, Ck, rk, Sk = np.zeros(9), np.zeros((9, 9)), np.zeros(9), np.zeros((9, 9))
        _lib.check(_lib.lib().vmm_ba_intrinsics_system(self._h, int(bool(robustify)), float(huber_a), C.byref(c),
                                                       _ptr(gk), _ptr(Ck), _ptr(rk), _ptr(Sk)))
        return {"cost": c.value, "g_k": gk, "C": Ck, "r_k": rk, "S_k": Sk}

    def solve_selfcal(self, options=None, trace_capacity=0, max_outer_iterations=None, refine_mask=None,
                      parameter_tolerance=None, function_tolerance=None, **kw):
        o = options or default_options(**kw)
        named = dict(max_outer_iterations=max_outer_iterations, refine_mask=refine_mask,
                     parameter_tolerance=parameter_tolerance, function_tolerance=function_tolerance)
        so = _options(_lib.SelfcalOptions, "vmm_ba_default_selfcal_options",
                      {k: v for k, v in named.items() if v is not None}, "self-calibration")
        (s, buf), r = _summary(trace_capacity), _lib.SelfcalReport()
        intr, dist, cov = np.zeros(4), np.zeros(5), np.zeros((9, 9))
        _lib.check(_lib.lib().vmm_ba_solve_selfcal(self._h, C.byref(o), C.byref(so), C.byref(s), C.byref(r), _ptr(intr),
                                                   _ptr(dist), _ptr(cov)))
        self.intr, self.dist = intr.copy(), dist.copy()
        return intr, dist, cov, _struct_dict(r), _summary_dict(s, buf, trace_capacity)

    def eval_blocks(self, robustify=True, huber_a=1.0, want_W=True):
        V, U = np.zeros((self.n_cams, 6, 6)), np.zeros((self.n_tags, 6, 6))
        W = np.zeros((self.n_obs, 6, 6)) if want_W else None
        gc, gt = np.zeros((self.n_cams, 6)), np.zeros((self.n_tags, 6))
        if self.landmarks == LANDMARK_POINTS:
            U = W = gt = None
        c = C.c_double(0)
        _lib.check(_lib.lib().vmm_ba_eval_blocks(self._h, int(bool(robustify)), float(huber_a), C.byref(c),
                                                 _ptr(V), _ptr(U), _ptr(W), _ptr(gc), _ptr(gt)))
        return {"cost": c.value, "V": V, "U": U, "W": W, "g_cam": gc, "g_tag": gt}

    def debug_overlap(self, reps=10):
        out = np.zeros(8)
        _lib.check(_lib.lib().vmm_ba_debug_overlap(self._h, int(reps), _ptr(out)))
        return dict(zip(("syrk_ms", "cholesky_ms", "sequential_ms", "concurrent_ms", "cholesky_in_concurrent_ms",
                         "syrk_in_concurrent_ms", "concurrent_syrk_first_ms", "cholesky_in_concurrent_syrk_first_ms"), out.tolist()))

    def time_kernels(self, options=None, reps=5):
        o = options or default_options()
        t = _lib.KernelTimes()
        _lib.check(_lib.lib().vmm_ba_time_kernels(self._h, C.byref(o), int(reps), C.byref(t)))
        return _struct_dict(t)


def joint_covariance(caa, cab, cbb):
    caa, cab, cbb = (np.asarray(m, np.float64).reshape(6, 6) for m in (caa, cab, cbb))
    return np.block([[caa, cab], [cab.T, cbb]])


def rccl_available():
    return bool(_lib.lib().vmm_ba_rccl_available())


def rccl_unique_id():
    buf = C.create_string_buffer(_lib.RCCL_ID_BYTES)
    _lib.check(_lib.lib().vmm_ba_rccl_unique_id(buf))
    return buf.raw


def project_points(intr, dist, points_cam, device=0):
    intr, dist = _model_arrays(intr, dist)
    pts = np.ascontiguousarray(points_cam, np.float64).reshape(-1, 3)
    uv = np.zeros((len(pts), 2))
    _lib.check(_lib.lib().vmm_ba_project_points(_ptr(intr), _ptr(dist), len(pts), _ptr(pts), _ptr(uv), device))
    return uv


def quad_poses(intr, dist, tag_wh, obs_px, device=0):
    intr, dist = _model_arrays(intr, dist)
    px = np.ascontiguousarray(obs_px, np.float64).reshape(-1, 8)
    wh = np.ascontiguousarray(tag_wh, np.float64).reshape(-1, 2)
    if len(wh) != len(px):
        raise ValueError("tag_wh and obs_px differ in length")
    qt2, rms2 = np.zeros((len(px), 2, 7)), np.zeros((len(px), 2))
    _lib.check(_lib.lib().vmm_ba_quad_poses(_ptr(intr), _ptr(dist), len(px), _ptr(wh), _ptr(px), _ptr(qt2), _ptr(rms2),
                                            device))
    return qt2, rms2


def default_localize_options(**kw):
    return _options(_lib.LocalizeOptions, "vmm_ba_default_localize_options", kw, "localisation")


assert _lib.LocalizeResult._fields_ == _lib.TriangulateResult._fields_


def _results(n):
    return np.zeros(n, np.dtype(_lib.LocalizeResult))


def _result_dicts(arr):
    return [dict(zip(arr.dtype.names, row)) for row in arr.tolist()]


def _map_batch_arrays(tag_qt, tag_wh, img_start, obs_tag, obs_px):
    tag_qt = np.ascontiguousarray(tag_qt, np.float64).reshape(-1, 7)
    tag_wh = np.ascontiguousarray(tag_wh, np.float64).reshape(-1, 2)
    img_start = np.ascontiguousarray(img_start, np.int64).reshape(-1)
    obs_tag = np.ascontiguousarray(obs_tag, np.int32).reshape(-1)
    obs_px = np.ascontiguousarray(obs_px, np.float64).reshape(-1, 8)
    if len(tag_wh) != len(tag_qt):
        raise ValueError("tag_wh and tag_qt differ in length")
    if len(obs_tag) != len(obs_px):
        raise ValueError("observation arrays differ in length")
    if len(img_start) < 1 or img_start[-1] != len(obs_tag):
        raise ValueError("img_start must have n_imgs + 1 entries and end at the number of observations")
    return tag_qt, tag_wh, img_start, obs_tag, obs_px


def localize(intr, dist, tag_qt, tag_wh, img_start, obs_tag, obs_px, device=0, **options):
    intr, dist = _model_arrays(intr, dist)
    tag_qt, tag_wh, img_start, obs_tag, obs_px = _map_batch_arrays(tag_qt, tag_wh, img_start, obs_tag, obs_px)
    o = default_localize_options(**options)
    n_imgs = len(img_start) - 1
    cam_qt, cam_cov = np.zeros((n_imgs, 7)), np.zeros((n_imgs, 6, 6))
    inl, res = np.zeros(len(obs_tag), np.uint8), _results(n_imgs)
    _lib.check(_lib.lib().vmm_ba_localize(_ptr(intr), _ptr(dist), len(tag_qt), _ptr(tag_qt), _ptr(tag_wh), n_imgs,
                                          _ptr(img_start), _ptr(obs_tag), _ptr(obs_px), C.byref(o), _ptr(cam_qt),
                                          _ptr(cam_cov), _ptr(inl), _ptr(res), device))
    return cam_qt, cam_cov, inl.astype(bool), _result_dicts(res)


def _rig_arrays(intr, dist, ext_qt, tag_qt, tag_wh, img_start, obs_tag, obs_px):
    intr, dist = _model_arrays(intr, dist, -1)
    ext_qt = np.ascontiguousarray(ext_qt, np.float64).reshape(-1, 7)
    if not len(intr) == len(dist) == len(ext_qt):
        raise ValueError("intr, dist and ext_qt must have one row per camera of the rig")
    tag_qt, tag_wh, img_start, obs_tag, obs_px = _map_batch_arrays(tag_qt, tag_wh, img_start, obs_tag, obs_px)
    n_rig_cams, n_slots = len(ext_qt), len(img_start) - 1
    if n_rig_cams < 1 or n_slots % n_rig_cams:
        raise ValueError("img_start must have n_frames * K + 1 entries for the K >= 1 cameras of the rig")
    return intr, dist, ext_qt, tag_qt, tag_wh, img_start, obs_tag, obs_px, n_rig_cams, n_slots // n_rig_cams


def rig_localize(intr, dist, ext_qt, tag_qt, tag_wh, img_start, obs_tag, obs_px, device=0, **options):
    intr, dist, ext_qt, tag_qt, tag_wh, img_start, obs_tag, obs_px, n_rig_cams, n_frames = _rig_arrays(
        intr, dist, ext_qt, tag_qt, tag_wh, img_start, obs_tag, obs_px)
    o = default_localize_options(**options)
    rig_qt, rig_cov = np.zeros((n_frames, 7)), np.zeros((n_frames, 6, 6))
    inl, res = np.zeros(len(obs_tag), np.uint8), _results(n_frames)
    _lib.check(_lib.lib().vmm_ba_rig_localize(n_rig_cams, _ptr(intr), _ptr(dist), _ptr(ext_qt), len(tag_qt), _ptr(tag_qt),
                                              _ptr(tag_wh), n_frames, _ptr(img_start), _ptr(obs_tag), _ptr(obs_px),
                                              C.byref(o), _ptr(rig_qt), _ptr(rig_cov), _ptr(inl), _ptr(res), device))
    return rig_qt, rig_cov, inl.astype(bool), _result_dicts(res)


def default_rig_calibrate_options(**kw):
    return _options(_lib.RigCalibrateOptions, "vmm_ba_default_rig_calibrate_options", kw, "rig calibration", ("loc_", "loc"))


def rig_calibrate(intr, dist, ext_qt0, tag_qt, tag_wh, img_start, obs_tag, obs_px, device=0, **options):
    intr, dist, ext_qt0, tag_qt, tag_wh, img_start, obs_tag, obs_px, n_rig_cams, n_frames = _rig_arrays(
        intr, dist, ext_qt0, tag_qt, tag_wh, img_start, obs_tag, obs_px)
    o = default_rig_calibrate_options(**options)
    ext_qt, ext_cov = np.zeros((n_rig_cams, 7)), np.zeros((6 * n_rig_cams, 6 * n_rig_cams))
    rig_qt, rig_cov = np.zeros((n_frames, 7)), np.zeros((n_frames, 6, 6))
    inl, res, rep = np.zeros(len(obs_tag), np.uint8), _results(n_frames), _lib.RigCalibrateReport()
    _lib.check(_lib.lib().vmm_ba_rig_calibrate(n_rig_cams, _ptr(intr), _ptr(dist), _ptr(ext_qt0), len(tag_qt), _ptr(tag_qt),
                                               _ptr(tag_wh), n_frames, _ptr(img_start), _ptr(obs_tag), _ptr(obs_px),
                                               C.byref(o), _ptr(ext_qt), _ptr(ext_cov), _ptr(rig_qt), _ptr(rig_cov),
                                               _ptr(inl), _ptr(res), C.byref(rep), device))
    return ext_qt, ext_cov, rig_qt, rig_cov, inl.astype(bool), _result_dicts(res), _struct_dict(rep)


def _pose_matrix(qt):
    w, x, y, z = qt[:4] / np.linalg.norm(qt[:4])
    R = np.array([[1 - 2 * (y * y + z * z), 2 * (x * y - w * z), 2 * (x * z + w * y)],
                  [2 * (x * y + w * z), 1 - 2 * (x * x + z * z), 2 * (y * z - w * x)],
                  [2 * (x * z - w * y), 2 * (y * z + w * x), 1 - 2 * (x * x + y * y)]])
    return R, np.asarray(qt[4:], np.float64)


def rig_extrinsics_start(n_rig_cams, n_frames, cam_qt, results):
    from .pnp import quat_from_R
    cam_qt = np.asarray(cam_qt, np.float64).reshape(n_frames * n_rig_cams, 7)
    if len(results) != n_frames * n_rig_cams:
        raise ValueError("results must have one entry per image, n_frames * K")
    ext_qt = np.zeros((n_rig_cams, 7))
    ext_qt[:, 0] = 1.0
    for c in range(1, n_rig_cams):
        best, best_f = -1, -1
        for f in range(n_frames):
            r0, rc = results[f * n_rig_cams], results[f * n_rig_cams + c]
            if r0["status"] != _lib.LOC_OK or rc["status"] != _lib.LOC_OK:
                continue
            n = r0["n_inlier_obs"] + rc["n_inlier_obs"]
            if n > best:
                best, best_f = n, f
        if best_f < 0:
            raise ValueError("camera %d of the rig shares no localised frame with camera 0: no starting extrinsic" % c)
# ... 217 lines not shown
```

Before: 2487 LM iterations/s.

## Fuse per-pose block sums into eval kernel and write whole Z lines

Adds a k_eval_sums kernel that packs each pose's evaluation tasks into one 8-wave workgroup and reduces the per-pose Hessian/gradient sums in LDS, replacing the separate eval and k_reduce_pose launches with their global partials buffer. The planner enables it only when padding overhead is small and fused_eval, multi-GPU and points are off. The dense Z formation kernel also gains a LINES variant that stores whole Z lines, and a debug elimination export is added. Risks include idle waves from padding slots and lower occupancy from the fixed 512-thread blocks.

```diff
diff --git a/__graft_entry__.py b/__graft_entry__.py
--- a/__graft_entry__.py
+++ b/__graft_entry__.py
@@ -13,6 +13,7 @@
     subprocess.check_call(["make", "-C", os.path.join(ROOT, "tools"), "all"])
     subprocess.check_call(["make", "-C", os.path.join(ROOT, "oracle"), "all"])
     subprocess.check_call(["make", "-C", os.path.join(ROOT, "tests", "cpp"), "all"])
+    subprocess.check_call(["make", "-C", os.path.join(ROOT, "tests", "cpp"), "-f", "pose_sums_test.mk", "pose_sums_test"])
     import visual_marker_mapping_amd
     from visual_marker_mapping_amd import _lib
     L = _lib.lib()
diff --git a/include/vmm_ba.h b/include/vmm_ba.h
--- a/include/vmm_ba.h
+++ b/include/vmm_ba.h
@@ -435,6 +435,8 @@
 
 int vmm_ba_debug_overlap(vmm_ba_handle h, int reps, double* ms);
 
+int vmm_ba_debug_elimination(vmm_ba_handle h, const vmm_ba_options* opt, int32_t* dims, double* Z, double* Le, double* ze);
+
 int vmm_ba_debug_chol_schedule(int n_blk, int n_df, int n_cu, int32_t* launches, int cap, int* n_launches, int* n_df_used);
 int vmm_ba_debug_chol_tile(int n_blk, const int32_t* launch, int t, int* bi, int* bj);
 
diff --git a/visual_marker_mapping_amd/_lib.py b/visual_marker_mapping_amd/_lib.py
--- a/visual_marker_mapping_amd/_lib.py
+++ b/visual_marker_mapping_amd/_lib.py
@@ -211,6 +211,7 @@
     "vmm_ba_dense_syrk": (_i, [_i, _i, _i, _a, _a]),
     "vmm_ba_pose_plus": (_i, [_i64, _a, _a, _a, _i]),
     "vmm_ba_debug_overlap": (_i, [_h, _i, _a]),
+    "vmm_ba_debug_elimination": (_i, [_h, _P(Options), _a, _a, _a, _a]),
     "vmm_ba_debug_chol_schedule": (_i, [_i, _i, _i, _a, _i, _a, _a]),
     "vmm_ba_debug_chol_tile": (_i, [_i, _a, _i, _a, _a]),
     "vmm_ba_time_kernels": (_i, [_h, _P(Options), _i, _P(KernelTimes)]),
@@ -221,7 +222,7 @@
             "vmm_ba_triangulate", "vmm_ba_locate_tags", "vmm_ba_default_predict_options", "vmm_ba_predict_localization",
             "vmm_ba_predict_localization_joint",
             "vmm_ba_set_intrinsics", "vmm_ba_get_intrinsics", "vmm_ba_intrinsics_system",
-            "vmm_ba_default_selfcal_options", "vmm_ba_solve_selfcal"}
+            "vmm_ba_default_selfcal_options", "vmm_ba_solve_selfcal", "vmm_ba_debug_elimination"}
 
 _LIB = None
 
diff --git a/visual_marker_mapping_amd/csrc/diagnostics.hip b/visual_marker_mapping_amd/csrc/diagnostics.hip
--- a/visual_marker_mapping_amd/csrc/diagnostics.hip
+++ b/visual_marker_mapping_amd/csrc/diagnostics.hip
@@ -296,4 +296,40 @@
     return VMM_BA_OK;
 }
 
-}
+int vmm_ba_debug_elimination(vmm_ba_handle h, const vmm_ba_options* opt, int32_t* dims, double* Z, double* Le, double* ze)
+{
+    if (!h || !opt || !dims) {
+        set_error("bad argument");
+        return VMM_BA_ERR_ARGUMENT;
+    }
+    Engine& e = *reinterpret_cast<Engine*>(h);
+    if (e.multi || e.sparse_schur || !e.Z) {
+        set_error("debug_elimination needs a single-GPU handle on the dense elimination path");
+        return VMM_BA_ERR_STATE;
+    }
+    dims[0] = e.k_pad;
+    dims[1] = e.ldz;
+    dims[2] = e.n_e;
+    if (!Z && !Le && !ze)
+        return VMM_BA_OK;
+    HIP_TRY(hipSetDevice(e.device));
+    int rc;
+    if ((rc = flush_state(e))) return rc;
+    if (e.trace_capacity < 1) {
+        if ((rc = dev_alloc(e, &e.trace, 1, false))) return rc;
+        e.trace_capacity = 1;
+        drop_graphs(e);
+    }
+    if ((rc = begin_lm_loop(e, *opt, 0))) return rc;
+    if ((rc = enqueue_iteration(e, *opt))) return rc;
+    HIP_TRY(hipStreamSynchronize(e.stream));
+    if (Z)
+        HIP_TRY(hipMemcpy(Z, e.Z, sizeof(double) * (size_t)e.k_pad * e.ldz, hipMemcpyDeviceToHost));
+    if (Le)
+        HIP_TRY(hipMemcpy(Le, e.Le, sizeof(double) * 36 * (size_t)e.n_e, hipMemcpyDeviceToHost));
+    if (ze)
+        HIP_TRY(hipMemcpy(ze, e.ze, sizeof(double) * 6 * (size_t)e.n_e, hipMemcpyDeviceToHost));
+    return VMM_BA_OK;
+}
+
+}
diff --git a/visual_marker_mapping_amd/csrc/engine.hpp b/visual_marker_mapping_amd/csrc/engine.hpp
--- a/visual_marker_mapping_amd/csrc/engine.hpp
+++ b/visual_marker_mapping_amd/csrc/engine.hpp
@@ -122,6 +122,13 @@
     double* fused_partE = nullptr;
     double* fused_partF = nullptr;
     int fused_n_e_act = 0, fused_f_pad = 0, fused_chunks = 0, fused_group = 1, fused_groups = 0;
+
+    bool pose_sums_in_block = false;
+    Task* sum_slotsE = nullptr;
+    Task* sum_slotsF = nullptr;
+    int32_t* sum_wg_poseE = nullptr;
+    int32_t* sum_wg_poseF = nullptr;
+    int sum_wgE = 0, sum_wgF = 0;
 
     double *scale = nullptr, *diag = nullptr, *D2 = nullptr, *delta = nullptr;
     int32_t* active = nullptr;
diff --git a/visual_marker_mapping_amd/csrc/kernels_eval.hip b/visual_marker_mapping_amd/csrc/kernels_eval.hip
--- a/visual_marker_mapping_amd/csrc/kernels_eval.hip
+++ b/visual_marker_mapping_amd/csrc/kernels_eval.hip
@@ -27,12 +27,8 @@
 __device__ __forceinline__ int tri(int a, int b) { return a * (a + 1) / 2 + b; }
 
 template <bool OWN_IS_CAM, bool WRITE_W, typename AT, bool POINTS = false>
-__device__ __forceinline__ void eval_body(const EvalArgs& a, const int wave)
-{
-    const int lane = threadIdx.x & 63;
-    if (wave >= a.n_tasks)
-        return;
-    const Task t = a.tasks[wave];
+__device__ __forceinline__ double eval_task(const EvalArgs& a, const Task t, const int lane)
+{
     const int64_t i = (int64_t)t.begin + lane;
     const bool valid = i < t.end;
     const int64_t is = valid ? i : t.begin;
@@ -154,7 +150,16 @@
 #pragma unroll
     for (int k = 28; k < 32; ++k)
         red[k] = 0.0;
-    const double mine = wave_sum32(red, lane);
+    return wave_sum32(red, lane);
+}
+
+template <bool OWN_IS_CAM, bool WRITE_W, typename AT, bool POINTS = false>
+__device__ __forceinline__ void eval_body(const EvalArgs& a, const int wave)
+{
+    const int lane = threadIdx.x & 63;
+    if (wave >= a.n_tasks)
+        return;
+    const double mine = eval_task<OWN_IS_CAM, WRITE_W, AT, POINTS>(a, a.tasks[wave], lane);
     const int slot = wave_sum32_index(lane);
     if (!(lane & 1) && slot < 28)
         a.part[(int64_t)wave * kPart + slot] = mine;
@@ -398,6 +403,48 @@
     double* gm_out;
 };
 
+template <typename LoadX>
+__device__ __forceinline__ void store_pose_sums(const ReduceArgs& r, const int64_t off, const int p, const int k, const double s,
+                                                const LoadX load_x)
+{
+    double* __restrict__ Hout = r.Hout + off;
+    double* __restrict__ gout = r.gout + off;
+    if (k < 21) {
+        int a = 0;
+        while ((a + 1) * (a + 2) / 2 <= k)
+            ++a;
+        const int b = k - a * (a + 1) / 2;
+        Hout[36 * (int64_t)p + 6 * a + b] = s;
+        Hout[36 * (int64_t)p + 6 * b + a] = s;
+    } else if (k < 27) {
+        gout[6 * (int64_t)p + (k - 21)] = s;
+    } else if (k == 27 && r.pose_cost) {
+        r.pose_cost[p] = s;
+    }
+    if (r.gm_out) {
+        double ng[6];
+#pragma unroll
+        for (int j = 0; j < 6; ++j)
+            ng[j] = -__shfl(s, 21 + j, 32);
+        if (k == 21) {
+            double x[7], xp[7], gm = 0.0;
+            load_x(x);
+            if (r.euclid) {
+#pragma unroll
+                for (int j = 0; j < 6; ++j)
+                    xp[j] = x[j] + ng[j];
+                xp[6] = x[6];
+            } else {
+                pose_plus(x, ng, xp);
+            }
+#pragma unroll
+            for (int j = 0; j < 7; ++j)
+                gm = fmax(gm, fabs(x[j] - xp[j]));
+            r.gm_out[p] = gm;
+        }
+    }
+}
+
 __global__ void k_reduce_pose(const LmCtl* ctl, const ReduceArgs rE, const ReduceArgs rF, const int64_t alt_off)
 {
     int64_t off = 0;
@@ -414,9 +461,6 @@
     const int n_pose = r.n_pose;
     const int32_t* __restrict__ pose_task = r.pose_task;
     const double* __restrict__ part = r.part;
-    double* __restrict__ Hout = r.Hout + off;
-    double* __restrict__ gout = r.gout + off;
-    double* __restrict__ pose_cost = r.pose_cost;
     const int p = tid >> 5, k = tid & 31;
     if (p >= n_pose || k >= 28)
         return;
@@ -434,39 +478,64 @@
     if (t + 1 < t1) s1 += pp[(int64_t)(t + 1) * r.st];
     if (t + 2 < t1) s2 += pp[(int64_t)(t + 2) * r.st];
     const double s = (s0 + s1) + (s2 + s3);
-    if (k < 21) {
-        int a = 0;
-        while ((a + 1) * (a + 2) / 2 <= k)
-            ++a;
-        const int b = k - a * (a + 1) / 2;
-        Hout[36 * (int64_t)p + 6 * a + b] = s;
-        Hout[36 * (int64_t)p + 6 * b + a] = s;
-    } else if (k < 27) {
-        gout[6 * (int64_t)p + (k - 21)] = s;
-    } else if (pose_cost) {
-        pose_cost[p] = s;
-    }
-    if (r.gm_out) {
-        double ng[6];
-#pragma unroll
-        for (int j = 0; j < 6; ++j)
-            ng[j] = -__shfl(s, 21 + j, 32);
-        if (k == 21) {
-            const double* x = r.pose7 + 7 * (int64_t)p;
-            double xp[7], gm = 0.0;
-            if (r.euclid) {
-#pragma unroll
-                for (int j = 0; j < 6; ++j)
-                    xp[j] = x[j] + ng[j];
-                xp[6] = x[6];
-            } else {
-                pose_plus(x, ng, xp);
-            }
-#pragma unroll
-            for (int j = 0; j < 7; ++j)
-                gm = fmax(gm, fabs(x[j] - xp[j]));
-            r.gm_out[p] = gm;
-        }
+    store_pose_sums(r, off, p, k, s, [&](double (&x)[7]) {
+#pragma unroll
+        for (int j = 0; j < 7; ++j)
+            x[j] = r.pose7[7 * (int64_t)p + j];
+    });
+}
+
+template <bool E_IS_CAM>
+__global__ __launch_bounds__(64 * kSumWaves) __attribute__((amdgpu_waves_per_eu(2, 2)))
+void k_eval_sums(const EvalArgs aE, const EvalArgs aF, const int nb_e, const ReduceArgs rE, const ReduceArgs rF,
+                 const int32_t* __restrict__ wg_pose_e, const int32_t* __restrict__ wg_pose_f, const int64_t alt_off)
+{
+    int64_t off = 0;
+    if (aE.ctl) {
+        if (aE.ctl->done)
+            return;
+        phase_stamp(aE.ctl, 0);
+        off = aE.ctl->w_which ? 0 : alt_off;
+    }
+    __shared__ double sh_sum[kSumWaves][28];
+    __shared__ int sh_pose[kSumWaves];
+    const bool is_e = (int)blockIdx.x < nb_e;
+    const int wg = is_e ? (int)blockIdx.x : (int)blockIdx.x - nb_e;
+    const int lane = threadIdx.x & 63, wave = threadIdx.x >> 6;
+    const ReduceArgs& r = is_e ? rE : rF;
+    const int32_t* __restrict__ wg_pose = is_e ? wg_pose_e : wg_pose_f;
+    const int p0 = wg_pose[wg], p1 = wg_pose[wg + 1];
+    const Task t = (is_e ? aE.tasks : aF.tasks)[wg * kSumWaves + wave];
+    if (lane == 0)
+        sh_pose[wave] = t.pose;
+    if (t.begin < t.end) {
+        const double mine = is_e ? eval_task<E_IS_CAM, true, double>(aE, t, lane) : eval_task<!E_IS_CAM, false, double>(aF, t, lane);
+        const int slot = wave_sum32_index(lane);
+        if (!(lane & 1) && slot < 28)
+            sh_sum[wave][slot] = mine;
+    }
+    __syncthreads();
+    const int k = threadIdx.x & 31;
+    for (int p = p0 + (int)(threadIdx.x >> 5); p < p1; p += 2 * kSumWaves) {
+        double s0 = 0.0, s1 = 0.0, s2 = 0.0, s3 = 0.0;
+        int j = 0;
+#pragma unroll
+        for (int w = 0; w < kSumWaves; ++w) {
+            if (sh_pose[w] != p)
+                continue;
+            const double v = sh_sum[w][k < 28 ? k : 0];
+            if ((j & 3) == 0) s0 += v;
+            if ((j & 3) == 1) s1 += v;
+            if ((j & 3) == 2) s2 += v;
+            if ((j & 3) == 3) s3 += v;
+            ++j;
+        }
+        const double s = (s0 + s1) + (s2 + s3);
+        store_pose_sums(r, off, p, k, s, [&](double (&x)[7]) {
+#pragma unroll
+            for (int i = 0; i < 7; ++i)
+                x[i] = r.pose7[7 * (int64_t)p + i];
+        });
     }
 }
 
@@ -698,7 +767,8 @@
     if (!use_ctl)
         aE.ctl = aF.ctl = nullptr;
     const int nb_e = blocks_for_tasks(aE.n_tasks), nb_f = blocks_for_tasks(aF.n_tasks);
-    if (e.fused_eval) {
+    if (e.pose_sums_in_block) {
+    } else if (e.fused_eval) {
         FusedArgs fa;
         fa.pair_obs = e.pair_obs;
         fa.e_list = e.fused_e_list;
@@ -785,8 +855,21 @@
     rF.Hout = e_is_cam ? oH_tag : oH_cam;
     rF.gout = e_is_cam ? og_tag : og_cam;
     rF.pose_cost = nullptr;
-    hipLaunchKernelGGL(k_reduce_pose, dim3(((e.n_e + e.n_f) * 32 + 255) / 256), dim3(256), 0, e.stream, ctl, rE, rF,
-                       (lm && !e.multi) ? e.small_alt_off : (int64_t)0);
+    const int64_t alt_off = (lm && !e.multi) ? e.small_alt_off : (int64_t)0;
+    if (e.pose_sums_in_block) {
+        aE.tasks = e.sum_slotsE;
+        aF.tasks = e.sum_slotsF;
+        const dim3 grid(e.sum_wgE + e.sum_wgF), block(64 * kSumWaves);
+        if (e_is_cam)
+            hipLaunchKernelGGL((k_eval_sums<true>), grid, block, 0, e.stream, aE, aF, e.sum_wgE, rE, rF,
+                               (const int32_t*)e.sum_wg_poseE, (const int32_t*)e.sum_wg_poseF, alt_off);
+        else
+            hipLaunchKernelGGL((k_eval_sums<false>), grid, block, 0, e.stream, aE, aF, e.sum_wgE, rE, rF,
+                               (const int32_t*)e.sum_wg_poseE, (const int32_t*)e.sum_wg_poseF, alt_off);
+    } else {
+        hipLaunchKernelGGL(k_reduce_pose, dim3(((e.n_e + e.n_f) * 32 + 255) / 256), dim3(256), 0, e.stream, ctl, rE, rF,
+                           alt_off);
+    }
     if (!lm)
         hipLaunchKernelGGL(k_sum, dim3(1), dim3(256), 0, e.stream, ctl, e.part_cost, e.n_e, 1,
                            e.cost_slot);
@@ -879,6 +962,8 @@
     bad += hipFuncGetAttributes(&at, reinterpret_cast<const void*>(&k_eval_both<false, float>)) != hipSuccess;
     bad += hipFuncGetAttributes(&at, reinterpret_cast<const void*>(&k_eval_both<true, double, true>)) != hipSuccess;
     bad += hipFuncGetAttributes(&at, reinterpret_cast<const void*>(&k_eval_both<false, double, true>)) != hipSuccess;
+    bad += hipFuncGetAttributes(&at, reinterpret_cast<const void*>(&k_eval_sums<true>)) != hipSuccess;
+    bad += hipFuncGetAttributes(&at, reinterpret_cast<const void*>(&k_eval_sums<false>)) != hipSuccess;
     bad += hipFuncGetAttributes(&at, reinterpret_cast<const void*>(&k_eval_fused<true, double, false>)) != hipSuccess;
     bad += hipFuncGetAttributes(&at, reinterpret_cast<const void*>(&k_eval_fused<false, double, false>)) != hipSuccess;
     bad += hipFuncGetAttributes(&at, reinterpret_cast<const void*>(&k_eval_fused<true, float, false>)) != hipSuccess;
diff --git a/visual_marker_mapping_amd/csrc/kernels_schur.hip b/visual_marker_mapping_amd/csrc/kernels_schur.hip
--- a/visual_marker_mapping_amd/csrc/kernels_schur.hip
+++ b/visual_marker_mapping_amd/csrc/kernels_schur.hip
@@ -9,7 +9,14 @@
     return cholesky<6>(A, A, RowMajor<6>{}, PivotOrOne{});
 }
 
-template <typename WT, bool SPARSE>
+__device__ __forceinline__ void wave_lds_fence()
+{
+    __builtin_amdgcn_fence(__ATOMIC_RELEASE, "wavefront");
+    __builtin_amdgcn_wave_barrier();
+    __builtin_amdgcn_fence(__ATOMIC_ACQUIRE, "wavefront");
+}
+
+template <typename WT, bool SPARSE, bool LINES = false>
 __global__ __launch_bounds__(256) void k_form_z(LmCtl* ctl, int64_t n_obs, int64_t n_pad,
                                                  const int32_t* __restrict__ own,
                                                  const int32_t* __restrict__ other,
@@ -22,56 +29,96 @@
                                                  int f_off_pose, double* __restrict__ Z, int ldz, int zcol,
                                                  const int32_t* __restrict__ e_start)
 {
+    static_assert(!(LINES && SPARSE), "whole-line stores are for the dense Z");
     if (ctl->done)
         return;
     phase_stamp(ctl, 2);
     const int64_t i = (int64_t)blockIdx.x * blockDim.x + threadIdx.x;
-    if (i >= n_obs)
-        return;
-    const WT* __restrict__ W = ctl->w_which ? W1 : W0;
-    const double* __restrict__ H_E = H_E0 + small_sel(ctl, alt_off);
-    const double* __restrict__ g_E = g_E0 + small_sel(ctl, alt_off);
-    const int e = own[i], f = other[i];
-    const double* se = scale + 6 * (int64_t)(e_off_pose + e);
-    const double* sf = scale + 6 * (int64_t)(f_off_pose + f);
-    double L[36];
-    {
-        const double* d2 = D2 + 6 * (int64_t)(e_off_pose + e);
-#pragma unroll
-        for (int a = 0; a < 6; ++a) {
+    const bool valid = i < n_obs;
+    if (!LINES && !valid)
+        return;
+    int e = -1, f = 0;
+    double X[36];
+    if (valid) {
+        const WT* __restrict__ W = ctl->w_which ? W1 : W0;
+        const double* __restrict__ H_E = H_E0 + small_sel(ctl, alt_off);
+        const double* __restrict__ g_E = g_E0 + small_sel(ctl, alt_off);
+        e = own[i];
+        f = other[i];
+        const double* se = scale + 6 * (int64_t)(e_off_pose + e);
+        const double* sf = scale + 6 * (int64_t)(f_off_pose + f);
+        double L[36];
+        {
+            const double* d2 = D2 + 6 * (int64_t)(e_off_pose + e);
+#pragma unroll
+            for (int a = 0; a < 6; ++a) {
+#pragma unroll
+                for (int b = 0; b < 6; ++b)
+                    L[6 * a + b] = se[a] * H_E[36 * (int64_t)e + 6 * a + b] * se[b];
+                L[6 * a + a] += d2[a];
+            }
+        }
+        const bool ok = chol6(L);
+        const bool first = i == 0 || own[i - 1] != e;
+        if (first) {
+            if (!ok)
+                ctl->lin_fail = 1;
+            double v[6];
+#pragma unroll
+            for (int a = 0; a < 6; ++a)
+                v[a] = se[a] * g_E[6 * (int64_t)e + a];
+            forward_substitute<6>(L, RowMajor<6>{}, [&](const int r) { return v[r]; }, [&](const int r, const double t) { v[r] = t; });
+#pragma unroll
+            for (int k = 0; k < 36; ++k)
+                Le[36 * (int64_t)e + k] = L[k];
+#pragma unroll
+            for (int k = 0; k < 6; ++k) {
+                ze[6 * (int64_t)e + k] = v[k];
+                if (!SPARSE)
+                    Z[(int64_t)(6 * e + k) * ldz + zcol] = v[k];
+            }
+        }
+#pragma unroll
+        for (int a = 0; a < 6; ++a)
 #pragma unroll
             for (int b = 0; b < 6; ++b)
-                L[6 * a + b] = se[a] * H_E[36 * (int64_t)e + 6 * a + b] * se[b];
-            L[6 * a + a] += d2[a];
-        }
-    }
-    const bool ok = chol6(L);
-    const bool first = i == 0 || own[i - 1] != e;
-    if (first) {
-        if (!ok)
-            ctl->lin_fail = 1;
-        double v[6];
-#pragma unroll
-        for (int a = 0; a < 6; ++a)
-            v[a] = se[a] * g_E[6 * (int64_t)e + a];
-        forward_substitute<6>(L, RowMajor<6>{}, [&](const int r) { return v[r]; }, [&](const int r, const double t) { v[r] = t; });
-#pragma unroll
-        for (int k = 0; k < 36; ++k)
-            Le[36 * (int64_t)e + k] = L[k];
-#pragma unroll
-        for (int k = 0; k < 6; ++k) {
-            ze[6 * (int64_t)e + k] = v[k];
-            if (!SPARSE)
-                Z[(int64_t)(6 * e + k) * ldz + zcol] = v[k];
-        }
-    }
-    double X[36];
-#pragma unroll
-    for (int a = 0; a < 6; ++a)
-#pragma unroll
-        for (int b = 0; b < 6; ++b)
-            X[6 * a + b] = se[a] * (double)W[(int64_t)(6 * a + b) * n_pad + i] * sf[b];
-    forward_block<6, 6>(L, RowMajor<6>{}, X);
+                X[6 * a + b] = se[a] * (double)W[(int64_t)(6 * a + b) * n_pad + i] * sf[b];
+        forward_block<6, 6>(L, RowMajor<6>{}, X);
+    }
+    if (LINES) {
+        __shared__ __attribute__((aligned(16))) double strip[4][kWave * 6];
+        __shared__ int2 strip_ef[4][kWave];
+        const int lane = threadIdx.x & 63, wave = threadIdx.x >> 6;
+        double* const st = strip[wave];
+        strip_ef[wave][lane] = make_int2(e, f);
+        wave_lds_fence();
+        int64_t zoff[3];
+        bool zok[3];
+#pragma unroll
+        for (int k = 0; k < 3; ++k) {
+            const int m = 2 * (lane + 64 * k);
+            const int2 ef = strip_ef[wave][m / 6];
+            zok[k] = ef.x >= 0;
+            zoff[k] = (int64_t)(6 * ef.x) * ldz + 6 * ef.y + m % 6;
+        }
+#pragma unroll
+        for (int r = 0; r < 6; ++r) {
+            if (valid) {
+#pragma unroll
+                for (int c = 0; c < 6; c += 2)
+                    *reinterpret_cast<double2*>(st + 6 * lane + c) = make_double2(X[6 * r + c], X[6 * r + c + 1]);
+            }
+            wave_lds_fence();
+#pragma unroll
+            for (int k = 0; k < 3; ++k) {
+                const double2 v = *reinterpret_cast<const double2*>(st + 2 * (lane + 64 * k));
+                if (zok[k])
+                    *reinterpret_cast<double2*>(Z + zoff[k] + (int64_t)r * ldz) = v;
+            }
+            wave_lds_fence();
+        }
+        return;
+    }
     int64_t rs = ldz;
     double* zrow = Z + (int64_t)(6 * e) * ldz + 6 * f;
     if (SPARSE) {
@@ -664,20 +711,23 @@
     if (e.ordE.n > 0) {
         const dim3 grid((unsigned)((e.ordE.n + 255) / 256));
         double* const Zout = e.sparse_schur ? e.Zc : e.Z;
-#define VMM_FORM_Z(WT, SP, W0, W1)                                                                                      \
-    hipLaunchKernelGGL((k_form_z<WT, SP>), grid, dim3(256), 0, e.stream, e.ctl, e.ordE.n, e.ordE.n_pad, e.ordE.own,      \
-                       e.ordE.other, (const WT*)(W0), (const WT*)(W1), H_E, g_E, e.small_alt_off, (const double*)e.D2,   \
-                       e.Le, e.ze, e.scale, e_off, f_off, Zout, e.ldz, e.n_pad, (const int32_t*)e.ordE.start)
+#define VMM_FORM_Z(WT, W0, W1, ...)                                                                                     \
+    hipLaunchKernelGGL((k_form_z<WT, __VA_ARGS__>), grid, dim3(256), 0, e.stream, e.ctl, e.ordE.n, e.ordE.n_pad,         \
+                       e.ordE.own, e.ordE.other, (const WT*)(W0), (const WT*)(W1), H_E, g_E, e.small_alt_off,            \
+                       (const double*)e.D2, e.Le, e.ze, e.scale, e_off, f_off, Zout, e.ldz, e.n_pad,                     \
+                       (const int32_t*)e.ordE.start)
         if (e.f32_accum) {
             if (e.sparse_schur)
-                VMM_FORM_Z(float, true, e.Wf, e.Wf2);
+                VMM_FORM_Z(float, e.Wf, e.Wf2, true);
             else
-                VMM_FORM_Z(float, false, e.Wf, e.Wf2);
+                VMM_FORM_Z(float, e.Wf, e.Wf2, false);
         } else {
             if (e.sparse_schur)
-                VMM_FORM_Z(double, true, e.W, e.W2);
+                VMM_FORM_Z(double, e.W, e.W2, true);
+            else if (e.sw.z_store_scalar)
+                VMM_FORM_Z(double, e.W, e.W2, false);
             else
-                VMM_FORM_Z(double, false, e.W, e.W2);
+                VMM_FORM_Z(double, e.W, e.W2, false, true);
         }
 #undef VMM_FORM_Z
     }
@@ -867,6 +917,7 @@
     hipFuncAttributes at;
     int bad = 0;
     bad += hipFuncGetAttributes(&at, reinterpret_cast<const void*>(&k_form_z<double, false>)) != hipSuccess;
+    bad += hipFuncGetAttributes(&at, reinterpret_cast<const void*>(&k_form_z<double, false, true>)) != hipSuccess;
     bad += hipFuncGetAttributes(&at, reinterpret_cast<const void*>(&k_form_z<float, false>)) != hipSuccess;
     bad += hipFuncGetAttributes(&at, reinterpret_cast<const void*>(&k_form_z<double, true>)) != hipSuccess;
     bad += hipFuncGetAttributes(&at, reinterpret_cast<const void*>(&k_form_z<float, true>)) != hipSuccess;
diff --git a/visual_marker_mapping_amd/csrc/plan.cpp b/visual_marker_mapping_amd/csrc/plan.cpp
--- a/visual_marker_mapping_amd/csrc/plan.cpp
+++ b/visual_marker_mapping_amd/csrc/plan.cpp
@@ -67,6 +67,10 @@
         s.syrk_slices = std::max(1, atoi(v));
     s.syrk_no_xcd = env_is("VMM_BA_SYRK_NO_XCD", '1');
     s.syrk_wide = !env_is("VMM_BA_SYRK_WIDE", '0');
+    if (const char* v = getenv("VMM_BA_POSE_SUMS"))
+        s.pose_sums_kernel = !strcmp(v, "kernel");
+    if (const char* v = getenv("VMM_BA_Z_STORE"))
+        s.z_store_scalar = !strcmp(v, "scalar");
     if (const char* v = getenv("VMM_BA_DF_MAX_WG"))
         s.df_max_wg = atoi(v);
     if (const char* v = getenv("VMM_BA_CHOL_TAIL"))
@@ -169,6 +173,33 @@
     o.pose_task[n_own] = (int32_t)o.tasks.size();
     o.start.assign(start.begin(), start.end());
     return o;
+}
+
+bool plan_pose_sums(const OrderPlan& o, int n_own, PoseSumOrder& out)
+{
+    out = PoseSumOrder();
+    if (o.tasks.empty())
+        return false;
+    Task empty;
+    empty.pose = -1;
+    empty.begin = empty.end = 0;
+    out.wg_pose.push_back(0);
+    for (int p = 0; p < n_own; ++p) {
+        const int t0 = o.pose_task[(size_t)p], t1 = o.pose_task[(size_t)p + 1];
+        if (t1 - t0 > kSumWaves)
+            return false;
+        const int used = (int)(out.slots.size() % kSumWaves);
+        if (used + (t1 - t0) > kSumWaves) {
+            out.pads += kSumWaves - used;
+            out.slots.resize(out.slots.size() + (size_t)(kSumWaves - used), empty);
+        }
+        if (t1 > t0 && out.slots.size() % kSumWaves == 0 && !out.slots.empty())
+            out.wg_pose.push_back(p);
+        out.slots.insert(out.slots.end(), o.tasks.begin() + t0, o.tasks.begin() + t1);
+    }
+    out.slots.resize((size_t)round_up((int64_t)out.slots.size(), kSumWaves), empty);
+    out.wg_pose.push_back(n_own);
+    return true;
 }
 
 SyrkSchedule plan_syrk(int n_row_blk, int n_col_blk, int k_pad, int n_cu, const Switches& sw)
@@ -669,6 +700,13 @@
             }
         }
     }
+    if (!sw.pose_sums_kernel && !multi && !points && !P.fused_eval && !P.sparse_schur &&
+        plan_pose_sums(P.ordE, n_e, P.sumE) && plan_pose_sums(P.ordF, n_f, P.sumF))
+        P.pose_sums_in_block = 8 * (size_t)(P.sumE.pads + P.sumF.pads) <= P.ordE.tasks.size() + P.ordF.tasks.size();
+    if (!P.pose_sums_in_block) {
+        P.sumE = PoseSumOrder();
+        P.sumF = PoseSumOrder();
+    }
     if (!P.sparse_schur)
         return P;
 
diff --git a/visual_marker_mapping_amd/csrc/plan.hpp b/visual_marker_mapping_amd/csrc/plan.hpp
--- a/visual_marker_mapping_amd/csrc/plan.hpp
+++ b/visual_marker_mapping_amd/csrc/plan.hpp
@@ -61,6 +61,8 @@
     int syrk_slices = 0;
     bool syrk_no_xcd = false;
     bool syrk_wide = true;
+    bool pose_sums_kernel = false;
+    bool z_store_scalar = false;
     int df_max_wg = 0;
     int chol_tail = -1;
     bool df_bulk = false;
@@ -87,6 +89,14 @@
 };
 OrderPlan plan_order(int n_own, const int32_t* own_idx, const int32_t* other_idx, const double* px, int64_t n);
 
+constexpr int kSumWaves = 8;
+struct PoseSumOrder {
+    std::vector<Task> slots;
+    std::vector<int32_t> wg_pose;
+    int pads = 0;
+};
+bool plan_pose_sums(const OrderPlan& o, int n_own, PoseSumOrder& out);
+
 struct SyrkSchedule {
     int n_tiles = 0, n_kt = 0, n_wg = 0, n_segments = 0;
     bool wide = false;
@@ -99,6 +109,8 @@
     std::string error;
     int n_e = 0, n_f = 0;
     OrderPlan ordE, ordF;
+    bool pose_sums_in_block = false;
+    PoseSumOrder sumE, sumF;
     bool fused_eval = false;
     int fused_n_e_act = 0, fused_f_pad = 0, fused_chunks = 0, fused_group = 1, fused_groups = 0, fused_slots = 0;
     std::vector<int32_t> pair_obs, fused_e_list, fused_e_part0, fused_pose_task;
diff --git a/visual_marker_mapping_amd/csrc/vmm_ba.hip b/visual_marker_mapping_amd/csrc/vmm_ba.hip
--- a/visual_marker_mapping_amd/csrc/vmm_ba.hip
+++ b/visual_marker_mapping_amd/csrc/vmm_ba.hip
@@ -617,6 +617,7 @@
     e.n_e = P.n_e;
     e.n_f = P.n_f;
     e.fused_eval = P.fused_eval;
+    e.pose_sums_in_block = P.pose_sums_in_block && !e.f32_accum;
     e.fused_n_e_act = P.fused_n_e_act;
     e.fused_f_pad = P.fused_f_pad;
     e.fused_chunks = P.fused_chunks;
@@ -687,6 +688,18 @@
         if ((rc = upload(e, e.fused_e_list, P.fused_e_list))) return rc;
         if ((rc = upload(e, e.fused_e_part0, P.fused_e_part0))) return rc;
         if ((rc = upload(e, e.fused_pose_task, P.fused_pose_task))) return rc;
+    }
+    if (e.pose_sums_in_block) {
+        e.sum_wgE = (int)(P.sumE.slots.size() / kSumWaves);
+        e.sum_wgF = (int)(P.sumF.slots.size() / kSumWaves);
+        if ((rc = dev_alloc(e, &e.sum_slotsE, P.sumE.slots.size()))) return rc;
+        if ((rc = dev_alloc(e, &e.sum_slotsF, P.sumF.slots.size()))) return rc;
+        if ((rc = dev_alloc(e, &e.sum_wg_poseE, P.sumE.wg_pose.size()))) return rc;
+        if ((rc = dev_alloc(e, &e.sum_wg_poseF, P.sumF.wg_pose.size()))) return rc;
+        if ((rc = upload(e, e.sum_slotsE, P.sumE.slots))) return rc;
+        if ((rc = upload(e, e.sum_slotsF, P.sumF.slots))) return rc;
+        if ((rc = upload(e, e.sum_wg_poseE, P.sumE.wg_pose))) return rc;
+        if ((rc = upload(e, e.sum_wg_poseF, P.sumF.wg_pose))) return rc;
     }
 
     e.small_count = (size_t)42 * n_pose + 2;
diff --git a/visual_marker_mapping_amd/engine.py b/visual_marker_mapping_amd/engine.py
--- a/visual_marker_mapping_amd/engine.py
+++ b/visual_marker_mapping_amd/engine.py
@@ -279,6 +279,14 @@
         return dict(zip(("syrk_ms", "cholesky_ms", "sequential_ms", "concurrent_ms", "cholesky_in_concurrent_ms",
                          "syrk_in_concurrent_ms", "concurrent_syrk_first_ms", "cholesky_in_concurrent_syrk_first_ms"), out.tolist()))
 
+    def debug_elimination(self, options=None):
+        o = options or default_options()
+        dims = np.zeros(3, np.int32)
+        _lib.check(_lib.lib().vmm_ba_debug_elimination(self._h, C.byref(o), _ptr(dims), None, None, None))
+        Z, Le, ze = np.zeros((dims[0], dims[1])), np.zeros((dims[2], 6, 6)), np.zeros((dims[2], 6))
+        _lib.check(_lib.lib().vmm_ba_debug_elimination(self._h, C.byref(o), _ptr(dims), _ptr(Z), _ptr(Le), _ptr(ze)))
+        return {"Z": Z, "Le": Le, "ze": ze}
+
     def time_kernels(self, options=None, reps=5):
         o = options or default_options()
         t = _lib.KernelTimes()
```

After: 2516 LM iterations/s (median of 6 runs). 1.01x the previous value.
